# Chuanming-Liu/DAzimSurfTomo

Measured on AMD Instinct MI355X. Metric: FMM traveltime fields/sec (256^2 grid, 16 periods) + LSQR SpMV HBM GB/s, higher is better.
Workload: dtype f32

## Files before the change

dazimsurftomo_amd/csrc/assemble.hip:

```cpp
#include "sparse_internal.h"

#include <rocprim/device/device_scan.hpp>

namespace {

__device__ __forceinline__ bool tikh_face(int cell, int nvx, int nvz, int nzm1, int &i, int &j, int &k) {
  k = cell / (nvx * nvz);
  const int r = cell - k * nvx * nvz;
  j = r / nvx;
  i = r - j * nvx;
  return i == 0 || i == nvx - 1 || j == 0 || j == nvz - 1 || k == 0 || k == nzm1 - 1;
}
__global__ void k_tikh_count(int64_t r0, int64_t nrow, int maxvp, int nvx, int nvz, int nzm1, long *cnt) {
  const int64_t r = (int64_t)blockIdx.x * VB + threadIdx.x;
  if (r > nrow) return;
  int i, j, k;
  cnt[r] = r == nrow ? 0 : (tikh_face((int)((r0 + r) % maxvp), nvx, nvz, nzm1, i, j, k) ? 1 : 7);
}
__global__ void k_tikh_fill(int64_t r0, int64_t nrow, int maxvp, int nvx, int nvz, int nzm1, const long *off, int64_t nnz0,
                            const float *__restrict__ w, int64_t *__restrict__ rowptr, int *__restrict__ col,
                            float *__restrict__ val) {
  const int64_t r = (int64_t)blockIdx.x * VB + threadIdx.x;
  if (r > nrow) return;
  rowptr[r] = nnz0 + off[r];
// ... 94 lines not shown
    if (ratio > 1.0f) sigma = sigma * (float)exp((double)(ratio - 1.0f));
    const float wt = 1.0f / sigma;
    wgt[i] = wt;
    rhs[i] = res[i] * wt;
  }
}
__global__ void k_weight_sums(int64_t n, const float *res, const float *wgt, const float *rhs, double *part) {
  double a[5] = {0, 0, 0, 0, 0};
  for (int64_t i = (int64_t)blockIdx.x * VB + threadIdx.x; i < n; i += (int64_t)gridDim.x * VB) {
    const double r = res[i];
    a[0] += r; a[1] += fabs(r); a[2] += r * r; a[3] += wgt[i]; a[4] += fabsf(rhs[i]);
  }
  __shared__ double s[5][VB / 64];
#pragma unroll
  for (int q = 0; q < 5; q++) {
    const double t = wave_sum(a[q]);
    if ((threadIdx.x & 63) == 0) s[q][threadIdx.x >> 6] = t;
  }
  __syncthreads();
  if (threadIdx.x < 5) {
    double t = 0.0;
    for (int i = 0; i < VB / 64; i++) t += s[threadIdx.x][i];
    part[blockIdx.x * 5 + threadIdx.x] = t;
  }
}
__global__ void k_model_update(int nx, int ny, int nzm1, int joint, float *vs, float *dv, float minvel, float maxvel, float *gc,
                               float *gs) {
  const int nvx = nx - 2, nvz = ny - 2, maxvp = nvx * nvz * nzm1;
  const int ii = blockIdx.x * VB + threadIdx.x;
  if (ii >= maxvp) return;
  const int k = ii / (nvx * nvz), r = ii - k * nvx * nvz, j = r / nvx, i = r - j * nvx;
  float p = dv[ii];
  if (p >= 0.500f) p = 0.500f;
  if (p <= -0.500f) p = -0.500f;
  if (fabsf(p) < 1e-5f) p = 0.0f;
  dv[ii] = p;
  const size_t iv = ((size_t)k * ny + (j + 1)) * nx + (i + 1);
  float v = vs[iv] + p;
  if (v < minvel) v = minvel;
  if (v > maxvel) v = maxvel;
  vs[iv] = v;
  if (joint) {
    if (gc) gc[ii] = dv[maxvp + ii];
    if (gs) gs[ii] = dv[2 * maxvp + ii];
  }
}
__global__ void k_map_update(int nx, int ny, int kmax, int azim, double *pv, float *dm, float minc, float maxc, float *a1, float *a2) {
  const int nvx = nx - 2, nvz = ny - 2, nmap = nvx * nvz * kmax;
  const int ii = blockIdx.x * VB + threadIdx.x;
  if (ii >= nmap) return;
  const int k = ii / (nvx * nvz), r = ii - k * nvx * nvz, j = r / nvx, i = r - j * nvx;
  float p = dm[ii];
  if (p >= 0.500f) p = 0.500f;
  if (p <= -0.500f) p = -0.500f;
  if (fabsf(p) < 1e-5f) p = 0.0f;
  dm[ii] = p;
  const size_t iv = ((size_t)k * ny + (j + 1)) * nx + (i + 1);
  float v = (float)pv[iv] + p;
  if (v < minc) v = minc;
  if (v > maxc) v = maxc;
  pv[iv] = (double)v;
  if (azim) {
    if (a1) a1[ii] = dm[nmap + ii];
    if (a2) a2[ii] = dm[2 * nmap + ii];
  }
}
__global__ void k_update_stats(int ncell, const float *dv, float *out) {
  const float *x = dv + (size_t)blockIdx.x * ncell;
  float mn = INFINITY, mx = -INFINITY;
  double sa = 0.0;
  for (int i = threadIdx.x; i < ncell; i += VB) {
    const float v = x[i];
    mn = fminf(mn, v);
    mx = fmaxf(mx, v);
    sa += fabsf(v);
  }
#pragma unroll
  for (int o = 32; o > 0; o >>= 1) {
    mn = fminf(mn, __shfl_xor(mn, o));
    mx = fmaxf(mx, __shfl_xor(mx, o));
  }
  sa = wave_sum(sa);
  __shared__ float s_mn[VB / 64], s_mx[VB / 64];
  __shared__ double s_sa[VB / 64];
  if ((threadIdx.x & 63) == 0) { s_mn[threadIdx.x >> 6] = mn; s_mx[threadIdx.x >> 6] = mx; s_sa[threadIdx.x >> 6] = sa; }
  __syncthreads();
  if (threadIdx.x == 0) {
    for (int i = 1; i < VB / 64; i++) { mn = fminf(mn, s_mn[i]); mx = fmaxf(mx, s_mx[i]); sa += s_sa[i]; }
    out[blockIdx.x * 3 + 0] = mn; out[blockIdx.x * 3 + 1] = mx; out[blockIdx.x * 3 + 2] = (float)sa;
  }
}

}

extern "C" {

static int append_stencil_rows(dazim_ctx *ctx, dazim_csr *A, bool lap2d, int nvx, int nvz, int nzm1, int64_t maxvp, int64_t row_lo,
                               int64_t nrow, int nblock, const float *w_host, float *dw, long *cnt, long *off);

int dazim_csr_append_tikhonov(dazim_ctx *ctx, dazim_csr *A, int nx, int ny, int nz, int nblock, const float *w_host) {
  if (nblock < 1 || nx < 3 || ny < 3 || nz < 2) return dz_fail(ctx, DAZIM_E_BAD_ARG, "bad arguments to dazim_csr_append_tikhonov");
  return dazim_csr_append_tikhonov_rows(ctx, A, nx, ny, nz, nblock, w_host, 0, (int64_t)(nx - 2) * (ny - 2) * (nz - 1) * nblock);
}
int dazim_csr_append_tikhonov_rows(dazim_ctx *ctx, dazim_csr *A, int nx, int ny, int nz, int nblock, const float *w_host,
                                   int64_t row_lo, int64_t row_hi) {
  if (!ctx || !A || !w_host || nblock < 1 || nx < 3 || ny < 3 || nz < 2) return dz_fail(ctx, DAZIM_E_BAD_ARG, "bad arguments to dazim_csr_append_tikhonov");
  const int nvx = nx - 2, nvz = ny - 2, nzm1 = nz - 1;
  const int64_t maxvp = (int64_t)nvx * nvz * nzm1, nrow = row_hi - row_lo;
  if (row_lo < 0 || row_hi < row_lo || row_hi > maxvp * nblock) return dz_fail(ctx, DAZIM_E_BAD_ARG, "bad row range of the regularisation block");
  if (maxvp * nblock > A->n || maxvp > 0x7ffffff0) return dz_fail(ctx, DAZIM_E_BAD_ARG, "regularisation blocks do not fit the %lld columns", (long long)A->n);
  DZ_HIP(hipSetDevice(ctx->device));
  int rc;
  long *cnt, *off;
  float *dw;
  if ((rc = dz_scratch(ctx, "tikh.cnt", (size_t)(nrow + 1), &cnt)) || (rc = dz_scratch(ctx, "tikh.off", (size_t)(nrow + 1), &off)) ||
      (rc = dz_scratch(ctx, "tikh.w", 64, &dw)))
    return rc;
  if (nblock > 64) return dz_fail(ctx, DAZIM_E_BAD_ARG, "too many regularisation blocks");
  return append_stencil_rows(ctx, A, false, nvx, nvz, nzm1, maxvp, row_lo, nrow, nblock, w_host, dw, cnt, off);
}

static int append_stencil_rows(dazim_ctx *ctx, dazim_csr *A, bool lap2d, int nvx, int nvz, int nzm1, int64_t maxvp, int64_t row_lo,
                               int64_t nrow, int nblock, const float *w_host, float *dw, long *cnt, long *off) {
  int rc;
  void *p;
  DZ_HIP(hipMemcpyAsync(dw, w_host, (size_t)nblock * 4, hipMemcpyHostToDevice, ctx->stream));
  const unsigned nb = (unsigned)((nrow + 1 + VB - 1) / VB);
  if (lap2d)
    hipLaunchKernelGGL(k_lap2d_count, dim3(nb), dim3(VB), 0, ctx->stream, nrow, (int)maxvp, nvx, nvz, cnt);
  else
    hipLaunchKernelGGL(k_tikh_count, dim3(nb), dim3(VB), 0, ctx->stream, row_lo, nrow, (int)maxvp, nvx, nvz, nzm1, cnt);
  auto fill = [&](int64_t *rowptr, int *col, float *val) {
    if (lap2d)
      hipLaunchKernelGGL(k_lap2d_fill, dim3(nb), dim3(VB), 0, ctx->stream, nrow, (int)maxvp, nvx, nvz, off, A->nnz, dw, rowptr, col, val);
    else
      hipLaunchKernelGGL(k_tikh_fill, dim3(nb), dim3(VB), 0, ctx->stream, row_lo, nrow, (int)maxvp, nvx, nvz, nzm1, off, A->nnz, dw,
                         rowptr, col, val);
  };
  size_t tb = 0;
  DZ_HIP(rocprim::exclusive_scan(nullptr, tb, cnt, off, 0l, (size_t)(nrow + 1), rocprim::plus<long>(), ctx->stream));
  if ((rc = dz_scratch(ctx, "tikh.scan", tb + 256, &p))) return rc;
  DZ_HIP(rocprim::exclusive_scan(p, tb, cnt, off, 0l, (size_t)(nrow + 1), rocprim::plus<long>(), ctx->stream));
  long nnz2 = 0;
  DZ_HIP(hipMemcpyAsync(&nnz2, off + nrow, 8, hipMemcpyDeviceToHost, ctx->stream));
  DZ_HIP(hipStreamSynchronize(ctx->stream));
  const int64_t m2 = A->m + nrow, nz2 = A->nnz + nnz2;
  if (nz2 > 0xfffffff0ll) return dz_fail(ctx, DAZIM_E_NNZ_OVERFLOW, "too many stored entries");
  if (A->cap_m >= m2 && A->cap_nnz >= nz2) {
    const int64_t nnz1 = A->nnz;
    fill(A->rowptr + A->m, A->col, A->val);
    DZ_HIP(hipGetLastError());
    A->m = m2;
    A->nnz = nz2;
    if ((rc = dz_build_colblocks(ctx, A, nnz1 > 0 ? nnz1 : 0))) return rc;
    if ((rc = dz_invalidate_transpose(A))) return rc;
    DZ_HIP(hipStreamSynchronize(ctx->stream));
    return 0;
  }
  int64_t *rowptr;
  int *col;
  float *val;
  if ((rc = dz_big_get(ctx, (size_t)(m2 + 1), &rowptr)) || (rc = dz_big_get(ctx, (size_t)(nz2 > 0 ? nz2 : 1), &col)) ||
      (rc = dz_big_get(ctx, (size_t)(nz2 > 0 ? nz2 : 1), &val)))
    return rc;
  DZ_HIP(hipMemcpyAsync(rowptr, A->rowptr, (size_t)A->m * 8, hipMemcpyDeviceToDevice, ctx->stream));
  DZ_HIP(hipMemcpyAsync(col, A->col, (size_t)A->nnz * 4, hipMemcpyDeviceToDevice, ctx->stream));
  DZ_HIP(hipMemcpyAsync(val, A->val, (size_t)A->nnz * 4, hipMemcpyDeviceToDevice, ctx->stream));
  fill(rowptr + A->m, col, val);
  DZ_HIP(hipGetLastError());
  DZ_HIP(hipStreamSynchronize(ctx->stream));
  dz_big_put(ctx, A->rowptr);
  dz_big_put(ctx, A->col);
  dz_big_put(ctx, A->val);
  A->rowptr = rowptr; A->col = col; A->val = val;
  A->m = m2; A->nnz = nz2;
  A->cap_m = A->cap_nnz = 0;
  if ((rc = dz_build_colblocks(ctx, A))) return rc;
  if ((rc = dz_invalidate_transpose(A))) return rc;
  DZ_HIP(hipStreamSynchronize(ctx->stream));
  return 0;
}

int dazim_csr_append_laplacian2d(dazim_ctx *ctx, dazim_csr *A, int nx, int ny, int nmap, const float *w_host) {
  if (!ctx || !A || !w_host || nmap < 1 || nx < 3 || ny < 3) return dz_fail(ctx, DAZIM_E_BAD_ARG, "bad arguments to dazim_csr_append_laplacian2d");
  const int nvx = nx - 2, nvz = ny - 2;
  const int64_t ncell = (int64_t)nvx * nvz, nrow = ncell * nmap;
  if (nrow > A->n || nrow > 0x7ffffff0) return dz_fail(ctx, DAZIM_E_BAD_ARG, "regularisation maps do not fit the %lld columns", (long long)A->n);
  DZ_HIP(hipSetDevice(ctx->device));
  int rc;
  long *cnt, *off;
  float *dw;
  if ((rc = dz_scratch(ctx, "tikh.cnt", (size_t)(nrow + 1), &cnt)) || (rc = dz_scratch(ctx, "tikh.off", (size_t)(nrow + 1), &off)) ||
      (rc = dz_scratch(ctx, "lap2d.w", (size_t)nmap, &dw)))
    return rc;
  return append_stencil_rows(ctx, A, true, nvx, nvz, 1, ncell, 0, nrow, nmap, w_host, dw, cnt, off);
}

int dazim_weight_data(dazim_ctx *ctx, dazim_csr *G, int64_t dall, const float *obst_u, const float *dsyn_u, float *res_u,
                      float *wgt_u, float *rhs_u, float *stats) {
  return dazim_weight_data_sharded(ctx, G, dall, 0, dall, obst_u, dsyn_u, res_u, wgt_u, rhs_u, stats);
}
int dazim_weight_data_sharded(dazim_ctx *ctx, dazim_csr *G, int64_t dall, int64_t row0, int64_t dall_glob, const float *obst_u,
                              const float *dsyn_u, float *res_u, float *wgt_u, float *rhs_u, float *stats) {
  if (!ctx || dall < 1 || !obst_u || !dsyn_u || !res_u || !wgt_u || !rhs_u || (G && G->m < dall) || row0 < 0 || row0 + dall > dall_glob)
    return dz_fail(ctx, DAZIM_E_BAD_ARG, "bad arguments to dazim_weight_data");
  const bool sharded = ctx->comm && dall_glob > dall;
  DZ_HIP(hipSetDevice(ctx->device));
  DzBuf<float> obst, dsyn, res, wgt, rhs;
  int rc;
  if ((rc = obst.init(ctx, obst_u, dall, true, false)) || (rc = dsyn.init(ctx, dsyn_u, dall, true, false)) ||
      (rc = res.init(ctx, res_u, dall, false, true)) || (rc = wgt.init(ctx, wgt_u, dall, false, true)) ||
      (rc = rhs.init(ctx, rhs_u, dall, false, true)))
    return rc;
  float *rel, *ms;
  double *part;
  if ((rc = dz_scratch(ctx, "wd.rel", (size_t)dall, &rel)) || (rc = dz_scratch(ctx, "wd.ms", 16, &ms)) ||
      (rc = dz_scratch(ctx, "wd.part", (size_t)NPART * 5, &part)))
    return rc;
  const int nb = nblk(dall, NPART);
  hipLaunchKernelGGL(k_residual, dim3(nb), dim3(VB), 0, ctx->stream, dall, obst.dev, dsyn.dev, res.dev, rel);
  if (sharded) {
    float *relg;
    if ((rc = dz_scratch(ctx, "wd.relg", (size_t)dall_glob, &relg))) return rc;
    DZ_HIP(hipMemsetAsync(relg, 0, (size_t)dall_glob * 4, ctx->stream));
    DZ_HIP(hipMemcpyAsync(relg + row0, rel, (size_t)dall * 4, hipMemcpyDeviceToDevice, ctx->stream));
    if ((rc = dz_allreduce(ctx, (DzComm *)ctx->comm, relg, (size_t)dall_glob, DZ_F32, DZ_SUM))) return rc;
    hipLaunchKernelGGL(k_sigma_stats, dim3(1), dim3(VB), 0, ctx->stream, dall_glob, relg, ms);
  } else {
    hipLaunchKernelGGL(k_sigma_stats, dim3(1), dim3(VB), 0, ctx->stream, dall, rel, ms);
  }
  hipLaunchKernelGGL(k_sigma_weights, dim3(nb), dim3(VB), 0, ctx->stream, dall, obst.dev, res.dev, rel, ms, wgt.dev, rhs.dev);
  hipLaunchKernelGGL(k_weight_sums, dim3(nb), dim3(VB), 0, ctx->stream, dall, res.dev, wgt.dev, rhs.dev, part);
  DZ_HIP(hipGetLastError());
  std::vector<double> hp((size_t)nb * 5);
  float hms[2];
  DZ_HIP(hipMemcpyAsync(hp.data(), part, hp.size() * 8, hipMemcpyDeviceToHost, ctx->stream));
  DZ_HIP(hipMemcpyAsync(hms, ms, 8, hipMemcpyDeviceToHost, ctx->stream));
  if (G && (rc = dz_scale_rows(ctx, G, dall, wgt.dev))) return rc;
  DZ_HIP(hipStreamSynchronize(ctx->stream));
  if (stats) {
    double a[5] = {0, 0, 0, 0, 0};
    for (int b = 0; b < nb; b++)
      for (int q = 0; q < 5; q++) a[q] += hp[(size_t)b * 5 + q];
    if (sharded && (rc = dazim_comm_allreduce(ctx, a, 5, DZ_F64, DZ_SUM))) return rc;
    const double n = (double)dall_glob, mean = a[0] / n;
    stats[0] = (float)mean;
    stats[1] = (float)sqrt(fmax(a[2] / n - mean * mean, 0.0));
    stats[2] = (float)(a[1] / n);
    stats[3] = (float)sqrt(a[2] / n);
    stats[4] = hms[0];
    stats[5] = hms[1];
    stats[6] = (float)(a[3] / n);
    stats[7] = (float)(a[4] / n);
  }
  if ((rc = res.finish()) || (rc = wgt.finish()) || (rc = rhs.finish())) return rc;
  DZ_HIP(hipStreamSynchronize(ctx->stream));
  return 0;
}

int dazim_model_update(dazim_ctx *ctx, int nx, int ny, int nz, int joint, float *vs_u, float *dv_u, float minvel, float maxvel,
                       float *gc_u, float *gs_u, float *stats) {
  if (!ctx || !vs_u || !dv_u || nx < 3 || ny < 3 || nz < 2) return dz_fail(ctx, DAZIM_E_BAD_ARG, "bad arguments to dazim_model_update");
  DZ_HIP(hipSetDevice(ctx->device));
  const int nzm1 = nz - 1, ncell = (nx - 2) * (ny - 2), maxvp = ncell * nzm1, nblock = joint ? 3 : 1;
  DzBuf<float> vs, dv, gc, gs;
  int rc;
  if ((rc = vs.init(ctx, vs_u, (size_t)nx * ny * nz, true, true)) || (rc = dv.init(ctx, dv_u, (size_t)maxvp * nblock, true, true)) ||
      (rc = gc.init(ctx, gc_u, joint ? maxvp : 0, false, true)) || (rc = gs.init(ctx, gs_u, joint ? maxvp : 0, false, true)))
    return rc;
  hipLaunchKernelGGL(k_model_update, dim3((maxvp + VB - 1) / VB), dim3(VB), 0, ctx->stream, nx, ny, nzm1, joint, vs.dev, dv.dev,
                     minvel, maxvel, joint ? gc.dev : nullptr, joint ? gs.dev : nullptr);
  DZ_HIP(hipGetLastError());
  if (stats) {
    float *p;
    if ((rc = dz_scratch(ctx, "mu.stats", (size_t)nblock * nzm1 * 3, &p))) return rc;
    hipLaunchKernelGGL(k_update_stats, dim3(nblock * nzm1), dim3(VB), 0, ctx->stream, ncell, dv.dev, p);
    DZ_HIP(hipGetLastError());
    DZ_HIP(hipMemcpyAsync(stats, p, (size_t)nblock * nzm1 * 3 * 4, hipMemcpyDeviceToHost, ctx->stream));
  }
  if ((rc = vs.finish()) || (rc = dv.finish()) || (rc = gc.finish()) || (rc = gs.finish())) return rc;
  DZ_HIP(hipStreamSynchronize(ctx->stream));
  return 0;
}

int dazim_phase_map_update(dazim_ctx *ctx, int nx, int ny, int kmax, int azim, double *pv_u, float *dm_u, float minc, float maxc,
                           float *a1_u, float *a2_u, float *stats) {
  if (!ctx || !pv_u || !dm_u || nx < 3 || ny < 3 || kmax < 1) return dz_fail(ctx, DAZIM_E_BAD_ARG, "bad arguments to dazim_phase_map_update");
  DZ_HIP(hipSetDevice(ctx->device));
  const int ncell = (nx - 2) * (ny - 2), nmap = ncell * kmax, nblock = azim ? 3 : 1;
  DzBuf<double> pv;
  DzBuf<float> dm, a1, a2;
  int rc;
  if ((rc = pv.init(ctx, pv_u, (size_t)nx * ny * kmax, true, true)) || (rc = dm.init(ctx, dm_u, (size_t)nmap * nblock, true, true)) ||
      (rc = a1.init(ctx, a1_u, azim ? nmap : 0, false, true)) || (rc = a2.init(ctx, a2_u, azim ? nmap : 0, false, true)))
    return rc;
  hipLaunchKernelGGL(k_map_update, dim3((nmap + VB - 1) / VB), dim3(VB), 0, ctx->stream, nx, ny, kmax, azim ? 1 : 0, pv.dev, dm.dev,
                     minc, maxc, azim ? a1.dev : nullptr, azim ? a2.dev : nullptr);
  DZ_HIP(hipGetLastError());
  if (stats) {
    float *p;
    if ((rc = dz_scratch(ctx, "mu.stats", (size_t)nblock * kmax * 3, &p))) return rc;
    hipLaunchKernelGGL(k_update_stats, dim3(nblock * kmax), dim3(VB), 0, ctx->stream, ncell, dm.dev, p);
    DZ_HIP(hipGetLastError());
    DZ_HIP(hipMemcpyAsync(stats, p, (size_t)nblock * kmax * 3 * 4, hipMemcpyDeviceToHost, ctx->stream));
  }
  if ((rc = pv.finish()) || (rc = dm.finish()) || (rc = a1.finish()) || (rc = a2.finish())) return rc;
  DZ_HIP(hipStreamSynchronize(ctx->stream));
  return 0;
}

}
```

dazimsurftomo_amd/csrc/dazim_internal.h:

```cpp
#pragma once
#include <hip/hip_runtime.h>
#include <rccl/rccl.h>

#include <cstdarg>
#include <cstdio>
#include <cstring>
#include <functional>
#include <map>
#include <memory>
#include <string>
#include <vector>

#include "../../include/dazim.h"

struct dazim_ctx {
  int device = 0;
  hipStream_t stream = nullptr;
  hipEvent_t ev0 = nullptr, ev1 = nullptr;
  std::string err;
  std::map<std::string, double> ksec;
  int num_cu = 256;
  std::map<std::string, int> opts;
  std::map<std::string, std::pair<void *, size_t>> scratch;
  std::map<std::string, std::pair<void *, size_t>> pinned;
  bool fmm_busy = false;
  struct StageBlock { void *p; size_t bytes; bool busy; };
  std::vector<StageBlock> stage;
  std::vector<StageBlock> big;
  hipStream_t stream2 = nullptr;
  hipEvent_t ev_fork = nullptr, ev_a0 = nullptr, ev_a1 = nullptr;
  bool aux_pending = false, aux_timed = false;
  struct AuxRange { const char *p; size_t bytes; };
  std::vector<AuxRange> aux_ranges;
  int (*aux_epilogue)(dazim_ctx *) = nullptr;
  struct ShardPending {
    int nx = 0, ny = 0, nz = 0, kmax = 0;
    const double *send = nullptr;
    double *svs = nullptr, *svp = nullptr, *srho = nullptr;
  } shard;
  struct TiledFields {
    const unsigned *tiled = nullptr;
    const int *tslot = nullptr;
    int nfield = 0, nnx = 0, nnz = 0, stride = 0, tsh = 0;
    const int *fdone = nullptr;
    unsigned nwg = 0;
    volatile unsigned *hprog = nullptr;
    unsigned total_tasks = 0;
  } fields;
  std::function<int()> fmm_finish;
  unsigned *hprog = nullptr;
  hipStream_t stream3 = nullptr;
  hipEvent_t ev_f0 = nullptr, ev_f1 = nullptr, ev_pre = nullptr, ev_r0 = nullptr, ev_r1 = nullptr;
  void *comm = nullptr;
  void (*comm_release)(dazim_ctx *) = nullptr;
  int nranks = 1, rank = 0;
};

int dz_fail(dazim_ctx *c, int code, const char *fmt, ...);
static inline int dz_opt(const dazim_ctx *ctx, const char *name, int def) {
  const auto it = ctx->opts.find(name);
  return it == ctx->opts.end() ? def : it->second;
}

struct DzComm {
  ncclComm_t nccl = nullptr;
  std::string dir;
  std::string tag;
  unsigned seq = 0;
  int nranks = 1, rank = 0;
};
enum { DZ_F32 = 0, DZ_F64 = 1, DZ_I64 = 2, DZ_SUM = 0, DZ_MAX = 1 };
int dz_allgather(dazim_ctx *ctx, DzComm *c, const void *send_dev, void *recv_dev, size_t bytes);
int dz_allreduce(dazim_ctx *ctx, DzComm *c, void *dbuf, size_t count, int dtype, int op);
void dz_comm_abort(dazim_ctx *ctx);
static inline void dz_shard_even(int64_t n, int world, int rank, int64_t *lo, int64_t *hi) {
  const int64_t base = n / world, rem = n % world;
  *lo = rank * base + (rank < rem ? rank : rem);
  *hi = *lo + base + (rank < rem ? 1 : 0);
}

#define DZ_NCCL(call)                                                                                        \
  do {                                                                                                        \
    ncclResult_t r_ = (call);                                                                                 \
    if (r_ != ncclSuccess) return dz_fail(ctx, -2000 - (int)r_, "%s:%d %s -> %s", __FILE__, __LINE__, #call, ncclGetErrorString(r_)); \
  } while (0)
int dz_aux_init(dazim_ctx *ctx);
int dz_async_init(dazim_ctx *ctx);
int dz_fmm_finish(dazim_ctx *ctx);
int dz_join_aux(dazim_ctx *ctx);
int dz_join_aux_if_touched(dazim_ctx *ctx, const void *dev, size_t bytes);

#define DZ_HIP(call)                                                                           \
  do {                                                                                         \
    hipError_t e_ = (call);                                                                    \
    if (e_ != hipSuccess)                                                                      \
      return dz_fail(ctx, -(int)e_ - 1000, "%s:%d %s -> %s", __FILE__, __LINE__, #call,       \
                     hipGetErrorString(e_));                                                   \
  } while (0)

__host__ __device__ constexpr int dz_tile_shift(int nz) { int l = 0; while ((1 << l) < ((nz + 3) >> 2)) l++; return l + 4; }
__host__ __device__ constexpr int dz_tile_records(int nx, int nz) { return ((nx + 3) >> 2) << dz_tile_shift(nz); }
__host__ __device__ __forceinline__ constexpr int dz_tile_x(int x0, int tsh) { return ((x0 >> 2) << tsh) + ((x0 & 3) << 2); }
__host__ __device__ __forceinline__ constexpr int dz_tile_z(int z0) { return ((z0 & ~3) << 2) | (z0 & 3); }

__device__ __forceinline__ double dz_row_kernel(float v, double svs, double svp, double srho) {
  const float coe_a = (2.0947f - 0.8206f * 2 * v + 0.2683f * 3 * (v * v) - 0.0251f * 4 * (v * v * v));
  const float vpft = 0.9409f + 2.0947f * v - 0.8206f * (v * v) + 0.2683f * (v * v * v) - 0.0251f * (v * v * v * v);
  const float coe_rho = coe_a * (1.6612f - 0.4721f * 2 * vpft + 0.0671f * 3 * (vpft * vpft) -
                                 0.0043f * 4 * (vpft * vpft * vpft) + 0.000106f * 5 * (vpft * vpft * vpft * vpft));
  return svp * (double)coe_a + srho * (double)coe_rho + svs;
}

int dz_scratch(dazim_ctx *ctx, const char *name, size_t bytes, void **out);
int dz_pinned(dazim_ctx *ctx, const char *name, size_t bytes, void **out);

size_t dz_trim_caches(dazim_ctx *ctx);
hipError_t dz_malloc_retry(dazim_ctx *ctx, void **p, size_t bytes);
bool dz_is_device_ptr(const void *p);
int dz_stage_get(dazim_ctx *ctx, size_t bytes, void **out);
void dz_stage_put(dazim_ctx *ctx, void *p);
int dz_big_get(dazim_ctx *ctx, size_t bytes, void **out);
void dz_big_put(dazim_ctx *ctx, void *p);
template <class T>
static inline int dz_scratch(dazim_ctx *ctx, const char *name, size_t count, T **out) {
  void *p = nullptr;
  const int rc = dz_scratch(ctx, name, count * sizeof(T), &p);
  *out = (T *)p;
  return rc;
}
template <class T>
static inline int dz_big_get(dazim_ctx *ctx, size_t count, T **out) {
  void *p = nullptr;
  const int rc = dz_big_get(ctx, count * sizeof(T), &p);
  *out = (T *)p;
  return rc;
}

extern "C" int dz_csr_adopt_cap(dazim_ctx *ctx, int64_t m, int64_t n, int64_t nnz, int64_t *rowptr, int *col, float *val,
                                int64_t cap_m, int64_t cap_nnz, dazim_csr **out);

extern "C" int dz_csr_set_twin(dazim_ctx *ctx, dazim_csr *A, dazim_csr *B);

int dz_check_range(dazim_ctx *ctx, const int *a_dev, int64_t n, int lo, int hi, const char *what);

template <class T>
struct DzBuf {
  dazim_ctx *ctx = nullptr;
  T *user = nullptr;
  T *dev = nullptr;
  size_t n = 0;
  bool staged = false, out = false;
  int init(dazim_ctx *c, const T *p, size_t count, bool copy_in, bool copy_out) {
    ctx = c;
    user = const_cast<T *>(p);
    n = count;
    out = copy_out;
    if (!p || count == 0) return 0;
    if (dz_is_device_ptr(p)) {
      dev = user;
      return 0;
    }
    staged = true;
    {
      void *blk = nullptr;
      int rc_ = dz_stage_get(ctx, n * sizeof(T), &blk);
      if (rc_) return rc_;
      dev = (T *)blk;
    }
    if (copy_in) DZ_HIP(hipMemcpyAsync(dev, user, n * sizeof(T), hipMemcpyHostToDevice, ctx->stream));
    return 0;
  }
  int finish() {
    if (staged && out && dev)
      DZ_HIP(hipMemcpyAsync(user, dev, n * sizeof(T), hipMemcpyDeviceToHost, ctx->stream));
    return 0;
  }
  ~DzBuf() {
    if (staged && dev) {
      (void)hipStreamSynchronize(ctx->stream);
      dz_stage_put(ctx, dev);
    }
  }
};

struct DzTimer {
  dazim_ctx *ctx;
  const char *name;
  DzTimer(dazim_ctx *c, const char *n) : ctx(c), name(n) { (void)hipEventRecord(ctx->ev0, ctx->stream); }
  void stop() {
    (void)hipEventRecord(ctx->ev1, ctx->stream);
    (void)hipEventSynchronize(ctx->ev1);
    float ms = 0;
    (void)hipEventElapsedTime(&ms, ctx->ev0, ctx->ev1);
    ctx->ksec[name] = ms * 1e-3;
  }
};
```

dazimsurftomo_amd/csrc/lsmr.hip:

```cpp
#include "sparse_internal.h"

#include <rccl/rccl.h>
#include <cstdlib>

namespace {

__global__ void finish_norm(const double *part, int np, float *res, double *res_d) {
  double t = 0.0;
  for (int i = threadIdx.x; i < np; i += 64) t += part[i];
  t = wave_sum(t);
  if (threadIdx.x == 0) {
    res[0] = (float)sqrt(t);
    if (res_d) res_d[0] = t;
  }
}
__global__ void k_sqrt_sum(const double *sum, float *res) { res[0] = (float)sqrt(sum[0]); }
__global__ void k_axpby_norm(int64_t n, const float *w, float *v, const float *beta_p, float beta_sign, double *part,
                             const int *guard) {
  if (guard && *guard) return;
  const float beta = beta_p ? beta_sign * beta_p[0] : beta_sign;
  double sq = 0.0;
  for (int64_t i = (int64_t)blockIdx.x * VB + threadIdx.x; i < n; i += (int64_t)gridDim.x * VB) {
    const float o = beta * v[i] + w[i];
    v[i] = o;
// ... 232 lines not shown
      v[idx[e]] = vr[e];
      sq += (double)vr[e] * vr[e];
    }
  sq = wave_sum(sq);
  __syncthreads();
  if (lane == 0) s_w[w] = sq;
  __syncthreads();
  if (tid == 0) {
    double t = 0.0;
    for (int i = 0; i < RC_THREADS / 64; i++) t += s_w[i];
    part_out[blockIdx.x] = t;
  }
}
__global__ void k_alpha_update(int64_t n, float *v, float *h, float *hbar, float *x, const double *part, int np,
                               double *partx, LsmrState *S) {
  if (S->stop) return;
  __shared__ float s_f[4];
  const bool half2 = !S->stop2;
  const double t = half2 ? block_total(part, np) : 0.0;
  if (threadIdx.x == 0) {
    LsmrState st = *S;
    const float alpha = half2 ? (float)sqrt(t) : st.alpha;
    float f1, f2, f3;
    lsmr_recur(st, alpha, st.beta, f1, f2, f3);
    s_f[0] = f1; s_f[1] = f2; s_f[2] = f3; s_f[3] = alpha;
    if (blockIdx.x == 0) S->alpha_new = alpha;
  }
  __syncthreads();
  const float f1 = s_f[0], f2 = s_f[1], f3 = s_f[2], alpha = s_f[3];
  const bool scal = half2 && alpha > 0.0f;
  const float a = scal ? 1.0f / alpha : 1.0f;
  double sq = 0.0;
  for (int64_t i = (int64_t)blockIdx.x * VB + threadIdx.x; i < n; i += (int64_t)gridDim.x * VB) {
    float vi = v[i];
    if (scal) {
      vi = a * vi;
      v[i] = vi;
    }
    const float hb = h[i] - f1 * hbar[i];
    const float xn = x[i] + f2 * hb;
    hbar[i] = hb;
    x[i] = xn;
    h[i] = vi - f3 * h[i];
    sq += (double)xn * xn;
  }
  block_partial(sq, partx);
}
__global__ void k_tests(const double *partx, int npx, const float *x, LsmrState *S, dazim_lsmr_rec *trace, int trace_cap) {
  if (S->stop) return;
  const double t = block_total(partx, npx);
  if (threadIdx.x != 0) return;
  LsmrState st = *S;
  float f1, f2, f3;
  lsmr_recur(st, st.alpha_new, st.beta, f1, f2, f3);
  const float normx = (float)sqrt(t);
  st.normx = normx;
  const float test1 = st.normr / st.normb, test2 = st.normAr / (st.normA * st.normr), test3 = 1.0f / st.condA;
  const float t1 = test1 / (1.0f + st.normA * normx / st.normb);
  const float rtol = st.btol + st.atol * st.normA * normx / st.normb;
  int istop = 0;
  if (st.itn >= st.itnlim) istop = 7;
  if (1.0f + test3 <= 1.0f) istop = 6;
  if (1.0f + test2 <= 1.0f) istop = 5;
  if (1.0f + t1 <= 1.0f) istop = 4;
  if (test3 <= st.ctol) istop = 3;
  if (test2 <= st.atol) istop = 2;
  if (test1 <= rtol) istop = 1;
  st.istop = istop;
  st.stop = istop != 0;
  st.stop2 = st.stop;
  if (trace && st.itn < trace_cap) {
    dazim_lsmr_rec r;
    r.itn = st.itn; r.x1 = x[0]; r.normr = st.normr; r.normAr = st.normAr; r.test1 = test1; r.test2 = test2;
    r.test3 = test3; r.rtol = rtol; r.normA = st.normA; r.condA = st.condA;
    trace[st.itn] = r;
  }
  *S = st;
}

constexpr int CHECK = 8, NSLOT = 2;
struct LsmrArgs {
  dazim_ctx *ctx; const dazim_csr *A; const float *b_u;
  float damp, atol, btol, conlim; int itnlim, localSize; float *x_u;
  int *istop_o, *itn_o; float *normA_o, *condA_o, *normr_o, *normAr_o, *normx_o;
  dazim_lsmr_rec *trace; int trace_cap, *trace_n;
};
struct LsmrSolve : LsmrArgs {
  const int64_t m, n;
  DzComm *comm;
  DzBuf<float> b, x;
  double *d_sum = nullptr;
  long long *d_cons = nullptr;
  float *wbuf = nullptr;
  char *gbuf = nullptr;
  const size_t w_sum_off, w_bytes;
  int64_t m_glob;
  int localVecs = 0;
  float *u = nullptr, *v = nullptr, *h = nullptr, *hbar = nullptr, *localV = nullptr, *d_scal = nullptr;
  double *part = nullptr, *part2 = nullptr, *partx = nullptr;
  LsmrState *S = nullptr;
  dazim_lsmr_rec *d_trace = nullptr;
  const int gm, gn, bn, bm;
  int gm_t, gn_t;
  struct Pinned {
    LsmrState *h = nullptr;
    hipEvent_t e0 = nullptr, e1 = nullptr, done[NSLOT] = {}, ta[NSLOT][4] = {};
    ~Pinned() {
      if (e0) (void)hipEventDestroy(e0);
      if (e1) (void)hipEventDestroy(e1);
      for (int i = 0; i < NSLOT; i++) {
        if (done[i]) (void)hipEventDestroy(done[i]);
        for (int j = 0; j < 4; j++)
          if (ta[i][j]) (void)hipEventDestroy(ta[i][j]);
      }
      if (h) (void)hipHostFree(h);
    }
  } guard;
  LsmrState *h_state = nullptr;
  float *h_scal = nullptr;
  const int *g1 = nullptr, *g2 = nullptr;
  int istop = 0, itn = 0, ntrace = 0;
  float normA = 0, condA = 0, normr = 0, normAr = 0, normx = 0, normb = 0;
  double t_spmv = 0, t_spmvt = 0;
  int n_spmv = 0, n_spmvt = 0;
  long n_enq = 0;
  long n_coll = 0;
  bool rccl_allreduce = false;
  int host_syncs = 0;
  int coop_max = 0, rcb = 0;
  int64_t per_thread = 0;
  unsigned reorth_barriers = 0;

  explicit LsmrSolve(const LsmrArgs &a)
      : LsmrArgs(a), m(A->m), n(A->n), comm((DzComm *)ctx->comm), w_sum_off((((size_t)n * 4 + 7) / 8) * 8), w_bytes(w_sum_off + 8),
        m_glob(m), gm(dz_spmv_blocks(ctx, m, n)), gn(dz_spmv_blocks(ctx, n, m)), bn(nblk(n, NPART)), bm(nblk(m, NPART)), gm_t(gm),
        gn_t(gn) {}

  int alloc() {
    int r;
    if ((r = b.init(ctx, b_u, m, true, false)) || (r = x.init(ctx, x_u, n, false, true))) return r;
    if (comm) {
      if ((r = dz_scratch(ctx, "lsmr.cons", 8, &d_cons)) || (r = dz_scratch(ctx, "lsmr.sum", 8, &d_sum)) ||
          (r = dz_scratch(ctx, "lsmr.w", w_bytes / 4, &wbuf)) || (r = dz_scratch(ctx, "lsmr.gather", w_bytes * (size_t)comm->nranks, &gbuf)))
        return r;
    }
    const int npart = gm > gn ? (gm > NPART ? gm : NPART) : (gn > NPART ? gn : NPART);
    if ((r = dz_scratch(ctx, "lsmr.u", (size_t)m, &u)) || (r = dz_scratch(ctx, "lsmr.v", (size_t)n, &v)) ||
        (r = dz_scratch(ctx, "lsmr.h", (size_t)n, &h)) || (r = dz_scratch(ctx, "lsmr.hbar", (size_t)n, &hbar)) ||
        (r = dz_scratch(ctx, "lsmr.part", (size_t)npart, &part)) || (r = dz_scratch(ctx, "lsmr.part2", (size_t)NPART * 2 + 8, &part2)) ||
        (r = dz_scratch(ctx, "lsmr.partx", (size_t)NPART, &partx)) || (r = dz_scratch(ctx, "lsmr.scal", 16, &d_scal)) ||
        (r = dz_scratch(ctx, "lsmr.state", 1, &S)))
      return r;
    if (trace && (r = dz_scratch(ctx, "lsmr.trace", (size_t)trace_cap, &d_trace))) return r;
    if (!dz_use_scatter(ctx, A) && !A->colptr && (r = dz_build_transpose(ctx, const_cast<dazim_csr *>(A)))) return r;
    const int64_t lv = localSize < 0 ? 0 : (localSize < n ? localSize : n);
    if (lv > 0 && (r = dz_scratch(ctx, "lsmr.localV", (size_t)n * lv, &localV))) return r;
    return 0;
  }
  int leave(int code) {
    if (comm) dz_comm_abort(ctx);
    comm = nullptr;
    return code;
  }
  int agree(int rc) {
    if (!comm) return rc;
    long long hv[4] = {rc != 0 ? 1 : 0, (long long)n, -(long long)n, 0}, *dv = d_cons;
    double hm = (double)m;
    if (!dv) return leave(rc ? rc : dz_fail(ctx, -3, "row-sharded LSMR: no memory for the consensus buffer"));
    (void)hipMemcpyAsync(dv, hv, sizeof hv, hipMemcpyHostToDevice, ctx->stream);
    (void)hipMemcpyAsync(dv + 4, &hm, 8, hipMemcpyHostToDevice, ctx->stream);
    const int r1 = dz_allreduce(ctx, comm, dv, 3, DZ_I64, DZ_MAX);
    const int r2 = dz_allreduce(ctx, comm, dv + 4, 1, DZ_F64, DZ_SUM);
    (void)hipMemcpyAsync(hv, dv, sizeof hv, hipMemcpyDeviceToHost, ctx->stream);
    (void)hipMemcpyAsync(&hm, dv + 4, 8, hipMemcpyDeviceToHost, ctx->stream);
    hipError_t e = hipStreamSynchronize(ctx->stream);
    if (rc) return rc;
    if (r1 != 0 || r2 != 0 || e != hipSuccess) return dz_fail(ctx, -2000, "row-sharded LSMR: consensus all-reduce failed");
    if (hv[0]) return dz_fail(ctx, -2001, "row-sharded LSMR: another rank failed during set-up");
    if (hv[1] != -hv[2]) return dz_fail(ctx, DAZIM_E_BAD_ARG, "row-sharded LSMR: the ranks disagree on the number of columns (%lld here, %lld elsewhere)", (long long)n, hv[1]);
    m_glob = (int64_t)hm;
    return 0;
  }
  int prepare() {
    localVecs = localSize < 0 ? 0 : localSize;
    if (m_glob < localVecs) localVecs = (int)m_glob;
    if (n < localVecs) localVecs = (int)n;
    DZ_HIP(hipHostMalloc((void **)&guard.h, sizeof(LsmrState) * (NSLOT + 1) + 64));
    h_state = guard.h;
    h_scal = (float *)(guard.h + NSLOT + 1);
    DZ_HIP(hipEventCreate(&guard.e0));
    DZ_HIP(hipEventCreate(&guard.e1));
    for (int i = 0; i < NSLOT; i++) {
      DZ_HIP(hipEventCreate(&guard.done[i]));
      for (int j = 0; j < 4; j++) DZ_HIP(hipEventCreate(&guard.ta[i][j]));
    }
    return 0;
  }
  void plan_reorth() {
    if (!getenv("DAZIM_CU_MASK")) {
      int occ = 0;
      if (hipOccupancyMaxActiveBlocksPerMultiprocessor(&occ, k_reorth_coop<16>, RC_THREADS, 0) == hipSuccess && occ > 0) coop_max = occ * ctx->num_cu;
      else (void)hipGetLastError();
    }
    rcb = (int)((n + (int64_t)RC_THREADS * RC_EMAX - 1) / ((int64_t)RC_THREADS * RC_EMAX));
    if (rcb < 8) rcb = 8;
    if (rcb > (int)((n + RC_THREADS - 1) / RC_THREADS)) rcb = (int)((n + RC_THREADS - 1) / RC_THREADS);
    if (rcb > RC_BLOCKS) rcb = RC_BLOCKS;
    per_thread = (n + (int64_t)rcb * RC_THREADS - 1) / ((int64_t)rcb * RC_THREADS);
  }
  int norm_to_host(const double *pp, int np, float *res, bool rowwise = false) {
    if (comm && rowwise) {
      hipLaunchKernelGGL(finish_norm, dim3(1), dim3(64), 0, ctx->stream, pp, np, d_scal, d_sum);
      if (const int rr = dz_allreduce(ctx, comm, d_sum, 1, DZ_F64, DZ_SUM)) return rr;
      hipLaunchKernelGGL(k_sqrt_sum, dim3(1), dim3(1), 0, ctx->stream, d_sum, d_scal);
    } else {
      hipLaunchKernelGGL(finish_norm, dim3(1), dim3(64), 0, ctx->stream, pp, np, d_scal, (double *)nullptr);
    }
    DZ_HIP(hipMemcpyAsync(h_scal, d_scal, 4, hipMemcpyDeviceToHost, ctx->stream));
    DZ_HIP(hipStreamSynchronize(ctx->stream));
    *res = h_scal[0];
    return 0;
  }
  int spmvT(const float *beta_p, float sign, const int *g) {
    if (!comm) return dz_launch_spmvT(ctx, A, u, 1.0f, v, beta_p, sign, part, &gn_t, g);
    DZ_HIP(hipMemsetAsync(wbuf, 0, n * 4, ctx->stream));
    if (const int r = dz_launch_spmvT(ctx, A, u, 1.0f, wbuf, nullptr, 1.0f, nullptr, nullptr, g)) return r;
    if (const int rr = dz_allreduce(ctx, comm, wbuf, (size_t)n, DZ_F32, DZ_SUM)) return rr;
    hipLaunchKernelGGL(k_axpby_norm, dim3(bn), dim3(VB), 0, ctx->stream, n, wbuf, v, beta_p, sign, part, g);
    gn_t = bn;
    return 0;
  }
  int start() {
    int rc;
    DZ_HIP(hipEventRecord(guard.e0, ctx->stream));
    hipLaunchKernelGGL(k_copy, dim3(bm), dim3(VB), 0, ctx->stream, m, b.dev, u);
    DZ_HIP(hipMemsetAsync(v, 0, n * 4, ctx->stream));
    DZ_HIP(hipMemsetAsync(x.dev, 0, n * 4, ctx->stream));
    DZ_HIP(hipMemsetAsync(hbar, 0, n * 4, ctx->stream));
    hipLaunchKernelGGL(k_sumsq, dim3(bm), dim3(VB), 0, ctx->stream, m, u, part);
    float alpha = 0.0f, beta = 0.0f;
    if ((rc = norm_to_host(part, bm, &beta, true))) return rc;
    if (beta > 0.0f) {
      hipLaunchKernelGGL(k_scal_inv, dim3(bm), dim3(VB), 0, ctx->stream, m, u, d_scal, 1.0f);
      if ((rc = spmvT(nullptr, 1.0f, nullptr))) return rc;
      if ((rc = norm_to_host(part, gn_t, &alpha))) return rc;
    }
    if (alpha > 0.0f) hipLaunchKernelGGL(k_scal_inv, dim3(bn), dim3(VB), 0, ctx->stream, n, v, d_scal, 1.0f);
    normAr = alpha * beta;
    normb = beta;
    if (trace) {
      memset(&trace[0], 0, sizeof trace[0]);
      trace[0].normr = beta; trace[0].normAr = normAr; trace[0].test1 = 1.0f; trace[0].test2 = beta > 0.0f ? alpha / beta : 0.0f;
      ntrace = 1;
    }
    if (normAr == 0.0f) return 0;
    if (localVecs > 0) hipLaunchKernelGGL(k_copy, dim3(bn), dim3(VB), 0, ctx->stream, n, v, localV);
    hipLaunchKernelGGL(k_copy, dim3(bn), dim3(VB), 0, ctx->stream, n, v, h);
    LsmrState &s0 = h_state[NSLOT];
    memset(&s0, 0, sizeof s0);
    s0.alpha = alpha; s0.beta = beta; s0.alphabar = alpha; s0.zetabar = alpha * beta; s0.rho = 1; s0.rhobar = 1; s0.cbar = 1;
    s0.betadd = beta; s0.rhodold = 1; s0.normA2 = alpha * alpha; s0.minrbar = 1e+30f; s0.normb = beta;
    s0.ctol = conlim > 0.0f ? 1.0f / conlim : 0.0f;
    s0.normr = beta; s0.normAr = normAr; s0.damp = damp; s0.atol = atol; s0.btol = btol; s0.itnlim = itnlim;
    DZ_HIP(hipMemcpyAsync(S, &s0, sizeof s0, hipMemcpyHostToDevice, ctx->stream));
    if (d_trace) DZ_HIP(hipMemsetAsync(d_trace, 0, (size_t)trace_cap * sizeof(dazim_lsmr_rec), ctx->stream));
    g1 = &S->stop;
    g2 = &S->stop2;
    plan_reorth();
    rccl_allreduce = comm && comm->nccl && dz_opt(ctx, "comm.allreduce", 0) == 1;
    DZ_HIP(hipMemsetAsync(part2 + 2 * NPART, 0, 64, ctx->stream));
    return 0;
  }
  int half_step_u(hipEvent_t *tev) {
    if (tev) DZ_HIP(hipEventRecord(tev[0], ctx->stream));
    if (const int r = dz_launch_spmvA(ctx, A, v, u, &S->alpha, -1.0f, part, &gm_t, g1)) return r;
    if (tev) DZ_HIP(hipEventRecord(tev[1], ctx->stream));
    return 0;
  }
  int half_step_v(float *slot, hipEvent_t *tev) {
    int r;
    if (!comm) {
      hipLaunchKernelGGL(k_beta_scal_u, dim3(bm > bn ? bm : bn), dim3(VB), 0, ctx->stream, m, u, part, gm_t,
                         (const double *)nullptr, n, v, slot, S);
      if (tev) DZ_HIP(hipEventRecord(tev[2], ctx->stream));
      if ((r = spmvT(&S->beta, -1.0f, g2))) return r;
      if (tev) DZ_HIP(hipEventRecord(tev[3], ctx->stream));
      return 0;
    }
    float *d_bp = reinterpret_cast<float *>(d_sum + 4);
    double *w_sum = reinterpret_cast<double *>(reinterpret_cast<char *>(wbuf) + w_sum_off);
    const int bmn = bm > bn ? bm : bn;
    hipLaunchKernelGGL(k_local_norm_scal, dim3(bm), dim3(VB), 0, ctx->stream, m, u, part, gm_t, w_sum, d_bp, S);
    if (tev) DZ_HIP(hipEventRecord(tev[2], ctx->stream));
    DZ_HIP(hipMemsetAsync(wbuf, 0, n * 4, ctx->stream));
    if ((r = dz_launch_spmvT(ctx, A, u, 1.0f, wbuf, nullptr, 1.0f, nullptr, nullptr, g1))) return r;
    hipLaunchKernelGGL(k_scale_by, dim3(bn), dim3(VB), 0, ctx->stream, n, wbuf, d_bp, g1);
    if (tev) DZ_HIP(hipEventRecord(tev[3], ctx->stream));
    if (rccl_allreduce) {
      DZ_NCCL(ncclGroupStart());
      const ncclResult_t ra = ncclAllReduce(wbuf, wbuf, (size_t)n, ncclFloat, ncclSum, comm->nccl, ctx->stream);
      const ncclResult_t rb = ncclAllReduce(w_sum, w_sum, 1, ncclDouble, ncclSum, comm->nccl, ctx->stream);
      const ncclResult_t rg = ncclGroupEnd();
      if (ra != ncclSuccess || rb != ncclSuccess || rg != ncclSuccess) {
        const ncclResult_t bad = ra != ncclSuccess ? ra : (rb != ncclSuccess ? rb : rg);
        return dz_fail(ctx, -2000 - (int)bad, "row-sharded LSMR: grouped ncclAllReduce -> %s", ncclGetErrorString(bad));
      }
// ... 156 lines not shown
```

dazimsurftomo_amd/csrc/rays.hip:

```cpp
#include <cmath>
#include <chrono>
#include <unistd.h>

#include "dazim_internal.h"

#include <rocprim/device/device_scan.hpp>
#include <rocprim/device/device_radix_sort.hpp>

namespace {

constexpr int GDX = 5, GDZ = 5;
constexpr int RM = DAZIM_RMAX;
constexpr float EARTH = 6371.0f;
constexpr float FTOL = 1e-4f;

struct RayArgs {
  dazim_geom g;
  int nx, ny, nz, kmax;
  long nray;
  const int *field;
  const float *rcx, *rcz;
  const float *scx, *scz;
  const int *period;
  const int *kidx;
  const float *veln;
  const float *ttn;
  const int *tslot;
  int tsh;
  long fstride;
  const int *fdone;
  int *defer_mark;
  int max_quads;
  int sweeps;
  const float *ttnr;
  const int *nstsr;
  const dazim_refbox *boxes;
  const float *vels;
  const double *svs, *svp, *srho;
  unsigned nvx_magic;
  const double *skern;
  const float *lsen;
  double r_dnx, r_dnz, r_dnxr, r_dnzr, r_dvx, r_dvz, r_e2dnx, r_e2dnxr;
  float dplh;
  float *dsurf;
  int *status;
  int *rbflag;
  long *count;
  int *nlist;
  unsigned short *lcell;
  float *lval;
  float *fdm_scratch;
  int LK;
  int lcap;
  const unsigned *perm;
  unsigned *qcount;
  float2 *pts;
  int *npts;
  int pcap;
  int dense;
  long *countd;
  int keep_small;
  const long *rowptr;
  float *val;
  int *col;
};

__device__ __forceinline__ float dz_sinf(float x) {
  if (!(x > 0.0f && x < 3.1415927f)) return (float)sin((double)x);
  const double y = (double)x - 1.5707963267948966192;
  const double y2 = y * y;
  double p = -1.5619206968586226e-16;
  p = fma(p, y2, 4.7794773323873853e-14);
  p = fma(p, y2, -1.1470745597729725e-11);
  p = fma(p, y2, 2.0876756987868099e-09);
  p = fma(p, y2, -2.7557319223985891e-07);
  p = fma(p, y2, 2.4801587301587302e-05);
  p = fma(p, y2, -1.3888888888888889e-03);
  p = fma(p, y2, 4.1666666666666664e-02);
  p = fma(p, y2, -0.5);
  p = fma(p, y2, 1.0);
  return (float)p;
}

__device__ __forceinline__ void step_azimuth(float x0, float z0, float x1, float z1, float &c2psi, float &s2psi) {
  const float PI_F = 3.1415926535898f;
  const float evtlat = (PI_F / 2 - x0) * 180.0f / PI_F, evtlon = z0 * 180.0f / PI_F;
  const float stalat = (PI_F / 2 - x1) * 180.0f / PI_F, stalon = z1 * 180.0f / PI_F;
  const double pi = (double)3.1415926535898f;
  const float piby2 = (float)(pi / (double)2.f);
  const double rad = (double)2.f * pi / (double)360.f;
  const double sph = (double)(1.0f / 298.257f);
  const double scolat = (double)piby2 - atan((1. - sph) * (1. - sph) * tan((double)stalat * rad));
  const double ecolat = (double)piby2 - atan((1. - sph) * (1. - sph) * tan((double)evtlat * rad));
  const double slon = (double)stalon * rad, elon = (double)evtlon * rad;
  const double a = sin(scolat) * cos(slon), b = sin(scolat) * sin(slon), c = cos(scolat);
  const double dd = sin(elon), ee = -cos(elon), cc = cos(ecolat);
  const double gg = -cc * ee, hh = cc * dd, kk = -sin(ecolat);
  const double rhs1 = (a - dd) * (a - dd) + (b - ee) * (b - ee) + c * c - (double)2.f;
  const double rhs2 = (a - gg) * (a - gg) + (b - hh) * (b - hh) + (c - kk) * (c - kk) - (double)2.f;
  double daz = atan2(rhs1, rhs2);
  if (daz < 0.0) daz = daz + 2 * pi;
  float az = (float)(daz / rad);
  if (fabsf(az - 360.f) < .00001f) az = 0.0f;
  const float rgpsi = az / 180 * PI_F;
  c2psi = (float)cos((double)(2.0f * rgpsi));
  s2psi = (float)sin((double)(2.0f * rgpsi));
}

__device__ __forceinline__ float divr(float x, double rd) { return (float)((double)x * rd); }

__device__ __forceinline__ void basis(float v, float b[4]) {
  const float om = 1.0f - v;
  b[0] = om * om * om / 6.0f;
  b[1] = (4.0f - 6.0f * (v * v) + 3.0f * (v * v * v)) / 6.0f;
  b[2] = (1.0f + 3.0f * v + 3.0f * (v * v) - 3.0f * (v * v * v)) / 6.0f;
  b[3] = v * v * v / 6.0f;
}

__device__ __forceinline__ float div6(float x) { return divr(x, 1.0 / 6.0); }
__device__ __forceinline__ float basis1(float v, int i) {
  const float om = 1.0f - v;
  const float n0 = om * om * om;
  const float n1 = 4.0f - 6.0f * (v * v) + 3.0f * (v * v * v);
  const float n2 = 1.0f + 3.0f * v + 3.0f * (v * v) - 3.0f * (v * v * v);
  const float n3 = v * v * v;
  return div6(i == 0 ? n0 : (i == 1 ? n1 : (i == 2 ? n2 : n3)));
}

__device__ __forceinline__ float vel_at(const dazim_geom &g, const float *veln, int ipx, int ipz, float drx, float drz,
                                        double rdnx, double rdnz) {
  float vel = 0.0f;
#pragma unroll
  for (int l = 1; l <= 2; l++)
#pragma unroll
    for (int m = 1; m <= 2; m++) {
      float produ = (1.0f - fabsf(divr((float)(m - 1) * g.dnz - drz, rdnz)));
      produ = produ * (1.0f - fabsf(divr((float)(l - 1) * g.dnx - drx, rdnx)));
      if (ipz - 1 + m <= g.nnz && ipx - 1 + l <= g.nnx && ipz - 1 + m >= 1 && ipx - 1 + l >= 1)
        vel = vel + veln[(size_t)(ipx - 2 + l) * g.nnz + (ipz - 2 + m)] * produ;
    }
  return vel;
}

__device__ __forceinline__ float bilin_cell(const dazim_geom &g, const float *veln, int cx, int cz, float px, float pz,
                                            double rdnx, double rdnz) {
  const float drx = (px - g.gox) - (float)(cx - 1) * g.dnx;
  const float drz = (pz - g.goz) - (float)(cz - 1) * g.dnz;
  float biv = 0.0f;
#pragma unroll
  for (int i = 1; i <= 2; i++)
#pragma unroll
    for (int j = 1; j <= 2; j++) {
      const float produ = (1.0f - fabsf(divr((float)(i - 1) * g.dnx - drx, rdnx))) *
                          (1.0f - fabsf(divr((float)(j - 1) * g.dnz - drz, rdnz)));
      biv = biv + veln[(size_t)(cx - 2 + i) * g.nnz + (cz - 2 + j)] * produ;
    }
  return biv;
}

__global__ void k_row_kernels(long n, int kmax, long ncol, const float *__restrict__ vels, const double *__restrict__ svs,
                              const double *__restrict__ svp, const double *__restrict__ srho, double *__restrict__ out) {
  const long i = (long)blockIdx.x * blockDim.x + threadIdx.x;
  if (i >= n) return;
  const long k = i / (kmax * ncol), c = i % ncol;
  out[i] = dz_row_kernel(vels[k * ncol + c], svs[i], svp[i], srho[i]);
}

__global__ void k_ray_keys(long nray, const int *__restrict__ field, const float *__restrict__ scx, const float *__restrict__ scz,
                           const float *__restrict__ rcx, const float *__restrict__ rcz, float inv_dmax, int dbits,
                           unsigned *__restrict__ keys, unsigned *__restrict__ iota, const int *__restrict__ order) {
  const long i = (long)blockIdx.x * blockDim.x + threadIdx.x;
  if (i >= nray) return;
  const int f = field[i];
  const float dx = scx[f] - rcx[i], dz = (scz[f] - rcz[i]) * __sinf(rcx[i]);
  const float d = sqrtf(dx * dx + dz * dz) * inv_dmax;
  const unsigned dmaxq = (1u << dbits) - 1u;
  unsigned q = d >= 1.0f ? dmaxq : (unsigned)(d * (float)dmaxq);
  keys[i] = ((unsigned)(order ? order[f] : f) << dbits) | (dmaxq - q);
  iota[i] = (unsigned)i;
}

constexpr int GP_COUNT = 8, GP_EMIT = 16;
constexpr int RAYS_MINW = 4;
constexpr int RPW_MAX = 64 / GP_COUNT;
__device__ __forceinline__ void cbar() { asm volatile("" ::: "memory"); }

template <bool EMIT, bool AZIM, bool TILED, bool MAP>
__global__ __launch_bounds__(64, AZIM ? 2 : RAYS_MINW) void rays_kernel(RayArgs A_) {
  using ArgP = const __attribute__((address_space(4))) RayArgs *;
  auto launder = [](ArgP p) {
    int z;
    asm volatile("v_mov_b32 %0, 0" : "=v"(z));
    return (ArgP)((const __attribute__((address_space(4))) char *)p + __builtin_amdgcn_readfirstlane(z));
  };
  ArgP Ap = launder((ArgP)__builtin_amdgcn_kernarg_segment_ptr());
#define A (*Ap)
#define RAYS_ARGS_FRESH Ap = launder(Ap)
  constexpr int GP = EMIT ? GP_EMIT : GP_COUNT;
  constexpr int RPW = 64 / GP;
  constexpr int LPR = 16 / GP;
  constexpr int LSTEP = 4 / LPR;
  constexpr unsigned GMASK = (1u << GP) - 1u;
  extern __shared__ __attribute__((aligned(16))) unsigned short s_lists[];
  dazim_geom g;
  g.nvx = A.g.nvx; g.nvz = A.g.nvz; g.nnx = A.g.nnx; g.nnz = A.g.nnz;
  g.gox = A.g.gox; g.goz = A.g.goz; g.dnx = A.g.dnx; g.dnz = A.g.dnz; g.dvx = A.g.dvx; g.dvz = A.g.dvz;
  const int lane = threadIdx.x, grp = lane / GP, gl = lane & (GP - 1);
  const int lm = gl & 3, l0 = gl >> 2;
  const int nnx = g.nnx, nnz = g.nnz, nvx = g.nvx, nvz = g.nvz, ldf = nvz + 2, nf = ldf * (nvx + 2);
  constexpr int NG = AZIM ? 3 : 1;
  const unsigned nvx_magic = A.nvx_magic;
  const int LC = A.lcap;
  unsigned short *s_list = s_lists + (size_t)grp * LC;
  float *gfdm = A.fdm_scratch + ((size_t)blockIdx.x * RPW + grp) * nf * NG;
  float *gfdmc = gfdm + nf, *gfdms = gfdm + 2 * nf;
  const float gox = g.gox, goz = g.goz, dnx = g.dnx, dnz = g.dnz, dvx = g.dvx, dvz = g.dvz;
  const double rdnx = A.r_dnx, rdnz = A.r_dnz, rdnxr = A.r_dnxr, rdnzr = A.r_dnzr, rdvx = A.r_dvx, rdvz = A.r_dvz;
  const unsigned gmask_shift = grp * GP;
  const long nquad = (A.nray + RPW - 1) / RPW;
  const int nxcd = (gridDim.x % 8 == 0) ? 8 : 1;
  unsigned *qcnt = A.qcount + (EMIT ? 8 : 0);
  int chunk = (int)(blockIdx.x % nxcd);
  int traced = 0;
  for (;;) {
    RAYS_ARGS_FRESH;
    long quad = -1;
    if (lane == 0) {
      for (int tried = 0; tried < nxcd; tried++) {
        const long lo = nquad * chunk / nxcd, hi = nquad * (chunk + 1) / nxcd;
        const long b = lo < hi ? (long)atomicAdd(&qcnt[chunk], 1u) : hi;
        if (lo + b < hi) {
          quad = lo + b;
          break;
        }
        if (!EMIT && A.sweeps > 1 && lo < hi && b < (hi - lo) * A.sweeps) {
          quad = lo + b % (hi - lo);
          break;
        }
        chunk = (chunk + 1) % nxcd;
      }
    }
    quad = ((long)__shfl((int)(quad >> 32), 0) << 32) | (unsigned)__shfl((int)quad, 0);
    chunk = __shfl(chunk, 0);
    if (quad < 0) break;
    const long slot = quad * RPW + grp;
    if (!EMIT && A.defer_mark) {
      if (!A.defer_mark[quad]) continue;
      if (A.fdone) {
        const int fq = slot < A.nray ? A.field[A.perm ? (long)A.perm[slot] : slot] : -1;
        const int st = fq >= 0 ? __hip_atomic_load(A.fdone + fq, __ATOMIC_ACQUIRE, __HIP_MEMORY_SCOPE_AGENT) : 1;
        if (__ballot(st != 1) != 0) continue;
        __builtin_amdgcn_fence(__ATOMIC_ACQUIRE, "agent");
      }
      if (A.max_quads > 0 && traced >= A.max_quads) break;
      int mine = 0;
      if (lane == 0) mine = __hip_atomic_exchange(A.defer_mark + quad, 0, __ATOMIC_RELAXED, __HIP_MEMORY_SCOPE_AGENT);
      mine = __shfl(mine, 0);
      if (!mine) continue;
      traced++;
      if (lane == 0) atomicAdd(&A.qcount[18], 1u);
    }
    if (slot >= A.nray) continue;
    const long ray = A.perm ? (long)A.perm[slot] : slot;
    const int f = A.field[ray];
    const float scx = A.scx[f], scz = A.scz[f], rcx = A.rcx[ray], rcz = A.rcz[ray];
    const float *veln = A.veln + (size_t)(A.period[f] - 1) * nnx * nnz;
    const float *ttn = TILED ? A.ttn + (size_t)(A.tslot ? A.tslot[f] : f) * A.fstride : A.ttn + (size_t)f * nnx * nnz;
    const int tsh = TILED ? A.tsh : 0;
    auto tnode = [&](int x0, int z0) -> float {
      return TILED ? ttn[dz_tile_x(x0, tsh) + dz_tile_z(z0)] : ttn[(size_t)x0 * nnz + z0];
    };
    const float *ttnr = A.ttnr + (size_t)f * RM * RM;
    const int *nstsr = A.nstsr + (size_t)f * RM * RM;
    const dazim_refbox bx = A.boxes[f];
    const int saved = EMIT ? A.nlist[ray] : -1;
    if (saved < 0)
      for (int i = gl; i < nf * NG; i += GP) gfdm[i] = 0.0f;
    cbar();
    int status = 0, rb = 0;
    if (!EMIT) {
      int irx = (int)divr(rcx - gox, rdnx) + 1, irz = (int)divr(rcz - goz, rdnz) + 1;
      if (irx < 1 || irx > nnx || irz < 1 || irz > nnz) status = DAZIM_E_RECEIVER_OUTSIDE;
      if (!status) {
        if (irx == nnx) irx--;
        if (irz == nnz) irz--;
        const int isx = (int)divr(scx - gox, rdnx) + 1, isz = (int)divr(scz - goz, rdnz) + 1;
        float sred = ((scx - rcx) * EARTH) * ((scx - rcx) * EARTH);
        const float e2 = (scz - rcz) * EARTH * dz_sinf(rcx);
        sred = sqrtf(sred + e2 * e2);
        bool sw = sred < A.dplh;
        if (isx == irx && isz == irz) sw = true;
        float trr;
        if (sw) {
          const float vs = bilin_cell(g, veln, isx, isz, scx, scz, rdnx, rdnz);
          const float vr = bilin_cell(g, veln, irx, irz, rcx, rcz, rdnx, rdnz);
          trr = 2.0f * sred / (vs + vr);
        } else {
          const float drx = (rcx - gox) - (float)(irx - 1) * dnx;
          const float drz = (rcz - goz) - (float)(irz - 1) * dnz;
          trr = 0.0f;
#pragma unroll
          for (int k = 1; k <= 2; k++)
#pragma unroll
            for (int l = 1; l <= 2; l++) {
              const float produ = (1.0f - fabsf(divr((float)(l - 1) * dnz - drz, rdnz))) *
                                  (1.0f - fabsf(divr((float)(k - 1) * dnx - drx, rdnx)));
              trr = trr + tnode(irx - 2 + k, irz - 2 + l) * produ;
            }
        }
        if (gl == 0) A.dsurf[ray] = trr;
      }
    }
    const float goxr = bx.goxr, gozr = bx.gozr, dnxr = bx.dnxr, dnzr = bx.dnzr;
    const int nnxr = bx.nnxr, nnzr = bx.nnzr;
    const int isx = (int)divr(scx - goxr, rdnxr) + 1, isz = (int)divr(scz - gozr, rdnzr) + 1;
    const float dpl = 0.5f * A.dplh;
    int ipx = (int)divr(rcx - gox, rdnx) + 1, ipz = (int)divr(rcz - goz, rdnz) + 1;
    if (ipx < 1 || ipx >= nnx || ipz < 1 || ipz >= nnz) status = DAZIM_E_RECEIVER_OUTSIDE;
    if (!status && saved < 0) {
      float x0 = rcx, z0 = rcz;
      float sinx0 = dz_sinf(x0);
      int sw = 0;
      float sred = ((scx - x0) * EARTH) * ((scx - x0) * EARTH);
      float e2 = (scz - z0) * EARTH * sinx0;
      sred = sqrtf(sred + e2 * e2);
      if (sred < 2.0f * dpl) sw = 1;
      int ipxr = (int)divr(rcx - goxr, rdnxr) + 1, ipzr = (int)divr(rcz - gozr, rdnzr) + 1;
      auto in_refined = [&](int px, int pz) -> int {
        if (px < 1 || px >= nnxr || pz < 1 || pz >= nnzr) return 0;
        const int *sp = nstsr + (size_t)(px - 1) * RM + (pz - 1);
        if (sp[0] != 0 || sp[1] != 0) return 0;
        if (sp[RM] != 0 || sp[RM + 1] != 0) return 0;
        return 1;
      };
      int igref = in_refined(ipxr, ipzr);
      if (sw == 0 && igref == 1 && ipxr == isx && ipzr == isz) sw = 1;
      const bool keep_pts = !EMIT && A.pts != nullptr && gl == 0;
      float2 *rp = A.pts ? A.pts + (size_t)ray * A.pcap : nullptr;
      int np = 1;
      if (keep_pts) {
        rp[0] = make_float2(rcx, rcz);
        if (sw == 1) { if (A.pcap > 1) rp[1] = make_float2(scx, scz); np = 2; }
      }
      int cbx = -100, cbz = -100;
      float acc[LPR], accc[LPR], accs[LPR];
#pragma unroll
      for (int q = 0; q < LPR; q++) acc[q] = accc[q] = accs[q] = 0.0f;
      auto flush = [&]() {
        if (cbx > -100) {
#pragma unroll
          for (int q = 0; q < LPR; q++) {
            const int fi = (cbx + lm) * ldf + (cbz + l0 + q * LSTEP);
            gfdm[fi] = acc[q];
            if (AZIM) { gfdmc[fi] = accc[q]; gfdms[fi] = accs[q]; }
          }
        }
      };
      float tc00, tc01, tc10, tc11, tr00 = 0.0f, tr01 = 0.0f, tr10 = 0.0f, tr11 = 0.0f;
      auto load_corner_times = [&]() {
        if (TILED) {
          const int x0 = dz_tile_x(ipx - 1, tsh), x1 = dz_tile_x(ipx, tsh), z0 = dz_tile_z(ipz - 1), z1 = dz_tile_z(ipz);
          tc00 = ttn[x0 + z0]; tc01 = ttn[x0 + z1]; tc10 = ttn[x1 + z0]; tc11 = ttn[x1 + z1];
        } else {
          const float *t = ttn + (size_t)(ipx - 1) * nnz + (ipz - 1);
          tc00 = t[0]; tc01 = t[1]; tc10 = t[nnz]; tc11 = t[nnz + 1];
        }
        if (ipxr >= 1 && ipxr < nnxr && ipzr >= 1 && ipzr < nnzr) {
          const float *u = ttnr + (size_t)(ipxr - 1) * RM + (ipzr - 1);
          tr00 = u[0]; tr01 = u[1]; tr10 = u[RM]; tr11 = u[RM + 1];
        }
      };
      load_corner_times();
      bool carry = false;
      float vel_c = 0.0f, vi_c = 0.0f, wi_c[LPR];
#pragma unroll
      for (int q = 0; q < LPR; q++) wi_c[q] = 0.0f;
// ... 127 lines not shown
            cbx = nbx;
            cbz = nbz;
#pragma unroll
            for (int q = 0; q < LPR; q++) {
              const int fi = (cbx + lm) * ldf + (cbz + l0 + q * LSTEP);
              acc[q] = gfdm[fi];
              if (AZIM) { accc[q] = gfdmc[fi]; accs[q] = gfdms[fi]; }
            }
          }
#pragma unroll
          for (int q = 0; q < LPR; q++) {
            const float rdc1 = vi * wi[q] / (vel * vel);
            const float rdc2 = vio * wio[q] / (velo * velo);
            float r1 = -(rdc1 + rdc2) * dinc / 2.0f;
            acc[q] = r1 + acc[q];
            if (AZIM) {
              r1 = -(rdc1 * c2psi + rdc2 * c2psi) * dinc / 2.0f;
              accc[q] = r1 + accc[q];
              r1 = -(rdc1 * s2psi + rdc2 * s2psi) * dinc / 2.0f;
              accs[q] = r1 + accs[q];
            }
          }
        }
        carry = endsame;
        vel_c = vel;
        vi_c = vi;
#pragma unroll
        for (int q = 0; q < LPR; q++) wi_c[q] = wi[q];
        x0 = x1;
        z0 = z1;
        sinx0 = sinx1;
      }
      flush();
      if (keep_pts) A.npts[ray] = np <= A.pcap ? np : -1;
    }
    cbar();
    if (!EMIT && gl == 0) {
      if (A.pts && status) A.npts[ray] = 0;
      A.status[ray] = status;
      A.rbflag[ray] = rb;
    }
    int nlist = 0;
    if (saved >= 0) {
      nlist = saved;
      const size_t o = (size_t)ray * A.LK, ov = o * NG;
      for (int i = gl; i < nlist; i += GP) {
        const int c = A.lcell[o + i];
        const int jj = (int)__umulhi((unsigned)c, nvx_magic) + 1, kk = c - (jj - 1) * nvx + 1;
        s_list[i] = (unsigned short)c;
        gfdm[kk * ldf + jj] = A.lval[ov + i];
        if (AZIM) {
          gfdmc[kk * ldf + jj] = A.lval[ov + A.LK + i];
          gfdms[kk * ldf + jj] = A.lval[ov + 2 * A.LK + i];
        }
      }
    } else if (!status) {
      for (int base = 0; base < nvz * nvx; base += GP) {
        const int c = base + gl;
        bool keep = false;
        if (c < nvz * nvx) {
          const int jj = (int)__umulhi((unsigned)c, nvx_magic) + 1, kk = c - (jj - 1) * nvx + 1;
          keep = fabsf(gfdm[kk * ldf + jj]) >= FTOL;
        }
        const unsigned m = (unsigned)((__ballot(keep) >> gmask_shift) & GMASK);
        const int pos = nlist + __popc(m & ((1u << gl) - 1u));
        if (keep && pos < LC) s_list[pos] = (unsigned short)c;
        nlist += __popc(m);
      }
    }
    cbar();
    if (!EMIT) {
      const size_t o = (size_t)ray * A.LK, ov = o * NG;
      if (nlist <= A.LK)
        for (int i = gl; i < nlist; i += GP) {
          const int c = s_list[i];
          const int jj = (int)__umulhi((unsigned)c, nvx_magic) + 1, kk = c - (jj - 1) * nvx + 1;
          A.lcell[o + i] = (unsigned short)c;
          A.lval[ov + i] = gfdm[kk * ldf + jj];
          if (AZIM) {
            A.lval[ov + A.LK + i] = gfdmc[kk * ldf + jj];
            A.lval[ov + 2 * A.LK + i] = gfdms[kk * ldf + jj];
          }
        }
      if (gl == 0) A.nlist[ray] = (status || nlist <= A.LK) ? (status ? 0 : nlist) : -1;
    }
    const size_t ncol = (size_t)A.nx * A.ny;
    const int kslot = A.kidx[f] - 1;
    long cnt = 0;
    const long rstart = EMIT ? A.rowptr[ray] : 0;
    const int nparpi = nvx * nvz * (A.nz - 1);
    const int nlay = MAP ? 1 : A.nz - 1;
    const int bstride = MAP ? A.kmax * nvx * nvz : nparpi;
    const int poff = MAP ? (A.period[f] - 1) * nvx * nvz : 0;
    const bool lovf = nlist > LC;
    const int ntot = lovf ? nvz * nvx : nlist;
    long cntd = 0;
    int jjL = 1, kkL = 1;
    if (A.dense) {
      int clast = -1;
      if (!lovf) {
        if (nlist > 0) clast = s_list[nlist - 1];
      } else {
        for (int base = ((nvz * nvx - 1) / GP) * GP; base >= 0 && clast < 0; base -= GP) {
          const int c = base + gl;
          bool k2 = false;
          if (c < nvz * nvx) {
            const int jj = (int)__umulhi((unsigned)c, nvx_magic) + 1, kk = c - (jj - 1) * nvx + 1;
            k2 = fabsf(gfdm[kk * ldf + jj]) >= FTOL;
          }
          const unsigned m2 = (unsigned)((__ballot(k2) >> gmask_shift) & GMASK);
          if (m2) clast = base + (31 - __clz(m2));
        }
      }
      if (clast >= 0) { jjL = (int)__umulhi((unsigned)clast, nvx_magic) + 1; kkL = clast - (jjL - 1) * nvx + 1; }
    }
    constexpr int RC = 8;
    const bool rowcache = !lovf && ntot <= RC * GP && (MAP || A.skern != nullptr) && !A.dense;
    if (rowcache) {
      int sidx[RC], cbase[RC], fidx[RC];
#pragma unroll
      for (int i = 0; i < RC; i++) {
        const int li = i * GP + gl;
        const int c = li < ntot ? (int)s_list[li] : 0;
        const int jj = (int)__umulhi((unsigned)c, nvx_magic) + 1, kk = c - (jj - 1) * nvx + 1;
        sidx[i] = jj * (nvx + 2) + kk;
        cbase[i] = (jj - 1) * nvx + kk;
        fidx[i] = kk * ldf + jj;
      }
      for (int blk = 0; blk < NG; blk++) {
        float fdv[RC];
        const float *fsrc = blk == 0 ? gfdm : (blk == 1 ? gfdmc : gfdms);
#pragma unroll
        for (int i = 0; i < RC; i++) fdv[i] = (i * GP + gl < ntot) ? fsrc[fidx[i]] : 0.0f;
        for (int k = 1; k <= nlay; k++) {
          const size_t sk = ((size_t)(k - 1) * A.kmax + kslot) * ncol;
          const int nk = blk * bstride + poff + (k - 1) * nvz * nvx;
#pragma unroll
          for (int i = 0; i < RC; i++) {
            if (i * GP >= ntot) break;
            const bool cell = i * GP + gl < ntot;
            float rowv = 0.0f;
            bool keep = false;
            if (cell) {
              if (MAP) rowv = fdv[i];
              else if (blk == 0) rowv = (float)(A.skern[sk + sidx[i]] * (double)fdv[i]);
              else rowv = A.lsen[sk + sidx[i]] * fdv[i];
              keep = A.keep_small ? (rowv != 0.0f) : (fabsf(rowv) > FTOL);
            }
            const unsigned m = (unsigned)((__ballot(keep) >> gmask_shift) & GMASK);
            if (EMIT && keep) {
              const long pos = rstart + cnt + __popc(m & ((1u << gl) - 1u));
              A.val[pos] = rowv;
              A.col[pos] = nk + cbase[i] - 1;
            }
            cnt += __popc(m);
          }
        }
      }
    } else
    for (int blk = 0; blk < NG; blk++)
      for (int k = 1; k <= nlay; k++) {
        for (int base = 0; base < ntot; base += GP) {
          const int li = base + gl;
          bool keep = false, keepd = false;
          float rowv = 0.0f;
          int nn = 0;
          bool cell = li < ntot;
          int c = 0;
          if (cell) c = lovf ? li : s_list[li];
          const int jj = (int)__umulhi((unsigned)c, nvx_magic) + 1, kk = c - (jj - 1) * nvx + 1;
          if (cell && lovf) cell = fabsf(gfdm[kk * ldf + jj]) >= FTOL;
          if (cell && MAP) {
            rowv = (blk == 0 ? gfdm : (blk == 1 ? gfdmc : gfdms))[kk * ldf + jj];
            keep = A.keep_small ? (rowv != 0.0f) : (fabsf(rowv) > FTOL);
            nn = blk * bstride + poff + (jj - 1) * nvx + kk;
          } else if (cell) {
            const size_t si = ((size_t)(k - 1) * A.kmax + kslot) * ncol + (size_t)jj * (nvx + 2) + kk;
            if (blk == 0) {
              const float fd = gfdm[kk * ldf + jj];
              double r;
              if (A.skern) {
                r = A.skern[si] * (double)fd;
              } else {
                const float v = A.vels[((size_t)(k - 1) * A.ny + jj) * A.nx + kk];
                const float coe_a = (2.0947f - 0.8206f * 2 * v + 0.2683f * 3 * (v * v) - 0.0251f * 4 * (v * v * v));
                const float vpft = 0.9409f + 2.0947f * v - 0.8206f * (v * v) + 0.2683f * (v * v * v) - 0.0251f * (v * v * v * v);
                const float coe_rho = coe_a * (1.6612f - 0.4721f * 2 * vpft + 0.0671f * 3 * (vpft * vpft) -
                                               0.0043f * 4 * (vpft * vpft * vpft) + 0.000106f * 5 * (vpft * vpft * vpft * vpft));
                r = (A.svp[si] * (double)coe_a + A.srho[si] * (double)coe_rho + A.svs[si]) * (double)fd;
              }
              rowv = (float)r;
              if (A.dense) {
                const float vL = A.vels[((size_t)(k - 1) * A.ny + jjL) * A.nx + kkL];
                const float caL = (2.0947f - 0.8206f * 2 * vL + 0.2683f * 3 * (vL * vL) - 0.0251f * 4 * (vL * vL * vL));
                const float vpL = 0.9409f + 2.0947f * vL - 0.8206f * (vL * vL) + 0.2683f * (vL * vL * vL) - 0.0251f * (vL * vL * vL * vL);
                const float crL = caL * (1.6612f - 0.4721f * 2 * vpL + 0.0671f * 3 * (vpL * vpL) -
                                         0.0043f * 4 * (vpL * vpL * vpL) + 0.000106f * 5 * (vpL * vpL * vpL * vpL));
                const double rd = (A.svp[si] * (double)caL + A.srho[si] * (double)crL + A.svs[si]) * (double)fd;
                keepd = (float)rd != 0.0f;
                if (EMIT && A.dense == 1) rowv = (float)rd;
              }
            } else {
              rowv = A.lsen[si] * (blk == 1 ? gfdmc : gfdms)[kk * ldf + jj];
              keepd = rowv != 0.0f;
            }
            keep = A.keep_small ? (rowv != 0.0f) : (fabsf(rowv) > FTOL);
            if (EMIT && A.dense == 1) keep = keepd;
            nn = blk * bstride + (k - 1) * nvz * nvx + (jj - 1) * nvx + kk;
          }
          if (!EMIT && A.dense == 2) cntd += __popc((unsigned)((__ballot(keepd) >> gmask_shift) & GMASK));
          const unsigned m = (unsigned)((__ballot(keep) >> gmask_shift) & GMASK);
          if (EMIT && keep) {
            const long pos = rstart + cnt + __popc(m & ((1u << gl) - 1u));
            A.val[pos] = rowv;
            A.col[pos] = nn - 1;
          }
          cnt += __popc(m);
        }
      }
    if (!EMIT && gl == 0) {
      A.count[ray] = cnt;
      if (A.dense == 2) A.countd[ray] = cntd;
      if (lovf) atomicAdd(&A.qcount[16], 1u);
      if (!status && nlist > A.LK) atomicAdd(&A.qcount[17], 1u);
    }
  }
}
#undef A
#undef RAYS_ARGS_FRESH

struct RayBuild {
  dazim_ctx *ctx;
  int nx = 0, ny = 0, nz = 0, kmax = 0, nfield = 0;
  float goxd = 0, gozd = 0, dvxd = 0, dvzd = 0;
  const float *vels = nullptr, *scx = nullptr, *scz = nullptr, *veln = nullptr, *ttn = nullptr, *ttnr = nullptr, *rcx = nullptr, *rcz = nullptr;
  const float *lsen = nullptr;
  const int *period = nullptr, *kidx = nullptr, *nstsr = nullptr, *field = nullptr;
  const dazim_refbox *boxes = nullptr;
  const double *svs = nullptr, *svp = nullptr, *srho = nullptr;
  int64_t nray = 0;
  float *dsurf = nullptr;
  dazim_csr **G = nullptr;
  int64_t *nnz_out = nullptr;
  int *n_boundary = nullptr;
  bool map = false, azim = false;
  struct StreamSwap {
    dazim_ctx *c; hipStream_t main; bool on = false;
    void restore() { if (on) { c->stream = main; on = false; } }
    ~StreamSwap() {
      if (on) (void)hipStreamSynchronize(c->stream);
      restore();
    }
  } swap;
  struct {
    DzBuf<float> vels, scx, scz, veln, ttn, ttnr, rcx, rcz, dsurf, lsen;
    DzBuf<int> period, kidx, nstsr, field;
    DzBuf<dazim_refbox> boxes;
    DzBuf<double> svs, svp, srho;
  } d;
  struct Arrays {
    dazim_ctx *c; int64_t *rp = nullptr; float *v = nullptr; int *cl = nullptr; int64_t nnz = 0, cap_nnz = 0; bool keep = false;
    ~Arrays() { if (!keep) { dz_big_put(c, rp); dz_big_put(c, v); dz_big_put(c, cl); } }
  } arrays, arrays_d;
  dazim_geom g;
  bool joint = false, tiled = false, overlap = false, twin = false;
  size_t nn = 0, nr = 0, ncol = 0, nk = 0, nr1 = 0, lds = 0;
  int64_t res_rows = 0, res_nnz = 0;
  long nwg = 0;
  double overlap_tail_s = 0.0;
  RayArgs A;
  explicit RayBuild(dazim_ctx *c) : ctx(c), swap{c, c ? c->stream : nullptr}, arrays{c}, arrays_d{c} {}
  int check() {
    if (!ctx || !G) return DAZIM_E_BAD_ARG;
    joint = map ? azim : lsen != nullptr;
    if (map) nz = 2;
    if (map && dz_opt(ctx, "rays.dense_twin", 0) != 0)
      return dz_fail(ctx, DAZIM_E_BAD_ARG, "dazim_rays_build_G_maps: option rays.dense_twin serves the 3-D program's diagnostics only");
    if (dazim_geometry(nx, ny, goxd, gozd, dvxd, dvzd, &g)) return dz_fail(ctx, DAZIM_E_BAD_ARG, "bad grid");
    if (nray < 0 || nfield < 1 || nz < 2 || kmax < 1 || (size_t)g.nvx * g.nvz > 65535u) return dz_fail(ctx, DAZIM_E_BAD_ARG, "bad arguments to dazim_rays_build_G");
    tiled = ttn == nullptr;
    if (tiled && (!ctx->fields.tiled || ctx->fields.nfield != nfield || ctx->fields.nnx != g.nnx || ctx->fields.nnz != g.nnz))
      return dz_fail(ctx, DAZIM_E_BAD_ARG, "dazim_rays_build_G: ttn is NULL and the last dazim_fmm_batch call did not keep %d fields of this grid inside the library (call it with ttn = NULL)", nfield);
    if (!scx || !scz || !period || !veln || !ttnr || !nstsr || !boxes || !dsurf ||
        (!map && (!vels || !svs || !svp || !srho)) || (nray > 0 && (!field || !rcx || !rcz)))
      return dz_fail(ctx, DAZIM_E_BAD_ARG, "dazim_rays_build_G: NULL array (the refined fields ttnr, nstsr and boxes of dazim_fmm_batch are required)");
    DZ_HIP(hipSetDevice(ctx->device));
    return 0;
  }
  int decide_overlap() {
    overlap = (bool)ctx->fmm_finish && tiled && ctx->fields.fdone && nray > 0;
    if (overlap && ctx->aux_epilogue && ctx->comm && ((DzComm *)ctx->comm)->nccl) overlap = false;
    if (overlap)
      for (const void *q : {(const void *)vels, (const void *)scx, (const void *)scz, (const void *)period, (const void *)veln,
                            (const void *)ttnr, (const void *)nstsr, (const void *)boxes, (const void *)field, (const void *)rcx,
                            (const void *)rcz, (const void *)svs, (const void *)svp, (const void *)srho, (const void *)dsurf,
                            (const void *)kidx, (const void *)lsen})
        if (q && !dz_is_device_ptr(q)) overlap = false;
    if (!overlap) { const int rcf = dz_fmm_finish(ctx); if (rcf) return rcf; }
    if (overlap) {
      DZ_HIP(hipStreamWaitEvent(ctx->stream3, ctx->ev_pre, 0));
      ctx->stream = ctx->stream3;
      swap.on = true;
    }
    return dz_join_aux(ctx);
  }
  int stage_inputs() {
    nn = (size_t)g.nnx * g.nnz; nr = (size_t)RM * RM; ncol = (size_t)nx * ny;
    int rc;
    if (!map && (rc = d.vels.init(ctx, vels, (size_t)nz * ncol, true, false))) return rc;
    if ((rc = d.scx.init(ctx, scx, nfield, true, false)) || (rc = d.scz.init(ctx, scz, nfield, true, false)) ||
        (rc = d.period.init(ctx, period, nfield, true, false)) || (rc = d.kidx.init(ctx, kidx ? kidx : period, nfield, true, false)) ||
        (rc = d.veln.init(ctx, veln, nn * kmax, true, false)) || (!tiled && (rc = d.ttn.init(ctx, ttn, nn * nfield, true, false))) ||
        (rc = d.ttnr.init(ctx, ttnr, nr * nfield, true, false)) || (rc = d.nstsr.init(ctx, nstsr, nr * nfield, true, false)) ||
        (rc = d.boxes.init(ctx, boxes, nfield, true, false)) || (rc = d.field.init(ctx, field, nray, true, false)) ||
        (rc = d.rcx.init(ctx, rcx, nray, true, false)) || (rc = d.rcz.init(ctx, rcz, nray, true, false)))
      return rc;
    nk = (size_t)nz * kmax * ncol;
    if (!map && ((rc = d.svs.init(ctx, svs, nk, true, false)) || (rc = d.svp.init(ctx, svp, nk, true, false)) ||
                  (rc = d.srho.init(ctx, srho, nk, true, false))))
      return rc;
    if ((rc = d.dsurf.init(ctx, dsurf, nray, false, true))) return rc;
    if (joint && !map && (rc = d.lsen.init(ctx, lsen, (size_t)(nz - 1) * kmax * ncol, true, false))) return rc;
    if ((rc = dz_check_range(ctx, d.period.dev, nfield, 1, kmax, "period_idx"))) return rc;
    if ((rc = dz_check_range(ctx, d.kidx.dev, nfield, 1, kmax, "kernel_idx"))) return rc;
    return dz_check_range(ctx, d.field.dev, nray, 0, nfield - 1, "field_of_ray");
  }
  int kernel_constants() {
    int rc;
    A.g = g;
    A.nx = nx; A.ny = ny; A.nz = nz; A.kmax = kmax;
    A.nray = nray;
    A.field = d.field.dev; A.rcx = d.rcx.dev; A.rcz = d.rcz.dev; A.scx = d.scx.dev; A.scz = d.scz.dev;
    A.period = d.period.dev; A.kidx = d.kidx.dev; A.veln = d.veln.dev; A.ttn = d.ttn.dev; A.ttnr = d.ttnr.dev;
    A.tslot = nullptr; A.tsh = 0; A.fstride = (long)nn;
    if (tiled) {
      A.ttn = reinterpret_cast<const float *>(ctx->fields.tiled);
      A.tslot = ctx->fields.tslot; A.tsh = ctx->fields.tsh; A.fstride = ctx->fields.stride;
    }
    ctx->ksec["rays.tiled_fields"] = tiled ? 1.0 : 0.0;
    ctx->ksec["rays.map"] = map ? 1.0 : 0.0;
    ctx->ksec["rays.overlap"] = overlap ? 1.0 : 0.0;
    A.fdone = overlap ? ctx->fields.fdone : nullptr;
    A.defer_mark = nullptr; A.max_quads = 0; A.sweeps = 1;
    A.nstsr = d.nstsr.dev; A.boxes = d.boxes.dev; A.vels = d.vels.dev; A.svs = d.svs.dev; A.svp = d.svp.dev; A.srho = d.srho.dev;
    A.lsen = joint && !map ? d.lsen.dev : nullptr;
    A.skern = nullptr;
    {
      const unsigned dv = (unsigned)g.nvx;
      A.nvx_magic = (unsigned)((0x100000000ull + dv - 1) / dv);
      for (unsigned c = 0; c < 65536u; c++)
        if ((unsigned)(((unsigned long long)c * A.nvx_magic) >> 32) != c / dv) return dz_fail(ctx, DAZIM_E_BAD_ARG, "internal: reciprocal of nvx");
    }
    if (!map && dz_opt(ctx, "rays.skern", 1) != 0) {
      double *pk;
      if ((rc = dz_scratch(ctx, "rays.skern", nk, &pk))) return rc;
      hipLaunchKernelGGL(k_row_kernels, dim3((unsigned)((nk + 255) / 256)), dim3(256), 0, ctx->stream, (long)nk, kmax, (long)ncol,
                         d.vels.dev, d.svs.dev, d.svp.dev, d.srho.dev, pk);
      DZ_HIP(hipGetLastError());
      A.skern = pk;
    }
    {
      float dpl = g.dnx * EARTH;
      float rd1 = g.dnz * EARTH * sinf(g.gox);
      if (rd1 < dpl) dpl = rd1;
      rd1 = g.dnz * EARTH * sinf(g.gox + (float)(g.nnx - 1) * g.dnx);
      if (rd1 < dpl) dpl = rd1;
      A.dplh = dpl;
    }
    {
      const float dnxr = g.dvx / (float)(GDX * 8), dnzr = g.dvz / (float)(GDZ * 8);
      const float e2dnx = 2.0f * EARTH * g.dnx, e2dnxr = 2.0f * EARTH * dnxr;
      A.r_dnx = 1.0 / (double)g.dnx;   A.r_dnz = 1.0 / (double)g.dnz;
      A.r_dnxr = 1.0 / (double)dnxr;   A.r_dnzr = 1.0 / (double)dnzr;
      A.r_dvx = 1.0 / (double)g.dvx;   A.r_dvz = 1.0 / (double)g.dvz;
      A.r_e2dnx = 1.0 / (double)e2dnx; A.r_e2dnxr = 1.0 / (double)e2dnxr;
    }
    return 0;
  }
  int scratch() {
    int rc;
    nr1 = (size_t)(nray > 0 ? nray : 1);
    if ((rc = dz_scratch(ctx, "rays.status", nr1, &A.status))) return rc;
    if ((rc = dz_scratch(ctx, "rays.rb", nr1, &A.rbflag))) return rc;
    if ((rc = dz_scratch(ctx, "rays.count", (size_t)(nray + 1), &A.count))) return rc;
    A.lcap = g.nvx * g.nvz <= 4096 ? 512 : 1024;
    if (dz_opt(ctx, "rays.lcap", 0) >= 16 && dz_opt(ctx, "rays.lcap", 0) <= 8192) A.lcap = dz_opt(ctx, "rays.lcap", 0);
    if (A.lcap > g.nvx * g.nvz) A.lcap = g.nvx * g.nvz;
    A.LK = A.lcap;
    A.keep_small = dz_opt(ctx, "rays.keep_small", 0) != 0 ? 1 : 0;
    A.pts = nullptr; A.npts = nullptr; A.pcap = 0;
    if (dz_opt(ctx, "rays.keep_paths", 0) != 0) {
      A.pcap = 4 * (g.nnx + g.nnz) + 16;
      if ((rc = dz_scratch(ctx, "rays.pts", nr1 * (size_t)A.pcap, &A.pts))) return rc;
      if ((rc = dz_scratch(ctx, "rays.npts", nr1, &A.npts))) return rc;
      DZ_HIP(hipMemsetAsync(A.npts, 0, nr1 * 4, ctx->stream));
    }
    ctx->ksec["rays.path_cap"] = A.pcap;
    ctx->ksec["rays.path_rays"] = A.pts ? (double)nray : 0.0;
    twin = dz_opt(ctx, "rays.dense_twin", 0) != 0 && !A.keep_small;
    A.dense = twin ? 2 : 0;
    A.countd = nullptr;
    if (twin) {
      if ((rc = dz_scratch(ctx, "rays.countd", (size_t)(nray + 1), &A.countd))) return rc;
      DZ_HIP(hipMemsetAsync(A.countd, 0, (size_t)(nray + 1) * 8, ctx->stream));
    }
    if ((rc = dz_scratch(ctx, "rays.nlist", nr1, &A.nlist))) return rc;
    if ((rc = dz_scratch(ctx, "rays.lcell", nr1 * A.LK, &A.lcell))) return rc;
    if ((rc = dz_scratch(ctx, "rays.lval", nr1 * A.LK * (joint ? 3 : 1), &A.lval))) return rc;
    res_rows = (int64_t)g.nvx * g.nvz * (map ? kmax : nz - 1) * (joint ? 3 : 1);
    res_nnz = (map ? 5 : 7) * res_rows;
    if (dz_opt(ctx, "csr.reserve_rows", 0) > res_rows) res_rows = dz_opt(ctx, "csr.reserve_rows", 0);
    if (dz_opt(ctx, "csr.reserve_nnz", 0) > res_nnz) res_nnz = dz_opt(ctx, "csr.reserve_nnz", 0);
    if ((rc = dz_big_get(ctx, (size_t)(nray + res_rows + 1), &arrays.rp))) return rc;
    A.dsurf = d.dsurf.dev;
    A.rowptr = (const long *)arrays.rp; A.val = nullptr; A.col = nullptr;
    return 0;
  }
  template <int I> static const void *kernel_no() { return (const void *)rays_kernel<(I & 8) != 0, (I & 4) != 0, (I & 2) != 0, (I & 1) != 0>; }
  const void *kern(bool emit) const {
    static const void *const tab[16] = {kernel_no<0>(),  kernel_no<1>(),  kernel_no<2>(),  kernel_no<3>(), kernel_no<4>(),  kernel_no<5>(),
                                        kernel_no<6>(),  kernel_no<7>(),  kernel_no<8>(),  kernel_no<9>(), kernel_no<10>(), kernel_no<11>(),
                                        kernel_no<12>(), kernel_no<13>(), kernel_no<14>(), kernel_no<15>()};
    return tab[(emit ? 8 : 0) + (joint ? 4 : 0) + (tiled ? 2 : 0) + (map ? 1 : 0)];
  }
  int launch(bool emit, const RayArgs &R, long nwg_) {
    RayArgs args = R;
    void *params[] = {&args};
    DZ_HIP(hipLaunchKernel(kern(emit), dim3((unsigned)nwg_), dim3(64), params, lds, ctx->stream));
    return 0;
  }
  int launch_shape() {
    lds = (size_t)A.lcap * 2 * RPW_MAX + 16;
    DZ_HIP(hipFuncSetAttribute(kern(false), hipFuncAttributeMaxDynamicSharedMemorySize, (int)lds));
    DZ_HIP(hipFuncSetAttribute(kern(true), hipFuncAttributeMaxDynamicSharedMemorySize, (int)lds));
    int per_cu = (int)(160 * 1024 / (lds + 256));
    {
      int occ = 0;
      const void *kf = kern(false);
      if (hipOccupancyMaxActiveBlocksPerMultiprocessor(&occ, kf, 64, lds) == hipSuccess && occ > 0 && occ < per_cu) per_cu = occ;
    }
    if (per_cu > 16) per_cu = 16;
    if (per_cu < 1) return dz_fail(ctx, DAZIM_E_BAD_ARG, "inversion grid too large for the LDS cell lists");
    if (dz_opt(ctx, "rays.wg_per_cu", 0) > 0 && dz_opt(ctx, "rays.wg_per_cu", 0) < per_cu) per_cu = dz_opt(ctx, "rays.wg_per_cu", 0);
    nwg = (long)ctx->num_cu * per_cu;
    if (nwg > (nray + RPW_MAX - 1) / RPW_MAX) nwg = (nray + RPW_MAX - 1) / RPW_MAX;
    if (nwg >= 8) nwg -= nwg % 8;
    if (nwg < 1) nwg = 1;
    return dz_scratch(ctx, "rays.fdm", (size_t)nwg * RPW_MAX * (g.nvx + 2) * (g.nvz + 2) * (joint ? 3 : 1), &A.fdm_scratch);
  }
  int sort_rays() {
    int rc;
    A.perm = nullptr;
    if (nray >= 64 && nray < (1ll << 32) && dz_opt(ctx, "rays.sort", 1) != 0) {
      int fbits = 1;
      while ((1ll << fbits) < nfield) fbits++;
      const int dbits = 32 - fbits > 12 ? 12 : 32 - fbits;
      if (dbits >= 4) {
        unsigned *k0, *k1, *v0, *v1;
        if ((rc = dz_scratch(ctx, "rays.sortbuf", (size_t)nray * 4 + 16, &k0))) return rc;
        k1 = k0 + nray; v0 = k1 + nray; v1 = v0 + nray;
        const float ex = (float)g.nnx * g.dnx, ez = (float)g.nnz * g.dnz;
        const float inv_dmax = 1.0f / sqrtf(ex * ex + ez * ez);
        hipLaunchKernelGGL(k_ray_keys, dim3((unsigned)((nray + 255) / 256)), dim3(256), 0, ctx->stream, (long)nray, d.field.dev, d.scx.dev,
                           d.scz.dev, d.rcx.dev, d.rcz.dev, inv_dmax, dbits, k0, v0, overlap ? A.tslot : (const int *)nullptr);
        size_t tb = 0;
        DZ_HIP(rocprim::radix_sort_pairs(nullptr, tb, k0, k1, v0, v1, (size_t)nray, 0, fbits + dbits, ctx->stream));
        void *tmp;
        if ((rc = dz_scratch(ctx, "rays.sorttmp", tb + 256, &tmp))) return rc;
        DZ_HIP(rocprim::radix_sort_pairs(tmp, tb, k0, k1, v0, v1, (size_t)nray, 0, fbits + dbits, ctx->stream));
        A.perm = v1;
      }
    }
    if ((rc = dz_scratch(ctx, "rays.qcount", 32, &A.qcount))) return rc;
    DZ_HIP(hipMemsetAsync(A.qcount, 0, 128, ctx->stream));
    if (overlap) {
      const size_t nq = (size_t)((nray + RPW_MAX - 1) / RPW_MAX) + 8;
      if ((rc = dz_scratch(ctx, "rays.defer", nq, &A.defer_mark))) return rc;
      DZ_HIP(hipMemsetAsync(A.defer_mark, 0, nq * 4, ctx->stream));
    }
    return 0;
  }
  int count_pass() { return nray > 0 ? launch(false, A, nwg) : 0; }
  int count_passes_beside_eikonal() {
    int rc;
    const auto t_poll0 = std::chrono::steady_clock::now();
    auto fmm_over = [&]() {
      const bool over = hipEventQuery(ctx->ev_f1) == hipSuccess;
      if (!over) (void)hipGetLastError();
      return over;
    };
    if (ctx->fields.hprog && ctx->fields.total_tasks > 0) {
      const unsigned slack = ctx->fields.nwg / 4 + 8 * 16;
      const unsigned total = ctx->fields.total_tasks;
      const unsigned want = total > slack ? total - slack : 0;
      for (;;) {
        unsigned have = 0;
        for (int c = 0; c < 8; c++) have += ctx->fields.hprog[c];
        if (have >= want || fmm_over()) break;
        if (std::chrono::steady_clock::now() - t_poll0 > std::chrono::seconds(120)) break;
        usleep(50);
      }
    }
    const unsigned nquad_all = (unsigned)((nray + RPW_MAX - 1) / RPW_MAX);
    unsigned pending = nquad_all, *h_traced = nullptr;
    { void *hp; if ((rc = dz_pinned(ctx, "rays.host_pending", 64, &hp))) return rc; h_traced = (unsigned *)hp; }
    DZ_HIP(hipMemsetAsync(A.defer_mark, 1, (size_t)nquad_all * 4, ctx->stream));
    int npass = 0;
    bool collected = false, ev0_set = false;
    unsigned left_by_first = 0;
    int rcf = 0;
    while (pending > 0) {
      const bool last = fmm_over();
      if (last && !collected) {
        swap.restore();
        DZ_HIP(hipStreamSynchronize(ctx->stream3));
        rcf = dz_fmm_finish(ctx);
        collected = true;
        if (rcf) break;
        if (npass == 0) (void)hipEventRecord(ctx->ev_r1, ctx->stream);
        (void)hipEventRecord(ctx->ev0, ctx->stream);
        ev0_set = true;
      }
      long nwg_pass = nwg;
      A.max_quads = 0;
      A.sweeps = collected ? 1 : 3;
      if (collected) A.fdone = nullptr;
      DZ_HIP(hipMemsetAsync(A.qcount, 0, 32, ctx->stream));
      if ((rc = launch(false, A, nwg_pass))) return rc;
      if (!collected) DZ_HIP(hipEventRecord(ctx->ev_r1, ctx->stream));
      DZ_HIP(hipMemcpyAsync(h_traced, A.qcount + 18, 4, hipMemcpyDeviceToHost, ctx->stream));
      DZ_HIP(hipStreamSynchronize(ctx->stream));
      const unsigned before = pending;
      pending = collected ? 0u : nquad_all - *h_traced;
      if (npass == 0) left_by_first = pending;
      npass++;
      if (pending > 0 && pending == before) usleep(100);
    }
    swap.restore();
    if (!collected) rcf = dz_fmm_finish(ctx);
    DZ_HIP(hipStreamSynchronize(ctx->stream3));
    if (rcf) return rcf;
    ctx->ksec["rays.passes"] = npass;
    ctx->ksec["rays.deferred_quads"] = left_by_first;
    A.fdone = nullptr; A.defer_mark = nullptr; A.max_quads = 0; A.sweeps = 1;
    float ms_tail = 0;
    if (hipEventElapsedTime(&ms_tail, ctx->ev_f1, ctx->ev_r1) == hipSuccess && ms_tail > 0) overlap_tail_s = ms_tail * 1e-3;
    if (!ev0_set) (void)hipEventRecord(ctx->ev0, ctx->stream);
    return 0;
  }
  int scan_and_emit(Arrays &M, long *count, int64_t slack, bool dense_twin) {
    int rc; void *p; size_t tb = 0;
    DZ_HIP(rocprim::exclusive_scan(nullptr, tb, count, (long *)M.rp, 0l, (size_t)(nray + 1), rocprim::plus<long>(), ctx->stream));
    if ((rc = dz_scratch(ctx, "rays.scan", tb + 256, &p))) return rc;
    DZ_HIP(rocprim::exclusive_scan(p, tb, count, (long *)M.rp, 0l, (size_t)(nray + 1), rocprim::plus<long>(), ctx->stream));
    DZ_HIP(hipMemcpyAsync(&M.nnz, M.rp + nray, 8, hipMemcpyDeviceToHost, ctx->stream));
    DZ_HIP(hipStreamSynchronize(ctx->stream));
    M.cap_nnz = M.nnz + slack;
    const size_t cap = (size_t)(M.cap_nnz > 0 ? M.cap_nnz : 1);
    if ((rc = dz_big_get(ctx, cap, &M.v)) || (rc = dz_big_get(ctx, cap, &M.cl))) return rc;
    RayArgs R = A;
    R.rowptr = (const long *)M.rp; R.val = M.v; R.col = M.cl;
    if (dense_twin) {
      R.dense = 1;
      DZ_HIP(hipMemsetAsync(A.qcount + 8, 0, 32, ctx->stream));
    }
    return nray > 0 ? launch(true, R, nwg) : 0;
  }
  int statuses() {
    int rc;
    std::vector<int> hs(nr1), hb(nr1);
    unsigned hq[2] = {0, 0};
    if (nray > 0) {
      DZ_HIP(hipMemcpyAsync(hq, A.qcount + 16, 8, hipMemcpyDeviceToHost, ctx->stream));
      DZ_HIP(hipMemcpyAsync(hs.data(), A.status, nray * 4, hipMemcpyDeviceToHost, ctx->stream));
      DZ_HIP(hipMemcpyAsync(hb.data(), A.rbflag, nray * 4, hipMemcpyDeviceToHost, ctx->stream));
      DZ_HIP(hipStreamSynchronize(ctx->stream));
    }
    int nb = 0, err = 0;
    for (int64_t i = 0; i < nray; i++) {
      nb += hb[i];
      if (hs[i] && !err) err = dz_fail(ctx, hs[i], "ray %ld: receiver lies outside model", (long)i);
    }
    if (n_boundary) *n_boundary = nb;
    if (nnz_out) *nnz_out = arrays.nnz;
    ctx->ksec["rays.list_sweeps"] = hq[0];
    ctx->ksec["rays.list_retraced"] = hq[1];
    ctx->ksec["rays.lcap"] = A.lcap;
    if ((rc = d.dsurf.finish())) return rc;
    DZ_HIP(hipStreamSynchronize(ctx->stream));
    return err;
  }
  int adopt() {
    int rc;
    const int64_t n = (int64_t)g.nvx * g.nvz * (map ? kmax : nz - 1) * (joint ? 3 : 1);
    arrays.keep = true;
    if ((rc = dz_csr_adopt_cap(ctx, nray, n, arrays.nnz, arrays.rp, arrays.cl, arrays.v, nray + res_rows, arrays.cap_nnz, G))) return rc;
    if (twin) {
      dazim_csr *Gd = nullptr;
      arrays_d.keep = true;
      if ((rc = dz_csr_adopt_cap(ctx, nray, n, arrays_d.nnz, arrays_d.rp, arrays_d.cl, arrays_d.v, 0, 0, &Gd)) || (rc = dz_csr_set_twin(ctx, *G, Gd))) {
        dazim_csr_free(ctx, *G);
        *G = nullptr;
        return rc;
      }
    }
    return 0;
  }
  int run() {
    int rc;
    if ((rc = check()) || (rc = decide_overlap()) || (rc = stage_inputs()) || (rc = kernel_constants()) || (rc = scratch()) ||
        (rc = launch_shape()) || (rc = sort_rays()))
      return rc;
    DzTimer t(ctx, "rays");
    DZ_HIP(hipMemsetAsync(A.count, 0, (size_t)(nray + 1) * 8, ctx->stream));
    if ((rc = overlap ? count_passes_beside_eikonal() : count_pass())) return rc;
    if ((rc = scan_and_emit(arrays, A.count, res_nnz, false))) return rc;
    if (twin && ((rc = dz_big_get(ctx, (size_t)(nray + 1), &arrays_d.rp)) || (rc = scan_and_emit(arrays_d, A.countd, 0, true)))) return rc;
    t.stop();
    if (overlap) {
      ctx->ksec["rays.after_fmm_count"] = overlap_tail_s;
      ctx->ksec["rays"] += overlap_tail_s;
    }
    return (rc = statuses()) ? rc : adopt();
  }
};

}

extern "C" int dazim_rays_build_G(dazim_ctx *ctx, int nx, int ny, int nz, float goxd, float gozd, float dvxd,
                                  float dvzd, int kmax, const float *vels, int nfield, const float *scx,
                                  const float *scz, const int *period, const int *kidx, const float *veln,
                                  const float *ttn, const float *ttnr, const int *nstsr, const dazim_refbox *boxes,
                                  int64_t nray, const int *field, const float *rcx, const float *rcz,
                                  const double *svs, const double *svp, const double *srho, float *dsurf,
                                  dazim_csr **G, int64_t *nnz_out, int *n_boundary) {
  RayBuild b(ctx);
  b.nx = nx; b.ny = ny; b.nz = nz; b.goxd = goxd; b.gozd = gozd; b.dvxd = dvxd; b.dvzd = dvzd;
  b.kmax = kmax; b.vels = vels; b.svs = svs; b.svp = svp; b.srho = srho;
  b.nfield = nfield; b.scx = scx; b.scz = scz; b.period = period; b.kidx = kidx;
  b.veln = veln; b.ttn = ttn; b.ttnr = ttnr; b.nstsr = nstsr; b.boxes = boxes;
  b.nray = nray; b.field = field; b.rcx = rcx; b.rcz = rcz;
  b.dsurf = dsurf; b.G = G; b.nnz_out = nnz_out; b.n_boundary = n_boundary;
  return b.run();
}
extern "C" int dazim_rays_build_G_joint(dazim_ctx *ctx, int nx, int ny, int nz, float goxd, float gozd, float dvxd,
                                        float dvzd, int kmax, const float *vels, int nfield, const float *scx,
                                        const float *scz, const int *period, const int *kidx, const float *veln,
                                        const float *ttn, const float *ttnr, const int *nstsr,
                                        const dazim_refbox *boxes, int64_t nray, const int *field, const float *rcx,
                                        const float *rcz, const double *svs, const double *svp, const double *srho,
                                        const float *lsen, float *dsurf, dazim_csr **G, int64_t *nnz_out,
                                        int *n_boundary) {
  if (!lsen) return dz_fail(ctx, DAZIM_E_BAD_ARG, "joint mode needs Lsen_Gsc");
  RayBuild b(ctx);
  b.nx = nx; b.ny = ny; b.nz = nz; b.goxd = goxd; b.gozd = gozd; b.dvxd = dvxd; b.dvzd = dvzd;
  b.kmax = kmax; b.vels = vels; b.svs = svs; b.svp = svp; b.srho = srho; b.lsen = lsen;
  b.nfield = nfield; b.scx = scx; b.scz = scz; b.period = period; b.kidx = kidx;
  b.veln = veln; b.ttn = ttn; b.ttnr = ttnr; b.nstsr = nstsr; b.boxes = boxes;
  b.nray = nray; b.field = field; b.rcx = rcx; b.rcz = rcz;
  b.dsurf = dsurf; b.G = G; b.nnz_out = nnz_out; b.n_boundary = n_boundary;
  return b.run();
}

extern "C" int dazim_rays_build_G_maps(dazim_ctx *ctx, int nx, int ny, float goxd, float gozd, float dvxd, float dvzd, int kmax,
                                       int azim, int nfield, const float *scx, const float *scz, const int *period,
                                       const float *veln, const float *ttn, const float *ttnr, const int *nstsr,
                                       const dazim_refbox *boxes, int64_t nray, const int *field, const float *rcx,
                                       const float *rcz, float *dsurf, dazim_csr **G, int64_t *nnz_out, int *n_boundary) {
  RayBuild b(ctx);
  b.map = true; b.azim = azim != 0;
  b.nx = nx; b.ny = ny; b.nz = 2; b.goxd = goxd; b.gozd = gozd; b.dvxd = dvxd; b.dvzd = dvzd;
  b.kmax = kmax; b.nfield = nfield; b.scx = scx; b.scz = scz; b.period = period;
  b.veln = veln; b.ttn = ttn; b.ttnr = ttnr; b.nstsr = nstsr; b.boxes = boxes;
  b.nray = nray; b.field = field; b.rcx = rcx; b.rcz = rcz;
  b.dsurf = dsurf; b.G = G; b.nnz_out = nnz_out; b.n_boundary = n_boundary;
  return b.run();
}

extern "C" int dazim_ray_paths_dims(dazim_ctx *ctx, int64_t *nray, int *cap) {
  if (!ctx || !nray || !cap) return DAZIM_E_BAD_ARG;
  *nray = (int64_t)dazim_last_kernel_seconds(ctx, "rays.path_rays");
  *cap = (int)dazim_last_kernel_seconds(ctx, "rays.path_cap");
  if (*nray < 0) *nray = 0;
  if (*cap < 0) *cap = 0;
  return 0;
}
extern "C" int dazim_ray_paths_copy(dazim_ctx *ctx, float *xz, int *nrp) {
  int64_t nray;
  int cap;
  if (!ctx || !xz || !nrp || dazim_ray_paths_dims(ctx, &nray, &cap)) return DAZIM_E_BAD_ARG;
  if (nray == 0 || cap == 0) return dz_fail(ctx, DAZIM_E_BAD_ARG, "no ray paths were kept (option rays.keep_paths)");
  auto a = ctx->scratch.find("rays.pts"), b = ctx->scratch.find("rays.npts");
  if (a == ctx->scratch.end() || b == ctx->scratch.end()) return dz_fail(ctx, DAZIM_E_BAD_ARG, "no ray paths were kept");
  DZ_HIP(hipMemcpyAsync(xz, a->second.first, (size_t)nray * cap * 8, hipMemcpyDefault, ctx->stream));
  DZ_HIP(hipMemcpyAsync(nrp, b->second.first, (size_t)nray * 4, hipMemcpyDefault, ctx->stream));
  DZ_HIP(hipStreamSynchronize(ctx->stream));
  return 0;
}
```

dazimsurftomo_amd/csrc/sparse.hip:

```cpp
#include "sparse_internal.h"

#include <type_traits>

#include <rocprim/device/device_radix_sort.hpp>
#include <rocprim/device/device_scan.hpp>

namespace {

__global__ __launch_bounds__(64 * WPB) void spmv_rows(int64_t nrows, const int64_t *__restrict__ ptr,
                                                        const int *__restrict__ idx,
                                                        const float *__restrict__ val,
                                                        const float *__restrict__ x, float *__restrict__ out,
                                                        const float *__restrict__ beta_p, float beta_sign,
                                                        double *__restrict__ sumsq, const int *__restrict__ guard) {
  if (guard && *guard) return;
  const int lane = threadIdx.x & 63, w = threadIdx.x >> 6;
  const float beta = beta_p ? beta_sign * beta_p[0] : beta_sign;
  double sq = 0.0;
  for (int64_t r = (int64_t)blockIdx.x * WPB + w; r < nrows; r += (int64_t)gridDim.x * WPB) {
    const int64_t s = ptr[r], e = ptr[r + 1];
    float acc = 0.0f;
    int64_t s4 = (s + 3) & ~(int64_t)3;
    if (s4 > e) s4 = e;
    for (int64_t i = s + lane; i < s4; i += 64) acc += val[i] * x[idx[i]];
// ... 35 lines not shown
                                                           const IT *__restrict__ idx, const float *__restrict__ val,
                                                           const float *__restrict__ x, float *__restrict__ out,
                                                           const float *__restrict__ beta_p, float beta_sign,
                                                           double *__restrict__ sumsq, const int *__restrict__ guard) {
  extern __shared__ __attribute__((aligned(16))) float xs[];
  if (guard && *guard) return;
  for (int64_t i = threadIdx.x * 4; i < nx; i += 64 * LWPB * 4) {
    if (i + 3 < nx)
      *reinterpret_cast<float4 *>(xs + i) = *reinterpret_cast<const float4 *>(x + i);
    else
      for (int64_t j = i; j < nx; j++) xs[j] = x[j];
  }
  __syncthreads();
  const int lane = threadIdx.x & 63, w = threadIdx.x >> 6;
  const float beta = beta_p ? beta_sign * beta_p[0] : beta_sign;
  double sq = 0.0;
  for (int64_t r = (int64_t)blockIdx.x * LWPB + w; r < nrows; r += (int64_t)gridDim.x * LWPB) {
    const int64_t s = ptr[r], e = ptr[r + 1];
    float acc = 0.0f;
    int64_t s4 = (s + 3) & ~(int64_t)3;
    if (s4 > e) s4 = e;
    for (int64_t i = s + lane; i < s4; i += 64) acc += val[i] * xs[idx[i]];
    const int64_t e4 = s4 + ((e - s4) & ~(int64_t)3);
    int64_t i = s4 + 4 * lane;
    for (; i + 768 < e4; i += 1024) {
      using I4 = typename Idx4<IT>::type;
      float4 v[4];
      I4 c[4];
#pragma unroll
      for (int g = 0; g < 4; g++) {
        v[g] = *reinterpret_cast<const float4 *>(val + i + 256 * g);
        c[g] = *reinterpret_cast<const I4 *>(idx + i + 256 * g);
      }
#pragma unroll
      for (int g = 0; g < 4; g++) {
        acc += v[g].x * xs[c[g].x];
        acc += v[g].y * xs[c[g].y];
        acc += v[g].z * xs[c[g].z];
        acc += v[g].w * xs[c[g].w];
      }
    }
    for (; i + 256 < e4; i += 512) {
      using I4 = typename Idx4<IT>::type;
      const float4 v0 = *reinterpret_cast<const float4 *>(val + i);
      const I4 c0 = *reinterpret_cast<const I4 *>(idx + i);
      const float4 v1 = *reinterpret_cast<const float4 *>(val + i + 256);
      const I4 c1 = *reinterpret_cast<const I4 *>(idx + i + 256);
      acc += v0.x * xs[c0.x];
      acc += v0.y * xs[c0.y];
      acc += v0.z * xs[c0.z];
      acc += v0.w * xs[c0.w];
      acc += v1.x * xs[c1.x];
      acc += v1.y * xs[c1.y];
      acc += v1.z * xs[c1.z];
      acc += v1.w * xs[c1.w];
    }
    for (; i < e4; i += 256) {
      using I4 = typename Idx4<IT>::type;
      const float4 v = *reinterpret_cast<const float4 *>(val + i);
      const I4 c = *reinterpret_cast<const I4 *>(idx + i);
      acc += v.x * xs[c.x];
      acc += v.y * xs[c.y];
      acc += v.z * xs[c.z];
      acc += v.w * xs[c.w];
    }
    for (int64_t k = e4 + lane; k < e; k += 64) acc += val[k] * xs[idx[k]];
    acc = wave_sum(acc);
    if (lane == 0) {
      const float o = beta * out[r] + acc;
      out[r] = o;
      sq += (double)o * (double)o;
    }
  }
  if (sumsq) {
    __shared__ double s_sq[LWPB];
    if (lane == 0) s_sq[w] = sq;
    __syncthreads();
    if (threadIdx.x == 0) {
      double t = 0.0;
      for (int k = 0; k < LWPB; k++) t += s_sq[k];
      sumsq[blockIdx.x] = t;
    }
  }
}
__global__ void k_scale_rows(int64_t nrows, const int64_t *ptr, float *val, const float *w) {
  const int lane = threadIdx.x & 63, wv = threadIdx.x >> 6;
  for (int64_t r = (int64_t)blockIdx.x * WPB + wv; r < nrows; r += (int64_t)gridDim.x * WPB) {
    const float a = w[r];
    for (int64_t i = ptr[r] + lane; i < ptr[r + 1]; i += 64) val[i] *= a;
  }
}
__global__ void k_col_abs_sums(int64_t n, const int *col, const float *val, double scale, unsigned long long *acc) {
  for (int64_t i = (int64_t)blockIdx.x * VB + threadIdx.x; i < n; i += (int64_t)gridDim.x * VB)
    atomicAdd(&acc[col[i]], (unsigned long long)__double2ll_rn((double)fabsf(val[i]) * scale));
}
__global__ void k_fixed_to_float(int64_t n, const unsigned long long *acc, double inv_scale, float *out) {
  for (int64_t i = (int64_t)blockIdx.x * VB + threadIdx.x; i < n; i += (int64_t)gridDim.x * VB) out[i] = (float)((double)acc[i] * inv_scale);
}
__global__ void k_gather_f(int64_t n, const unsigned *perm, const float *src, float *dst) {
  for (int64_t i = (int64_t)blockIdx.x * VB + threadIdx.x; i < n; i += (int64_t)gridDim.x * VB) dst[i] = src[perm[i]];
}
__global__ void k_gather_i(int64_t n, const unsigned *perm, const int *src, int *dst, int add) {
  for (int64_t i = (int64_t)blockIdx.x * VB + threadIdx.x; i < n; i += (int64_t)gridDim.x * VB) dst[i] = src[perm ? perm[i] : (unsigned)i] + add;
}
__global__ void k_iota_keys(int64_t n, const int *one_based, unsigned *keys, unsigned *iota) {
  for (int64_t i = (int64_t)blockIdx.x * VB + threadIdx.x; i < n; i += (int64_t)gridDim.x * VB) {
    if (keys) keys[i] = (unsigned)(one_based[i] - 1);
    iota[i] = (unsigned)i;
  }
}
__global__ void k_lower_bound(int64_t nrows, int64_t nnz, const unsigned *keys, int64_t *ptr) {
  for (int64_t r = (int64_t)blockIdx.x * VB + threadIdx.x; r <= nrows; r += (int64_t)gridDim.x * VB) {
    int64_t lo = 0, hi = nnz;
    while (lo < hi) {
      const int64_t mid = (lo + hi) >> 1;
      if ((int64_t)keys[mid] < r) lo = mid + 1; else hi = mid;
    }
    ptr[r] = lo;
  }
}
__global__ void k_check_range(int64_t n, const int *a, int lo, int hi, int *bad) {
  for (int64_t i = (int64_t)blockIdx.x * VB + threadIdx.x; i < n; i += (int64_t)gridDim.x * VB)
    if (a[i] < lo || a[i] > hi) atomicOr(bad, 1);
}

constexpr int SCW = 16;
constexpr int CBW_MAX = 19 * 1024;

__global__ void k_colblock_ptr(int64_t nrows, int ncb, int cbw, const int64_t *__restrict__ ptr,
                               const int *__restrict__ col, int64_t *__restrict__ cbptr) {
  const int64_t t = (int64_t)blockIdx.x * VB + threadIdx.x;
  if (t >= nrows * (ncb + 1)) return;
  const int64_t r = t / (ncb + 1);
  const int b = (int)(t - r * (ncb + 1));
  int64_t lo = ptr[r], hi = ptr[r + 1];
  const int target = b * cbw;
  while (lo < hi) {
    const int64_t mid = (lo + hi) >> 1;
    if (col[mid] < target) lo = mid + 1; else hi = mid;
  }
  cbptr[t] = lo;
}
constexpr int SPLIT_SHORT = 64;
__global__ void k_last_long_row(int64_t nrows, const int64_t *__restrict__ ptr, int thresh, unsigned long long *res) {
  unsigned long long best = 0;
  for (int64_t r = (int64_t)blockIdx.x * VB + threadIdx.x; r < nrows; r += (int64_t)gridDim.x * VB)
    if (ptr[r + 1] - ptr[r] >= thresh) best = (unsigned long long)(r + 1);
#pragma unroll
  for (int o = 32; o > 0; o >>= 1) {
    const unsigned long long b = __shfl_xor(best, o);
    best = b > best ? b : best;
  }
  if ((threadIdx.x & 63) == 0 && best) atomicMax(res, best);
}
__global__ void k_narrow_cols(int64_t n, const int *__restrict__ col, unsigned short *__restrict__ col16, int mod) {
  for (int64_t i = ((int64_t)blockIdx.x * VB + threadIdx.x) * 4; i < n; i += (int64_t)gridDim.x * VB * 4) {
    if (i + 3 < n) {
      int4 c = *reinterpret_cast<const int4 *>(col + i);
      if (mod > 0) { c.x %= mod; c.y %= mod; c.z %= mod; c.w %= mod; }
      *reinterpret_cast<ushort4 *>(col16 + i) = make_ushort4((unsigned short)c.x, (unsigned short)c.y, (unsigned short)c.z, (unsigned short)c.w);
    } else {
      for (int64_t j = i; j < n; j++) col16[j] = (unsigned short)(mod > 0 ? col[j] % mod : col[j]);
    }
  }
}
__global__ void k_absmax(int64_t n, const float *x, float *part) {
  float v = 0.0f;
  const int64_t n4 = ((reinterpret_cast<uintptr_t>(x) & 15) == 0) ? n / 4 : 0;
  for (int64_t i = (int64_t)blockIdx.x * VB + threadIdx.x; i < n4; i += (int64_t)gridDim.x * VB) {
    const float4 q = reinterpret_cast<const float4 *>(x)[i];
    v = fmaxf(fmaxf(v, fmaxf(fabsf(q.x), fabsf(q.y))), fmaxf(fabsf(q.z), fabsf(q.w)));
  }
  for (int64_t i = n4 * 4 + (int64_t)blockIdx.x * VB + threadIdx.x; i < n; i += (int64_t)gridDim.x * VB) v = fmaxf(v, fabsf(x[i]));
#pragma unroll
  for (int o = 32; o > 0; o >>= 1) v = fmaxf(v, __shfl_xor(v, o));
  __shared__ float s[VB / 64];
  if ((threadIdx.x & 63) == 0) s[threadIdx.x >> 6] = v;
  __syncthreads();
  if (threadIdx.x == 0) {
    float t = 0.0f;
    for (int i = 0; i < VB / 64; i++) t = fmaxf(t, s[i]);
    part[blockIdx.x] = t;
  }
}
__global__ void k_absmax_finish(const float *part, int np, float *res) {
  float v = 0.0f;
  for (int i = threadIdx.x; i < np; i += 64) v = fmaxf(v, part[i]);
#pragma unroll
  for (int o = 32; o > 0; o >>= 1) v = fmaxf(v, __shfl_xor(v, o));
  if (threadIdx.x == 0) res[0] = v;
}

struct RowPtr { int64_t s, e; float aux; };
template <int GL, int NG, class IT, class PtrF, class ElemF, class EndF>
__device__ __forceinline__ void walk_rows(int64_t r_first, int64_t stride, int64_t nrows, int lane, const IT *__restrict__ col,
                                          const float *__restrict__ val, PtrF ptrf, ElemF elemf, EndF endf) {
  using I4 = typename Idx4<IT>::type;
  struct Ent { int64_t r, s4, e4; float aux; float4 v[NG]; I4 k[NG]; float hv, tv; int hk, tk; bool hh, ht; };
  auto load_ptr = [&](int64_t r) {
    RowPtr p = ptrf(r < nrows ? r : 0);
    if (r >= nrows) p.e = p.s;
    return p;
  };
  auto issue = [&](int64_t r, const RowPtr &p) {
    Ent t;
    t.r = r;
    t.aux = p.aux;
    t.s4 = (p.s + 3) & ~(int64_t)3;
    if (t.s4 > p.e) t.s4 = p.e;
    t.e4 = t.s4 + ((p.e - t.s4) & ~(int64_t)3);
#pragma unroll
    for (int g = 0; g < NG; g++) {
      const int64_t i = t.s4 + 4 * lane + (int64_t)g * 4 * GL;
      const int64_t j = i < t.e4 ? i : 0;
      t.v[g] = *reinterpret_cast<const float4 *>(val + j);
      t.k[g] = *reinterpret_cast<const I4 *>(col + j);
    }
    const int64_t ih = p.s + lane, it = t.e4 + lane;
    t.hh = ih < t.s4;
    t.ht = it < p.e;
    t.hv = val[t.hh ? ih : 0];
    t.hk = (int)col[t.hh ? ih : 0];
    t.tv = val[t.ht ? it : 0];
    t.tk = (int)col[t.ht ? it : 0];
    return t;
  };
  auto consume = [&](const Ent &t) {
    if (t.hh) elemf(t.hk, t.hv, t.aux);
#pragma unroll
    for (int g = 0; g < NG; g++) {
      const int64_t i = t.s4 + 4 * lane + (int64_t)g * 4 * GL;
      if (i < t.e4) {
        elemf((int)t.k[g].x, t.v[g].x, t.aux); elemf((int)t.k[g].y, t.v[g].y, t.aux);
        elemf((int)t.k[g].z, t.v[g].z, t.aux); elemf((int)t.k[g].w, t.v[g].w, t.aux);
      }
    }
    for (int64_t i = t.s4 + 4 * lane + (int64_t)NG * 4 * GL; i < t.e4; i += 4 * GL) {
      const float4 v = *reinterpret_cast<const float4 *>(val + i);
      const I4 k = *reinterpret_cast<const I4 *>(col + i);
      elemf((int)k.x, v.x, t.aux); elemf((int)k.y, v.y, t.aux); elemf((int)k.z, v.z, t.aux); elemf((int)k.w, v.w, t.aux);
    }
    if (t.ht) elemf(t.tk, t.tv, t.aux);
    endf(t.r, t.aux);
  };
  int64_t r = r_first;
  Ent eC = issue(r, load_ptr(r));
  RowPtr pB = load_ptr(r + stride);
  for (; r < nrows; r += stride) {
    const RowPtr pA = load_ptr(r + 2 * stride);
    const Ent eB = issue(r + stride, pB);
    consume(eC);
    eC = eB;
    pB = pA;
  }
}

template <int GL, int NG, class IT>
__global__ __launch_bounds__(64 * SCW) void spmvT_scatter(int64_t nsplit, int64_t nrows, int nchunk, int ncb, int cbw, int64_t ncols,
                                                          const int64_t *__restrict__ cbptr, const IT *__restrict__ col,
                                                          const float *__restrict__ val, const float *__restrict__ y,
                                                          double scale, long long *__restrict__ part, const int *__restrict__ guard,
                                                          int pairlocal) {
  extern __shared__ __attribute__((aligned(16))) long long acc[];
  if (guard && *guard) return;
  const int chunk = blockIdx.x / ncb, cb = blockIdx.x - chunk * ncb;
  const int c0 = cb * cbw;
  const int csub = pairlocal ? (cb & 1) * cbw : c0;
  const int width = (int)((ncols - c0) < cbw ? (ncols - c0) : cbw);
  for (int i = threadIdx.x; i < width; i += 64 * SCW) acc[i] = 0;
  __syncthreads();
  constexpr int RPWV = 64 / GL;
  const int lane = (threadIdx.x & 63) % GL, grp = (threadIdx.x & 63) / GL;
  constexpr double MAGIC = 6755399441055744.0;
  auto ptrf = [&](int64_t r) { return RowPtr{cbptr[r * (ncb + 1) + cb], cbptr[r * (ncb + 1) + cb + 1], y[r]}; };
  auto elemf = [&](int c, float v, float yr) {
    atomicAdd((unsigned long long *)&acc[c - csub],
              (unsigned long long)(__double_as_longlong(fma((double)(v * yr), scale, MAGIC)) - __double_as_longlong(MAGIC)));
  };
  walk_rows<GL, NG, IT>(((int64_t)chunk + (int64_t)nchunk * (threadIdx.x >> 6)) * RPWV + grp, (int64_t)nchunk * SCW * RPWV, nsplit, lane,
                        col, val, ptrf, elemf, [](int64_t, float) {});
  if (nsplit < nrows) {
    constexpr int GS = 16, RS = 64 / GS;
    const int lane_s = (threadIdx.x & 63) % GS, grp_s = (threadIdx.x & 63) / GS;
    walk_rows<GS, 1, IT>(nsplit + ((int64_t)chunk + (int64_t)nchunk * (threadIdx.x >> 6)) * RS + grp_s, (int64_t)nchunk * SCW * RS, nrows,
                         lane_s, col, val, ptrf, elemf, [](int64_t, float) {});
  }
  __syncthreads();
  long long *dst = part + (size_t)chunk * ncols + c0;
  for (int i = threadIdx.x; i < width; i += 64 * SCW) dst[i] = acc[i];
}
__global__ void k_scatter_combine(int64_t ncols, int nchunk, const long long *__restrict__ part, double inv_scale,
                                  float *__restrict__ out, const float *__restrict__ beta_p, float beta_sign,
                                  double *__restrict__ sumsq, const int *__restrict__ guard) {
  if (guard && *guard) return;
  const float beta = beta_p ? beta_sign * beta_p[0] : beta_sign;
  double sq = 0.0;
  for (int64_t c = (int64_t)blockIdx.x * VB + threadIdx.x; c < ncols; c += (int64_t)gridDim.x * VB) {
    long long t8[8] = {0, 0, 0, 0, 0, 0, 0, 0};
    int k = 0;
    for (; k + 8 <= nchunk; k += 8)
#pragma unroll
      for (int j = 0; j < 8; j++) t8[j] += part[(size_t)(k + j) * ncols + c];
    for (; k < nchunk; k++) t8[0] += part[(size_t)k * ncols + c];
    const long long t = ((t8[0] + t8[1]) + (t8[2] + t8[3])) + ((t8[4] + t8[5]) + (t8[6] + t8[7]));
    const float o = beta * out[c] + (float)((double)t * inv_scale);
    out[c] = o;
    sq += (double)o * o;
  }
  if (sumsq) block_partial(sq, sumsq);
}

template <int GL, int NG, class IT>
__global__ __launch_bounds__(64 * SCW) void spmv_rows_blocked(int64_t nsplit, int64_t nrows, int nset, int npair, int ncb, int cbw, int64_t ncols,
                                                              const int64_t *__restrict__ cbptr, const IT *__restrict__ col,
                                                              const float *__restrict__ val, const float *__restrict__ x,
                                                              float *__restrict__ part, const int *__restrict__ guard, int pairlocal) {
  extern __shared__ __attribute__((aligned(16))) float xblk[];
  if (guard && *guard) return;
  const int set = blockIdx.x / npair, pr = blockIdx.x - set * npair;
  const int cb0 = 2 * pr, cb1 = (cb0 + 2 < ncb) ? cb0 + 2 : ncb;
  const int c0 = cb0 * cbw;
  const int csub = pairlocal ? 0 : c0;
  const int width = (int)((ncols - c0) < 2 * (int64_t)cbw ? (ncols - c0) : 2 * (int64_t)cbw);
  for (int i = threadIdx.x; i < width; i += 64 * SCW) xblk[i] = x[c0 + i];
  __syncthreads();
  constexpr int RPWV = 64 / GL;
  const int lane = (threadIdx.x & 63) % GL, grp = (threadIdx.x & 63) / GL;
  float acc = 0.0f;
  float *dst = part + (size_t)pr * nrows;
  auto ptrf = [&](int64_t r) { return RowPtr{cbptr[r * (ncb + 1) + cb0], cbptr[r * (ncb + 1) + cb1], 0.0f}; };
  auto elemf = [&](int c, float v, float) { acc += v * xblk[c - csub]; };
  walk_rows<GL, NG, IT>(((int64_t)set + (int64_t)nset * (threadIdx.x >> 6)) * RPWV + grp, (int64_t)nset * SCW * RPWV, nsplit, lane, col, val,
                        ptrf, elemf, [&](int64_t r, float) {
                          float a = acc;
#pragma unroll
                          for (int o = GL / 2; o > 0; o >>= 1) a += __shfl_xor(a, o);
                          if (lane == 0 && r < nsplit) dst[r] = a;
                          acc = 0.0f;
                        });
  if (nsplit < nrows) {
    constexpr int GS = 16, RS = 64 / GS;
    const int lane_s = (threadIdx.x & 63) % GS, grp_s = (threadIdx.x & 63) / GS;
    acc = 0.0f;
    walk_rows<GS, 1, IT>(nsplit + ((int64_t)set + (int64_t)nset * (threadIdx.x >> 6)) * RS + grp_s, (int64_t)nset * SCW * RS, nrows, lane_s,
                         col, val, ptrf, elemf, [&](int64_t r, float) {
                           float a = acc;
#pragma unroll
                           for (int o = GS / 2; o > 0; o >>= 1) a += __shfl_xor(a, o);
                           if (lane_s == 0 && r < nrows) dst[r] = a;
                           acc = 0.0f;
                         });
  }
}
__global__ void k_rows_combine(int64_t nrows, int npair, const float *__restrict__ part, float *__restrict__ out,
                               const float *__restrict__ beta_p, float beta_sign, double *__restrict__ sumsq,
                               const int *__restrict__ guard) {
  if (guard && *guard) return;
  const float beta = beta_p ? beta_sign * beta_p[0] : beta_sign;
  double sq = 0.0;
  for (int64_t r = (int64_t)blockIdx.x * blockDim.x + threadIdx.x; r < nrows; r += (int64_t)gridDim.x * blockDim.x) {
    float t = part[r];
    for (int k = 1; k < npair; k++) t += part[(size_t)k * nrows + r];
    const float o = beta * out[r] + t;
    out[r] = o;
    sq += (double)o * o;
  }
  if (sumsq) block_partial(sq, sumsq);
}

constexpr int64_t LDSX_MAX = 38 * 1024;
bool use_ldsx(dazim_ctx *ctx, int64_t nrows, int64_t nx) {
  if (dz_opt(ctx, "spmv.ldsx", 1) == 0) return false;
  return nx <= LDSX_MAX && nrows >= (int64_t)ctx->num_cu * LWPB * 4;
}
int launch_spmv(dazim_ctx *ctx, int64_t nrows, int64_t nx, const int64_t *ptr, const int *idx, const float *val,
                const float *x, float *out, const float *beta_p, float beta_sign, double *sumsq,
                int nblocks, const int *guard = nullptr, const unsigned short *idx16 = nullptr) {
  if (use_ldsx(ctx, nrows, nx)) {
    const size_t lds = (size_t)((nx + 3) & ~(int64_t)3) * 4;
    if (idx16) {
      DZ_HIP(hipFuncSetAttribute((const void *)spmv_rows_ldsx<unsigned short>, hipFuncAttributeMaxDynamicSharedMemorySize, (int)lds));
      hipLaunchKernelGGL(spmv_rows_ldsx<unsigned short>, dim3(nblocks), dim3(64 * LWPB), lds, ctx->stream, nrows, nx, ptr, idx16, val,
                         x, out, beta_p, beta_sign, sumsq, guard);
    } else {
      DZ_HIP(hipFuncSetAttribute((const void *)spmv_rows_ldsx<int>, hipFuncAttributeMaxDynamicSharedMemorySize, (int)lds));
      hipLaunchKernelGGL(spmv_rows_ldsx<int>, dim3(nblocks), dim3(64 * LWPB), lds, ctx->stream, nrows, nx, ptr, idx, val, x, out,
                         beta_p, beta_sign, sumsq, guard);
    }
  } else {
    hipLaunchKernelGGL(spmv_rows, dim3(nblocks), dim3(64 * WPB), 0, ctx->stream, nrows, ptr, idx, val, x, out,
                       beta_p, beta_sign, sumsq, guard);
  }
  DZ_HIP(hipGetLastError());
  return 0;
}
__global__ void k_expand_rows(int64_t nrows, const int64_t *ptr, unsigned *rowid) {
  const int lane = threadIdx.x & 63, wv = threadIdx.x >> 6;
  for (int64_t r = (int64_t)blockIdx.x * WPB + wv; r < nrows; r += (int64_t)gridDim.x * WPB)
    for (int64_t i = ptr[r] + lane; i < ptr[r + 1]; i += 64) rowid[i] = (unsigned)r;
}
__global__ void k_offset_ptr(int64_t n, const int64_t *src, int64_t add, int64_t *dst) {
  for (int64_t i = (int64_t)blockIdx.x * VB + threadIdx.x; i < n; i += (int64_t)gridDim.x * VB) dst[i] = src[i] + add;
}
template <bool FILL>
__global__ __launch_bounds__(256) void k_threshold_rows(int64_t m, const int64_t *__restrict__ rowptr, const int *__restrict__ col,
                                                        const float *__restrict__ val, float tol, long *__restrict__ cnt,
                                                        const long *__restrict__ rowptr2, int *__restrict__ col2,
                                                        float *__restrict__ val2) {
  const int lane = threadIdx.x & 63;
  const int64_t r = (int64_t)blockIdx.x * 4 + (threadIdx.x >> 6);
  if (r > m) return;
  if (r == m) {
    if (!FILL && lane == 0) cnt[m] = 0;
    return;
  }
  const int64_t s = rowptr[r], e = rowptr[r + 1];
  long kept = 0;
  const long o = FILL ? rowptr2[r] : 0;
  for (int64_t i = s; i < e; i += 64) {
    const int64_t k = i + lane;
    float v = 0.0f;
    int c = 0;
    if (k < e) { v = val[k]; c = col[k]; }
    const bool keep = k < e && fabsf(v) > tol;
    const unsigned long long b = __ballot(keep);
    if (FILL && keep) {
      const long q = o + kept + __popcll(b & ((1ull << lane) - 1ull));
      val2[q] = v;
      col2[q] = c;
    }
    kept += __popcll(b);
  }
  if (!FILL && lane == 0) cnt[r] = kept;
}

bool use_blocked(dazim_ctx *ctx, const dazim_csr *A) {
  if (dz_opt(ctx, "spmv.blocked", 1) == 0) return false;
  return A->cbptr && A->n > LDSX_MAX && A->nnz >= (1 << 22) && A->m >= (int64_t)ctx->num_cu * SCW;
}
int absmax_to_host(dazim_ctx *ctx, const float *x, int64_t n, float *res) {
  int rc;
  float *pm;
  if ((rc = dz_scratch(ctx, "csr.absmax", (size_t)APART + 4, &pm))) return rc;
  const int nb = nblk((n + 3) / 4, APART);
  hipLaunchKernelGGL(k_absmax, dim3(nb), dim3(VB), 0, ctx->stream, n, x, pm);
  hipLaunchKernelGGL(k_absmax_finish, dim3(1), dim3(64), 0, ctx->stream, pm, nb, pm + APART);
  DZ_HIP(hipMemcpyAsync(res, pm + APART, 4, hipMemcpyDeviceToHost, ctx->stream));
  return 0;
}
double fixed_scale(double pm, int64_t m) {
  int e = 0;
  if (pm > 0) (void)frexp(pm, &e);
  int lgm = 0;
  while (((int64_t)1 << lgm) < m) lgm++;
  const int fb = 62 - lgm < 40 ? 62 - lgm : 40;
  return ldexp(1.0, fb - e);
}
struct RowSplit { int64_t nsplit; bool shortseg; };
RowSplit row_split(dazim_ctx *ctx, const dazim_csr *A, double thresh) {
  const bool split = dz_opt(ctx, "spmv.split", 1) != 0 && A->split_row < A->m;
  return {split ? A->split_row : A->m, (split ? A->long_avg : (double)A->nnz / (double)A->m) < thresh};
}
template <class F>
int dispatch_rows(const dazim_csr *A, bool shortseg, F launch) {
  using GL16 = std::integral_constant<int, 16>; using NG2 = std::integral_constant<int, 2>;
  using GL64 = std::integral_constant<int, 64>; using NG4 = std::integral_constant<int, 4>;
  if (A->col16) return shortseg ? launch(GL16(), NG2(), A->col16) : launch(GL64(), NG4(), A->col16);
  return shortseg ? launch(GL16(), NG2(), A->col) : launch(GL64(), NG4(), A->col);
}

}

int dz_spmv_blocks(dazim_ctx *ctx, int64_t nrows, int64_t nx) {
  if (nx >= 0 && use_ldsx(ctx, nrows, nx)) return ctx->num_cu;
  int64_t b = (nrows + WPB - 1) / WPB;
  const int64_t cap = (int64_t)ctx->num_cu * 8;
  if (b > cap) b = cap;
  if (b < 1) b = 1;
  return (int)b;
}

int dz_invalidate_transpose(dazim_csr *A) {
  for (void **pp : {(void **)&A->colptr, (void **)&A->row, (void **)&A->tval, (void **)&A->tperm})
    if (*pp) { (void)hipFree(*pp); *pp = nullptr; }
  return 0;
}
int dz_build_transpose(dazim_ctx *ctx, dazim_csr *A) {
  const int64_t nnz = A->nnz, n = A->n, m = A->m;
  const size_t nz = (size_t)(nnz > 0 ? nnz : 1);
  (void)dz_invalidate_transpose(A);
  DZ_HIP(dz_malloc_retry(ctx, (void **)&A->colptr, (n + 1) * 8));
  DZ_HIP(dz_malloc_retry(ctx, (void **)&A->row, nz * 4));
  DZ_HIP(dz_malloc_retry(ctx, (void **)&A->tval, nz * 4));
  DZ_HIP(dz_malloc_retry(ctx, (void **)&A->tperm, nz * 4));
  if (nnz == 0) {
    DZ_HIP(hipMemsetAsync(A->colptr, 0, (n + 1) * 8, ctx->stream));
    return 0;
  }
  int rc;
  unsigned *ck, *cks, *iota, *rowid;
  if ((rc = dz_scratch(ctx, "csr.k0", nz, &ck)) || (rc = dz_scratch(ctx, "csr.k1", nz, &cks)) ||
      (rc = dz_scratch(ctx, "csr.v0", nz, &iota)) || (rc = dz_scratch(ctx, "csr.perm", nz, &rowid)))
    return rc;
  const int nb = nblk(nnz);
  int cbits = 1;
  while (((int64_t)1 << cbits) < n) cbits++;
  hipLaunchKernelGGL(k_gather_i, dim3(nb), dim3(VB), 0, ctx->stream, nnz, (const unsigned *)nullptr, A->col, (int *)ck, 0);
  hipLaunchKernelGGL(k_iota_keys, dim3(nb), dim3(VB), 0, ctx->stream, nnz, (const int *)nullptr, (unsigned *)nullptr, iota);
  hipLaunchKernelGGL(k_expand_rows, dim3(dz_spmv_blocks(ctx, m, -1)), dim3(64 * WPB), 0, ctx->stream, m, A->rowptr, rowid);
  size_t tb = 0;
  DZ_HIP(rocprim::radix_sort_pairs(nullptr, tb, ck, cks, iota, A->tperm, (size_t)nnz, 0, cbits, ctx->stream));
  void *tmp;
  if ((rc = dz_scratch(ctx, "csr.tmp", tb + 256, &tmp))) return rc;
  DZ_HIP(rocprim::radix_sort_pairs(tmp, tb, ck, cks, iota, A->tperm, (size_t)nnz, 0, cbits, ctx->stream));
  hipLaunchKernelGGL(k_lower_bound, dim3(nblk(n + 1)), dim3(VB), 0, ctx->stream, n, nnz, cks, A->colptr);
  hipLaunchKernelGGL(k_gather_f, dim3(nb), dim3(VB), 0, ctx->stream, nnz, A->tperm, A->val, A->tval);
  hipLaunchKernelGGL(k_gather_i, dim3(nb), dim3(VB), 0, ctx->stream, nnz, A->tperm, (const int *)rowid, A->row, 0);
  DZ_HIP(hipGetLastError());
  return 0;
}

int dz_build_colblocks(dazim_ctx *ctx, dazim_csr *A, int64_t changed_from) {
  if (A->cbptr) { dz_big_put(ctx, A->cbptr); A->cbptr = nullptr; }
  A->ncb = (int)((A->n + CBW_MAX - 1) / CBW_MAX);
  A->cbw = (int)(((A->n + A->ncb - 1) / A->ncb + 3) & ~3ll);
  const int mod16 = A->n <= 65536 ? 0 : 2 * A->cbw;
  const bool want16 = mod16 <= 65536 && A->nnz > 0 && dz_opt(ctx, "spmv.col16", 1) != 0;
  if (A->col16 && (!want16 || A->col16_cap < A->nnz || changed_from == 0 || A->col16_mod != mod16)) {
    dz_big_put(ctx, A->col16);
    A->col16 = nullptr;
    A->col16_cap = 0;
  }
  if (want16 && (!A->col16 || changed_from >= 0)) {
    int64_t from = 0;
    if (!A->col16) {
      A->col16_cap = ((A->cap_nnz > A->nnz ? A->cap_nnz : A->nnz) + 3) & ~(int64_t)3;
      if (int rcp = dz_big_get(ctx, (size_t)A->col16_cap, &A->col16)) return rcp;
      A->col16_mod = mod16;
    } else {
      from = changed_from & ~(int64_t)3;
    }
    const int64_t cnt = A->nnz - from;
    if (cnt > 0)
      hipLaunchKernelGGL(k_narrow_cols, dim3(nblk((cnt + 3) / 4)), dim3(VB), 0, ctx->stream, cnt, A->col + from, A->col16 + from, mod16);
    DZ_HIP(hipGetLastError());
  }
  const int64_t np = A->m * (A->ncb + 1);
  if (np > 0) {
    if (int rcp = dz_big_get(ctx, (size_t)np, &A->cbptr)) return rcp;
    hipLaunchKernelGGL(k_colblock_ptr, dim3((unsigned)((np + VB - 1) / VB)), dim3(VB), 0, ctx->stream, A->m, A->ncb, A->cbw,
                       A->rowptr, A->col, A->cbptr);
    DZ_HIP(hipGetLastError());
  }
  int rc;
  A->vmax = 0.0f;
  A->split_row = A->m;
  A->long_avg = A->m > 0 ? (double)A->nnz / (double)A->m : 0.0;
  if (A->m > 0 && A->nnz > 0) {
    float *pm;
    if ((rc = dz_scratch(ctx, "csr.absmax", (size_t)APART + 4, &pm))) return rc;
    unsigned long long *d_last = reinterpret_cast<unsigned long long *>(pm + APART + 2), h_last = 0;
    DZ_HIP(hipMemsetAsync(d_last, 0, 8, ctx->stream));
    hipLaunchKernelGGL(k_last_long_row, dim3(nblk(A->m)), dim3(VB), 0, ctx->stream, A->m, A->rowptr, SPLIT_SHORT, d_last);
    DZ_HIP(hipMemcpyAsync(&h_last, d_last, 8, hipMemcpyDeviceToHost, ctx->stream));
    DZ_HIP(hipStreamSynchronize(ctx->stream));
    if ((int64_t)h_last < A->m && (int64_t)h_last > 0) {
      int64_t at = 0;
      DZ_HIP(hipMemcpy(&at, A->rowptr + h_last, 8, hipMemcpyDeviceToHost));
      A->split_row = (int64_t)h_last;
      A->long_avg = (double)at / (double)h_last;
    }
  }
  if (A->nnz > 0 && (rc = absmax_to_host(ctx, A->val, A->nnz, &A->vmax))) return rc;
  DZ_HIP(hipStreamSynchronize(ctx->stream));
  return 0;
}
bool dz_use_scatter(dazim_ctx *ctx, const dazim_csr *A) {
  if (dz_opt(ctx, "spmv.scatter", 1) == 0) return false;
  return A->cbptr && A->nnz >= (1 << 22) && A->m >= (int64_t)ctx->num_cu * SCW;
}
int dz_launch_spmvT(dazim_ctx *ctx, const dazim_csr *A, const float *y, float ymax, float *out, const float *beta_p,
                    float beta_sign, double *sumsq, int *npart, const int *guard) {
  const double pm = (double)A->vmax * (double)ymax;
  ctx->ksec["spmvt.kind"] = (dz_use_scatter(ctx, A) && std::isfinite(pm)) ? 1 : 0;
  ctx->ksec["spmvt.idx_bytes"] = (A->col16 && dz_use_scatter(ctx, A) && std::isfinite(pm)) ? 2 : 4;
  if (!dz_use_scatter(ctx, A) || !std::isfinite(pm)) {
    if (!A->colptr) {
      int rc0 = dz_build_transpose(ctx, const_cast<dazim_csr *>(A));
      if (rc0) return rc0;
    }
    const int gn = dz_spmv_blocks(ctx, A->n, A->m);
    if (npart) *npart = gn;
    return launch_spmv(ctx, A->n, A->m, A->colptr, A->row, A->tval, y, out, beta_p, beta_sign, sumsq, gn, guard);
  }
  int nchunk = ctx->num_cu / A->ncb;
  if (nchunk < 1) nchunk = 1;
  int rc;
  long long *part;
  if ((rc = dz_scratch(ctx, "spmvt.part", (size_t)nchunk * A->n, &part))) return rc;
  const double scale = fixed_scale(pm, A->m);
  const size_t lds = (size_t)A->cbw * 8;
  const RowSplit rs = row_split(ctx, A, 400.0 * A->ncb);
  ctx->ksec["spmvt.split_row"] = (double)rs.nsplit;
  const dim3 sgrid(nchunk * A->ncb), sblock(64 * SCW);
  rc = dispatch_rows(A, rs.shortseg, [&](auto gl, auto ng, auto *colp) -> int {
    using IT = std::remove_pointer_t<decltype(colp)>;
    const auto kern = spmvT_scatter<decltype(gl)::value, decltype(ng)::value, IT>;
    DZ_HIP(hipFuncSetAttribute((const void *)kern, hipFuncAttributeMaxDynamicSharedMemorySize, (int)lds));
    hipLaunchKernelGGL(kern, sgrid, sblock, lds, ctx->stream, rs.nsplit, A->m, nchunk, A->ncb, A->cbw, A->n, A->cbptr,
                       (const IT *)colp, A->val, y, scale, part, guard, (sizeof(IT) == 2 && A->col16_mod > 0) ? 1 : 0);
    return 0;
  });
  if (rc) return rc;
  const int nb = nblk(A->n, NPART);
  hipLaunchKernelGGL(k_scatter_combine, dim3(nb), dim3(VB), 0, ctx->stream, A->n, nchunk, part, 1.0 / scale, out, beta_p,
                     beta_sign, sumsq, guard);
  DZ_HIP(hipGetLastError());
  if (npart) *npart = nb;
  return 0;
}

int dz_launch_spmvA(dazim_ctx *ctx, const dazim_csr *A, const float *x, float *out, const float *beta_p, float beta_sign,
                    double *sumsq, int *npart, const int *guard) {
  ctx->ksec["spmv.kind"] = use_blocked(ctx, A) ? 2 : (use_ldsx(ctx, A->m, A->n) ? 1 : 0);
  ctx->ksec["spmv.idx_bytes"] = (A->col16 && (use_blocked(ctx, A) || (use_ldsx(ctx, A->m, A->n) && A->col16_mod == 0))) ? 2 : 4;
  if (!use_blocked(ctx, A)) {
    const int gm = dz_spmv_blocks(ctx, A->m, A->n);
    if (npart) *npart = gm;
    return launch_spmv(ctx, A->m, A->n, A->rowptr, A->col, A->val, x, out, beta_p, beta_sign, sumsq, gm, guard,
                       A->col16_mod == 0 ? A->col16 : nullptr);
  }
  const int npair = (A->ncb + 1) / 2;
  int nset = ctx->num_cu / npair;
  if (nset < 1) nset = 1;
  int rc;
  float *part;
  if ((rc = dz_scratch(ctx, "spmv.part", (size_t)npair * A->m, &part))) return rc;
  const size_t lds = (size_t)A->cbw * 2 * 4;
  const RowSplit rs = row_split(ctx, A, 600.0 * npair);
  ctx->ksec["spmv.split_row"] = (double)rs.nsplit;
  const dim3 bgrid(nset * npair), bblock(64 * SCW);
  rc = dispatch_rows(A, rs.shortseg, [&](auto gl, auto ng, auto *colp) -> int {
    using IT = std::remove_pointer_t<decltype(colp)>;
    const auto kern = spmv_rows_blocked<decltype(gl)::value, decltype(ng)::value, IT>;
    DZ_HIP(hipFuncSetAttribute((const void *)kern, hipFuncAttributeMaxDynamicSharedMemorySize, (int)lds));
    hipLaunchKernelGGL(kern, bgrid, bblock, lds, ctx->stream, rs.nsplit, A->m, nset, npair, A->ncb, A->cbw, A->n, A->cbptr,
                       (const IT *)colp, A->val, x, part, guard, (sizeof(IT) == 2 && A->col16_mod > 0) ? 1 : 0);
    return 0;
  });
  if (rc) return rc;
  const int nb = nblk(A->m, NPART);
  hipLaunchKernelGGL(k_rows_combine, dim3(nb), dim3(VB), 0, ctx->stream, A->m, npair, part, out, beta_p, beta_sign, sumsq, guard);
  DZ_HIP(hipGetLastError());
  if (npart) *npart = nb;
  return 0;
}
int dz_scale_rows(dazim_ctx *ctx, dazim_csr *A, int64_t nrows, const float *w) {
  hipLaunchKernelGGL(k_scale_rows, dim3(dz_spmv_blocks(ctx, nrows, -1)), dim3(64 * WPB), 0, ctx->stream, nrows, A->rowptr, A->val, w);
  if (A->tperm) hipLaunchKernelGGL(k_gather_f, dim3(nblk(A->nnz)), dim3(VB), 0, ctx->stream, A->nnz, A->tperm, A->val, A->tval);
  DZ_HIP(hipGetLastError());
  DZ_HIP(hipStreamSynchronize(ctx->stream));
  return dz_build_colblocks(ctx, A, -1);
}

extern "C" {

int dz_csr_set_twin(dazim_ctx *ctx, dazim_csr *A, dazim_csr *B) {
  if (!A || !B || A->twin) return dz_fail(ctx, DAZIM_E_BAD_ARG, "bad arguments to dz_csr_set_twin");
  A->twin = B;
  return 0;
}
int dazim_csr_take_twin(dazim_ctx *ctx, dazim_csr *A, dazim_csr **twin) {
  if (!A || !twin) return dz_fail(ctx, DAZIM_E_BAD_ARG, "bad arguments to dazim_csr_take_twin");
  *twin = A->twin;
  A->twin = nullptr;
  return 0;
}

int dazim_csr_free(dazim_ctx *ctx, dazim_csr *A) {
  if (!A) return 0;
  if (A->twin) { dazim_csr *t = A->twin; A->twin = nullptr; (void)dazim_csr_free(ctx, t); }
  if (ctx) DZ_HIP(hipStreamSynchronize(ctx->stream));
  else (void)hipDeviceSynchronize();
  void *ps[] = {A->rowptr, A->colptr, A->col, A->row, A->val, A->tval, A->tperm, A->cbptr, A->col16};
  for (void *p : ps)
    if (p) dz_big_put(ctx, p);
  delete A;
  return 0;
}

int dazim_csr_dims(const dazim_csr *A, int64_t *m, int64_t *n, int64_t *nnz) {
  if (!A) return DAZIM_E_BAD_ARG;
  if (m) *m = A->m;
  if (n) *n = A->n;
  if (nnz) *nnz = A->nnz;
  return 0;
}

int dazim_csr_from_coo(dazim_ctx *ctx, int64_t m, int64_t n, int64_t nnz, const int *irow_u,
                       const int *icol_u, const float *rw_u, dazim_csr **out) {
  if (!ctx || !out || m < 1 || n < 1 || nnz < 0 || nnz > 0xfffffff0ll || m > 0x7ffffff0 || n > 0x7ffffff0)
    return dz_fail(ctx, DAZIM_E_BAD_ARG, "bad arguments to dazim_csr_from_coo");
  DZ_HIP(hipSetDevice(ctx->device));
  DzBuf<int> irow, icol;
  DzBuf<float> rw;
  int rc;
  if ((rc = irow.init(ctx, irow_u, nnz, true, false))) return rc;
  if ((rc = icol.init(ctx, icol_u, nnz, true, false))) return rc;
  if ((rc = rw.init(ctx, rw_u, nnz, true, false))) return rc;
  dazim_csr *A = new dazim_csr;
  auto fail = [&](int r) { dazim_csr_free(ctx, A); return r; };
  A->m = m;
  A->n = n;
  A->nnz = nnz;
  const size_t nz = (size_t)(nnz > 0 ? nnz : 1);
  if ((rc = dz_big_get(ctx, (size_t)m + 1, &A->rowptr)) || (rc = dz_big_get(ctx, nz, &A->col)) || (rc = dz_big_get(ctx, nz, &A->val)))
    return fail(rc);
  unsigned *k0, *k1, *v0, *perm;
  int *bad;
  if ((rc = dz_scratch(ctx, "csr.k0", nz, &k0)) || (rc = dz_scratch(ctx, "csr.k1", nz, &k1)) ||
      (rc = dz_scratch(ctx, "csr.v0", nz, &v0)) || (rc = dz_scratch(ctx, "csr.perm", nz, &perm)) ||
      (rc = dz_scratch(ctx, "csr.bad", 4, &bad)))
    return fail(rc);
  DZ_HIP(hipMemsetAsync(bad, 0, 4, ctx->stream));
  const int nb = nblk(nnz);
  if (nnz > 0) {
    hipLaunchKernelGGL(k_check_range, dim3(nb), dim3(VB), 0, ctx->stream, nnz, irow.dev, 1, (int)m, bad);
    hipLaunchKernelGGL(k_check_range, dim3(nb), dim3(VB), 0, ctx->stream, nnz, icol.dev, 1, (int)n, bad);
    int hbad = 0;
    DZ_HIP(hipMemcpyAsync(&hbad, bad, 4, hipMemcpyDeviceToHost, ctx->stream));
    DZ_HIP(hipStreamSynchronize(ctx->stream));
    if (hbad) {
      dazim_csr_free(ctx, A);
      return dz_fail(ctx, DAZIM_E_BAD_ARG, "COO index outside 1..m / 1..n");
    }
    int rbits = 1, cbits = 1;
    while (((int64_t)1 << rbits) < m) rbits++;
    while (((int64_t)1 << cbits) < n) cbits++;
    unsigned *permc;
    if ((rc = dz_scratch(ctx, "csr.permc", nz, &permc))) return fail(rc);
    hipLaunchKernelGGL(k_iota_keys, dim3(nb), dim3(VB), 0, ctx->stream, nnz, icol.dev, k0, v0);
    size_t tb = 0, tb1 = 0;
    DZ_HIP(rocprim::radix_sort_pairs(nullptr, tb, k0, k1, v0, permc, (size_t)nnz, 0, cbits, ctx->stream));
    DZ_HIP(rocprim::radix_sort_pairs(nullptr, tb1, k0, k1, permc, perm, (size_t)nnz, 0, rbits, ctx->stream));
    if (tb1 > tb) tb = tb1;
    void *tmp;
    if ((rc = dz_scratch(ctx, "csr.tmp", tb + 256, &tmp))) return fail(rc);
    DZ_HIP(rocprim::radix_sort_pairs(tmp, tb, k0, k1, v0, permc, (size_t)nnz, 0, cbits, ctx->stream));
    hipLaunchKernelGGL(k_gather_i, dim3(nb), dim3(VB), 0, ctx->stream, nnz, permc, irow.dev, (int *)k0, -1);
    DZ_HIP(rocprim::radix_sort_pairs(tmp, tb, k0, k1, permc, perm, (size_t)nnz, 0, rbits, ctx->stream));
    hipLaunchKernelGGL(k_lower_bound, dim3(nblk(m + 1)), dim3(VB), 0, ctx->stream, m, nnz, k1, A->rowptr);
    hipLaunchKernelGGL(k_gather_f, dim3(nb), dim3(VB), 0, ctx->stream, nnz, perm, rw.dev, A->val);
    hipLaunchKernelGGL(k_gather_i, dim3(nb), dim3(VB), 0, ctx->stream, nnz, perm, icol.dev, A->col, -1);
    DZ_HIP(hipGetLastError());
  } else {
    DZ_HIP(hipMemsetAsync(A->rowptr, 0, (m + 1) * 8, ctx->stream));
  }
  if ((rc = dz_build_colblocks(ctx, A))) return fail(rc);
  if ((rc = dz_invalidate_transpose(A))) return fail(rc);
  DZ_HIP(hipStreamSynchronize(ctx->stream));
  *out = A;
  return 0;
}

int dazim_csr_adopt(dazim_ctx *ctx, int64_t m, int64_t n, int64_t nnz, int64_t *rowptr, int *col, float *val,
                    dazim_csr **out) {
  return dz_csr_adopt_cap(ctx, m, n, nnz, rowptr, col, val, 0, 0, out);
}

int dz_csr_adopt_cap(dazim_ctx *ctx, int64_t m, int64_t n, int64_t nnz, int64_t *rowptr, int *col, float *val,
                     int64_t cap_m, int64_t cap_nnz, dazim_csr **out) {
  if (!ctx || !out || !rowptr) return DAZIM_E_BAD_ARG;
  dazim_csr *A = new dazim_csr;
  A->m = m; A->n = n; A->nnz = nnz;
  A->rowptr = rowptr; A->col = col; A->val = val;
  if (cap_m > m) A->cap_m = cap_m;
  if (cap_nnz > nnz) A->cap_nnz = cap_nnz;
  int rc;
  if ((rc = dz_build_colblocks(ctx, A)) || (rc = dz_invalidate_transpose(A))) {
    dazim_csr_free(ctx, A);
    return rc;
  }
  DZ_HIP(hipStreamSynchronize(ctx->stream));
  *out = A;
  return 0;
}

int dazim_csr_threshold(dazim_ctx *ctx, const dazim_csr *A, float tol, int64_t reserve_rows, int64_t reserve_nnz, dazim_csr **out) {
  if (!ctx || !A || !out || reserve_rows < 0 || reserve_nnz < 0) return dz_fail(ctx, DAZIM_E_BAD_ARG, "bad arguments to dazim_csr_threshold");
  DZ_HIP(hipSetDevice(ctx->device));
  const int64_t m = A->m;
  int rc;
  long *cnt;
  if ((rc = dz_scratch(ctx, "thr.cnt", (size_t)(m + 1), &cnt))) return rc;
  int64_t *rowptr = nullptr;
  float *val = nullptr;
  int *col = nullptr;
  struct Arrays {
    dazim_ctx *c; int64_t *&rp; float *&v; int *&cl; bool keep = false;
    ~Arrays() { if (!keep) { dz_big_put(c, rp); dz_big_put(c, v); dz_big_put(c, cl); } }
  } arrays{ctx, rowptr, val, col};
  if ((rc = dz_big_get(ctx, (size_t)(m + reserve_rows + 1), &rowptr))) return rc;
  const unsigned nb = (unsigned)((m + 1 + 3) / 4);
  hipLaunchKernelGGL((k_threshold_rows<false>), dim3(nb), dim3(256), 0, ctx->stream, m, A->rowptr, A->col, A->val, tol, cnt,
                     (const long *)nullptr, (int *)nullptr, (float *)nullptr);
  size_t tb = 0;
  DZ_HIP(rocprim::exclusive_scan(nullptr, tb, cnt, (long *)rowptr, 0l, (size_t)(m + 1), rocprim::plus<long>(), ctx->stream));
  void *p;
  if ((rc = dz_scratch(ctx, "thr.scan", tb + 256, &p))) return rc;
  DZ_HIP(rocprim::exclusive_scan(p, tb, cnt, (long *)rowptr, 0l, (size_t)(m + 1), rocprim::plus<long>(), ctx->stream));
  long nnz = 0;
  DZ_HIP(hipMemcpyAsync(&nnz, rowptr + m, 8, hipMemcpyDeviceToHost, ctx->stream));
  DZ_HIP(hipStreamSynchronize(ctx->stream));
  const int64_t cap = nnz + reserve_nnz;
  if ((rc = dz_big_get(ctx, (size_t)(cap > 0 ? cap : 1), &val)) || (rc = dz_big_get(ctx, (size_t)(cap > 0 ? cap : 1), &col))) return rc;
  hipLaunchKernelGGL((k_threshold_rows<true>), dim3(nb), dim3(256), 0, ctx->stream, m, A->rowptr, A->col, A->val, tol, cnt,
                     (const long *)rowptr, col, val);
  DZ_HIP(hipGetLastError());
  arrays.keep = true;
  return dz_csr_adopt_cap(ctx, m, A->n, nnz, rowptr, col, val, m + reserve_rows, cap, out);
}

int dazim_csr_append_coo(dazim_ctx *ctx, dazim_csr *A, int64_t extra_m, int64_t nnz2, const int *irow_u,
                         const int *icol_u, const float *rw_u) {
  if (!ctx || !A || extra_m < 0 || nnz2 < 0) return DAZIM_E_BAD_ARG;
  if (extra_m == 0 && nnz2 == 0) return 0;
  DzBuf<int> irow;
  int rc;
  if ((rc = irow.init(ctx, irow_u, nnz2, true, false))) return rc;
  int *shifted;
  if ((rc = dz_scratch(ctx, "csr.shift", (size_t)(nnz2 > 0 ? nnz2 : 1), &shifted))) return rc;
  if (nnz2 > 0) hipLaunchKernelGGL(k_gather_i, dim3(nblk(nnz2)), dim3(VB), 0, ctx->stream, nnz2, (const unsigned *)nullptr, irow.dev, shifted, (int)-A->m);
  dazim_csr *B = nullptr;
  if ((rc = dazim_csr_from_coo(ctx, extra_m > 0 ? extra_m : 1, A->n, nnz2, shifted, icol_u, rw_u, &B))) return rc;
  const int64_t m2 = A->m + extra_m, nz2 = A->nnz + nnz2;
  if (A->cap_m >= m2 && A->cap_nnz >= nz2) {
    const int64_t nnz1 = A->nnz;
    if (extra_m > 0)
      hipLaunchKernelGGL(k_offset_ptr, dim3(nblk(extra_m + 1)), dim3(VB), 0, ctx->stream, extra_m + 1, B->rowptr, A->nnz, A->rowptr + A->m);
    DZ_HIP(hipMemcpyAsync(A->col + nnz1, B->col, (size_t)nnz2 * 4, hipMemcpyDeviceToDevice, ctx->stream));
    DZ_HIP(hipMemcpyAsync(A->val + nnz1, B->val, (size_t)nnz2 * 4, hipMemcpyDeviceToDevice, ctx->stream));
    DZ_HIP(hipStreamSynchronize(ctx->stream));
    dazim_csr_free(ctx, B);
    A->m = m2;
    A->nnz = nz2;
    if ((rc = dz_build_colblocks(ctx, A, nnz1 > 0 ? nnz1 : 0))) return rc;
    if ((rc = dz_invalidate_transpose(A))) return rc;
    DZ_HIP(hipStreamSynchronize(ctx->stream));
    return 0;
  }
  int64_t *rowptr;
  int *col;
  float *val;
  if ((rc = dz_big_get(ctx, (size_t)(m2 + 1), &rowptr)) || (rc = dz_big_get(ctx, (size_t)(nz2 > 0 ? nz2 : 1), &col)) ||
      (rc = dz_big_get(ctx, (size_t)(nz2 > 0 ? nz2 : 1), &val)))
    return rc;
  DZ_HIP(hipMemcpyAsync(rowptr, A->rowptr, (A->m + 1) * 8, hipMemcpyDeviceToDevice, ctx->stream));
  if (extra_m > 0)
    hipLaunchKernelGGL(k_offset_ptr, dim3(nblk(extra_m + 1)), dim3(VB), 0, ctx->stream, extra_m + 1, B->rowptr, A->nnz, rowptr + A->m);
  DZ_HIP(hipMemcpyAsync(col, A->col, (size_t)A->nnz * 4, hipMemcpyDeviceToDevice, ctx->stream));
  DZ_HIP(hipMemcpyAsync(val, A->val, (size_t)A->nnz * 4, hipMemcpyDeviceToDevice, ctx->stream));
  DZ_HIP(hipMemcpyAsync(col + A->nnz, B->col, (size_t)nnz2 * 4, hipMemcpyDeviceToDevice, ctx->stream));
  DZ_HIP(hipMemcpyAsync(val + A->nnz, B->val, (size_t)nnz2 * 4, hipMemcpyDeviceToDevice, ctx->stream));
  DZ_HIP(hipStreamSynchronize(ctx->stream));
  dazim_csr_free(ctx, B);
  dz_big_put(ctx, A->rowptr);
  dz_big_put(ctx, A->col);
  dz_big_put(ctx, A->val);
  A->rowptr = rowptr; A->col = col; A->val = val;
  A->m = m2; A->nnz = nz2;
  A->cap_m = A->cap_nnz = 0;
  if ((rc = dz_build_colblocks(ctx, A))) return rc;
  if ((rc = dz_invalidate_transpose(A))) return rc;
  DZ_HIP(hipStreamSynchronize(ctx->stream));
  return 0;
}

int dazim_csr_to_coo(dazim_ctx *ctx, const dazim_csr *A, int *irow_u, int *icol_u, float *rw_u) {
  if (!ctx || !A) return DAZIM_E_BAD_ARG;
  DzBuf<int> irow, icol;
  DzBuf<float> rw;
  int rc;
  if ((rc = irow.init(ctx, irow_u, A->nnz, false, true))) return rc;
  if ((rc = icol.init(ctx, icol_u, A->nnz, false, true))) return rc;
  if ((rc = rw.init(ctx, rw_u, A->nnz, false, true))) return rc;
  if (A->nnz > 0) {
    unsigned *rowid;
    if ((rc = dz_scratch(ctx, "csr.perm", (size_t)A->nnz, &rowid))) return rc;
    hipLaunchKernelGGL(k_expand_rows, dim3(dz_spmv_blocks(ctx, A->m, -1)), dim3(64 * WPB), 0, ctx->stream, A->m, A->rowptr, rowid);
    const int nb = nblk(A->nnz);
    if (irow.dev) hipLaunchKernelGGL(k_gather_i, dim3(nb), dim3(VB), 0, ctx->stream, A->nnz, (const unsigned *)nullptr, (const int *)rowid, irow.dev, 1);
    if (icol.dev) hipLaunchKernelGGL(k_gather_i, dim3(nb), dim3(VB), 0, ctx->stream, A->nnz, (const unsigned *)nullptr, A->col, icol.dev, 1);
    if (rw.dev) DZ_HIP(hipMemcpyAsync(rw.dev, A->val, (size_t)A->nnz * 4, hipMemcpyDeviceToDevice, ctx->stream));
    DZ_HIP(hipGetLastError());
  }
  if ((rc = irow.finish()) || (rc = icol.finish()) || (rc = rw.finish())) return rc;
  DZ_HIP(hipStreamSynchronize(ctx->stream));
  return 0;
}

int dazim_csr_scale_rows(dazim_ctx *ctx, dazim_csr *A, const float *w_u) {
  if (!ctx || !A || !w_u) return DAZIM_E_BAD_ARG;
  DzBuf<float> w;
  int rc;
  if ((rc = w.init(ctx, w_u, A->m, true, false))) return rc;
  return dz_scale_rows(ctx, A, A->m, w.dev);
}

int dazim_csr_col_abs_sums(dazim_ctx *ctx, const dazim_csr *A, float *out_u) {
  if (!ctx || !A || !out_u) return DAZIM_E_BAD_ARG;
  DzBuf<float> out;
  int rc;
  if ((rc = out.init(ctx, out_u, A->n, false, true))) return rc;
  unsigned long long *acc;
  if ((rc = dz_scratch(ctx, "csr.colacc", (size_t)A->n, &acc))) return rc;
  DZ_HIP(hipMemsetAsync(acc, 0, (size_t)A->n * 8, ctx->stream));
  const double scale = fixed_scale((double)A->vmax, A->m);
  if (A->nnz) hipLaunchKernelGGL(k_col_abs_sums, dim3(nblk(A->nnz)), dim3(VB), 0, ctx->stream, A->nnz, A->col, A->val, scale, acc);
  hipLaunchKernelGGL(k_fixed_to_float, dim3(nblk(A->n)), dim3(VB), 0, ctx->stream, A->n, acc, 1.0 / scale, out.dev);
  DZ_HIP(hipGetLastError());
  if ((rc = out.finish())) return rc;
  DZ_HIP(hipStreamSynchronize(ctx->stream));
  return 0;
}

int dazim_aprod(dazim_ctx *ctx, int mode, const dazim_csr *A, float *x_u, float *y_u) {
  if (!ctx || !A || !x_u || !y_u || (mode != 1 && mode != 2)) return dz_fail(ctx, DAZIM_E_BAD_ARG, "bad arguments to dazim_aprod");
  DZ_HIP(hipSetDevice(ctx->device));
  DzBuf<float> x, y;
  int rc;
  if ((rc = x.init(ctx, x_u, A->n, true, mode == 2))) return rc;
  if ((rc = y.init(ctx, y_u, A->m, true, mode == 1))) return rc;
  if (mode == 1) {
    DzTimer t(ctx, "spmv");
    if ((rc = dz_launch_spmvA(ctx, A, x.dev, y.dev, nullptr, 1.0f, nullptr, nullptr))) return rc;
    t.stop();
  } else {
    float ymax = 1.0f;
    if (dz_use_scatter(ctx, A)) {
      if ((rc = absmax_to_host(ctx, y.dev, A->m, &ymax))) return rc;
      DZ_HIP(hipStreamSynchronize(ctx->stream));
    }
    DzTimer t(ctx, "spmvt");
    if ((rc = dz_launch_spmvT(ctx, A, y.dev, ymax, x.dev, nullptr, 1.0f, nullptr, nullptr))) return rc;
    t.stop();
  }
  if ((rc = x.finish()) || (rc = y.finish())) return rc;
  DZ_HIP(hipStreamSynchronize(ctx->stream));
  return 0;
}

}
```

dazimsurftomo_amd/csrc/sparse_internal.h:

```cpp
#pragma once
#include "dazim_internal.h"

struct dazim_csr {
  int64_t m = 0, n = 0, nnz = 0;
  int64_t *rowptr = nullptr, *colptr = nullptr;
  int *col = nullptr, *row = nullptr;
  float *val = nullptr, *tval = nullptr;
  unsigned *tperm = nullptr;
  int ncb = 0, cbw = 0;
  int64_t *cbptr = nullptr;
  float vmax = 0.0f;
  int64_t split_row = 0;
  double long_avg = 0.0;
  unsigned short *col16 = nullptr;
  int64_t col16_cap = 0;
  int col16_mod = 0;
  int64_t cap_m = 0, cap_nnz = 0;
  dazim_csr *twin = nullptr;
};

constexpr int WPB = 4;
constexpr int VB = 256;
constexpr int NPART = 256;
constexpr int APART = 2048;

__device__ __forceinline__ float wave_sum(float v) {
#pragma unroll
  for (int o = 32; o > 0; o >>= 1) v += __shfl_xor(v, o);
  return v;
}
__device__ __forceinline__ double wave_sum(double v) {
#pragma unroll
  for (int o = 32; o > 0; o >>= 1) v += __shfl_xor(v, o);
  return v;
}
__device__ __forceinline__ void block_partial(double v, double *part) {
  __shared__ double s[VB / 64];
  v = wave_sum(v);
  if ((threadIdx.x & 63) == 0) s[threadIdx.x >> 6] = v;
  __syncthreads();
  if (threadIdx.x == 0) {
    double t = 0.0;
    for (int i = 0; i < VB / 64; i++) t += s[i];
    part[blockIdx.x] = t;
  }
}
inline int nblk(int64_t n, int cap = 2048) {
  int64_t b = (n + VB - 1) / VB;
  if (b < 1) b = 1;
  return (int)(b > cap ? cap : b);
}

#pragma GCC visibility push(hidden)
int dz_spmv_blocks(dazim_ctx *ctx, int64_t nrows, int64_t nx = -1);
bool dz_use_scatter(dazim_ctx *ctx, const dazim_csr *A);
int dz_launch_spmvA(dazim_ctx *ctx, const dazim_csr *A, const float *x, float *out, const float *beta_p, float beta_sign,
                    double *sumsq, int *npart, const int *guard = nullptr);
int dz_launch_spmvT(dazim_ctx *ctx, const dazim_csr *A, const float *y, float ymax, float *out, const float *beta_p,
                    float beta_sign, double *sumsq, int *npart, const int *guard = nullptr);
int dz_build_transpose(dazim_ctx *ctx, dazim_csr *A);
int dz_invalidate_transpose(dazim_csr *A);
int dz_build_colblocks(dazim_ctx *ctx, dazim_csr *A, int64_t changed_from = 0);
int dz_scale_rows(dazim_ctx *ctx, dazim_csr *A, int64_t nrows, const float *w);
#pragma GCC visibility pop
```

Before: 54440.

## Defer CSR column-block prep, emit col16 and vmax in ray kernel, reduce statuses on device

Splits column-block construction into a lazy dz_csr_prepare that runs on first SpMV use, and tracks staleness and vmax knowledge. Appends can then update vmax from the new tail only, instead of rescanning all values. The ray emit kernel now writes 16-bit column indices and a wave-reduced absolute max directly, so separate narrowing and absmax passes are skipped. Ray status and boundary counts are reduced on the device into a pinned struct instead of copying full arrays to the host, which also removes several host syncs. The cost is more state to keep consistent: stale flags, vmax_known, and the col16 ownership passed into adopt.

Result: no change. 54670 (median of 6 runs) (+0.4%).

```diff
diff --git a/dazimsurftomo_amd/csrc/assemble.hip b/dazimsurftomo_amd/csrc/assemble.hip
--- a/dazimsurftomo_amd/csrc/assemble.hip
+++ b/dazimsurftomo_amd/csrc/assemble.hip
@@ -270,11 +270,12 @@
     DZ_HIP(hipGetLastError());
     A->m = m2;
     A->nnz = nz2;
-    if ((rc = dz_build_colblocks(ctx, A, nnz1 > 0 ? nnz1 : 0))) return rc;
+    if ((rc = dz_csr_cols_changed(ctx, A, nnz1 > 0 ? nnz1 : 0, nnz1))) return rc;
     if ((rc = dz_invalidate_transpose(A))) return rc;
     DZ_HIP(hipStreamSynchronize(ctx->stream));
     return 0;
   }
+  const int64_t nnz1 = A->nnz;
   int64_t *rowptr;
   int *col;
   float *val;
@@ -293,7 +294,7 @@
   A->rowptr = rowptr; A->col = col; A->val = val;
   A->m = m2; A->nnz = nz2;
   A->cap_m = A->cap_nnz = 0;
-  if ((rc = dz_build_colblocks(ctx, A))) return rc;
+  if ((rc = dz_csr_cols_changed(ctx, A, 0, nnz1))) return rc;
   if ((rc = dz_invalidate_transpose(A))) return rc;
   DZ_HIP(hipStreamSynchronize(ctx->stream));
   return 0;
diff --git a/dazimsurftomo_amd/csrc/dazim_internal.h b/dazimsurftomo_amd/csrc/dazim_internal.h
--- a/dazimsurftomo_amd/csrc/dazim_internal.h
+++ b/dazimsurftomo_amd/csrc/dazim_internal.h
@@ -137,7 +137,7 @@
 }
 
 extern "C" int dz_csr_adopt_cap(dazim_ctx *ctx, int64_t m, int64_t n, int64_t nnz, int64_t *rowptr, int *col, float *val,
-                                int64_t cap_m, int64_t cap_nnz, dazim_csr **out);
+                                int64_t cap_m, int64_t cap_nnz, dazim_csr **out, unsigned short *col16, const float *vmax);
 
 extern "C" int dz_csr_set_twin(dazim_ctx *ctx, dazim_csr *A, dazim_csr *B);
 
diff --git a/dazimsurftomo_amd/csrc/lsmr.hip b/dazimsurftomo_amd/csrc/lsmr.hip
--- a/dazimsurftomo_amd/csrc/lsmr.hip
+++ b/dazimsurftomo_amd/csrc/lsmr.hip
@@ -408,6 +408,7 @@
         (r = dz_scratch(ctx, "lsmr.state", 1, &S)))
       return r;
     if (trace && (r = dz_scratch(ctx, "lsmr.trace", (size_t)trace_cap, &d_trace))) return r;
+    if ((r = dz_csr_prepare(ctx, A))) return r;
     if (!dz_use_scatter(ctx, A) && !A->colptr && (r = dz_build_transpose(ctx, const_cast<dazim_csr *>(A)))) return r;
     const int64_t lv = localSize < 0 ? 0 : (localSize < n ? localSize : n);
     if (lv > 0 && (r = dz_scratch(ctx, "lsmr.localV", (size_t)n * lv, &localV))) return r;
diff --git a/dazimsurftomo_amd/csrc/rays.hip b/dazimsurftomo_amd/csrc/rays.hip
--- a/dazimsurftomo_amd/csrc/rays.hip
+++ b/dazimsurftomo_amd/csrc/rays.hip
@@ -63,6 +63,8 @@
   const long *rowptr;
   float *val;
   int *col;
+  unsigned short *col16;
+  unsigned *vmax_bits;
 };
 
 __device__ __forceinline__ float dz_sinf(float x) {
@@ -222,6 +224,7 @@
   unsigned *qcnt = A.qcount + (EMIT ? 8 : 0);
   int chunk = (int)(blockIdx.x % nxcd);
   int traced = 0;
+  float vmax = 0.0f;
   for (;;) {
     RAYS_ARGS_FRESH;
     long quad = -1;
@@ -655,6 +658,8 @@
               const long pos = rstart + cnt + __popc(m & ((1u << gl) - 1u));
               A.val[pos] = rowv;
               A.col[pos] = nk + cbase[i] - 1;
+              if (A.col16) A.col16[pos] = (unsigned short)(nk + cbase[i] - 1);
+              vmax = fmaxf(vmax, fabsf(rowv));
             }
             cnt += __popc(m);
           }
@@ -717,6 +722,8 @@
             const long pos = rstart + cnt + __popc(m & ((1u << gl) - 1u));
             A.val[pos] = rowv;
             A.col[pos] = nn - 1;
+            if (A.col16) A.col16[pos] = (unsigned short)(nn - 1);
+            vmax = fmaxf(vmax, fabsf(rowv));
           }
           cnt += __popc(m);
         }
@@ -728,9 +735,38 @@
       if (!status && nlist > A.LK) atomicAdd(&A.qcount[17], 1u);
     }
   }
+  if (EMIT) {
+    RAYS_ARGS_FRESH;
+#pragma unroll
+    for (int o = 32; o > 0; o >>= 1) vmax = fmaxf(vmax, __shfl_xor(vmax, o));
+    if (lane == 0 && A.vmax_bits && vmax > 0.0f) atomicMax(A.vmax_bits, __float_as_uint(vmax));
+  }
 }
 #undef A
 #undef RAYS_ARGS_FRESH
+
+__global__ void k_ray_status_reduce(long nray, const int *__restrict__ status, const int *__restrict__ rbflag, unsigned *out) {
+  int nb = 0;
+  unsigned long long key = 0;
+  for (long i = (long)blockIdx.x * blockDim.x + threadIdx.x; i < nray; i += (long)gridDim.x * blockDim.x) {
+    nb += rbflag[i];
+    if (status[i] && !key) key = (unsigned long long)(nray - i);
+  }
+#pragma unroll
+  for (int o = 32; o > 0; o >>= 1) {
+    nb += __shfl_xor(nb, o);
+    const unsigned long long k2 = __shfl_xor(key, o);
+    key = k2 > key ? k2 : key;
+  }
+  if ((threadIdx.x & 63) == 0) {
+    if (nb) atomicAdd(out, (unsigned)nb);
+    if (key) atomicMax(reinterpret_cast<unsigned long long *>(out) + 1, key);
+  }
+}
+__global__ void k_ray_status_pick(long nray, const int *__restrict__ status, unsigned *out) {
+  const unsigned long long key = reinterpret_cast<const unsigned long long *>(out)[1];
+  out[1] = key ? (unsigned)status[nray - (long)key] : 0u;
+}
 
 struct RayBuild {
   dazim_ctx *ctx;
@@ -763,7 +799,8 @@
   } d;
   struct Arrays {
     dazim_ctx *c; int64_t *rp = nullptr; float *v = nullptr; int *cl = nullptr; int64_t nnz = 0, cap_nnz = 0; bool keep = false;
-    ~Arrays() { if (!keep) { dz_big_put(c, rp); dz_big_put(c, v); dz_big_put(c, cl); } }
+    unsigned short *c16 = nullptr;
+    ~Arrays() { if (!keep) { dz_big_put(c, rp); dz_big_put(c, v); dz_big_put(c, cl); if (c16) dz_big_put(c, c16); } }
   } arrays, arrays_d;
   dazim_geom g;
   bool joint = false, tiled = false, overlap = false, twin = false;
@@ -771,6 +808,9 @@
   int64_t res_rows = 0, res_nnz = 0;
   long nwg = 0;
   double overlap_tail_s = 0.0;
+  int64_t ncols = 0;
+  bool have_vmax = false;
+  float vmax = 0.0f;
   RayArgs A;
   explicit RayBuild(dazim_ctx *c) : ctx(c), swap{c, c ? c->stream : nullptr}, arrays{c}, arrays_d{c} {}
   int check() {
@@ -1063,6 +1103,14 @@
     if ((rc = dz_big_get(ctx, cap, &M.v)) || (rc = dz_big_get(ctx, cap, &M.cl))) return rc;
     RayArgs R = A;
     R.rowptr = (const long *)M.rp; R.val = M.v; R.col = M.cl;
+    R.col16 = nullptr; R.vmax_bits = nullptr;
+    if (!dense_twin && nray > 0) {
+      if (ncols <= 65536 && M.nnz > 0 && dz_opt(ctx, "spmv.col16", 1) != 0 && dz_opt(ctx, "rays.emit_col16", 1) != 0) {
+        if ((rc = dz_big_get(ctx, (size_t)((M.cap_nnz + 3) & ~(int64_t)3), &M.c16))) return rc;
+        R.col16 = M.c16;
+      }
+      if (dz_opt(ctx, "rays.emit_vmax", 1) != 0) { R.vmax_bits = A.qcount + 24; have_vmax = true; }
+    }
     if (dense_twin) {
       R.dense = 1;
       DZ_HIP(hipMemsetAsync(A.qcount + 8, 0, 32, ctx->stream));
@@ -1071,37 +1119,56 @@
   }
   int statuses() {
     int rc;
-    std::vector<int> hs(nr1), hb(nr1);
-    unsigned hq[2] = {0, 0};
+    struct Host { unsigned sweeps, retraced, pending, pad, nb, status; unsigned long long key; unsigned vmax_bits; } *h;
+    { void *hp; if ((rc = dz_pinned(ctx, "rays.host_status", sizeof(Host), &hp))) return rc; h = (Host *)hp; }
+    memset(h, 0, sizeof(Host));
+    const bool reduce = dz_opt(ctx, "rays.status_reduce", 1) != 0;
+    std::vector<int> hs, hb;
     if (nray > 0) {
-      DZ_HIP(hipMemcpyAsync(hq, A.qcount + 16, 8, hipMemcpyDeviceToHost, ctx->stream));
-      DZ_HIP(hipMemcpyAsync(hs.data(), A.status, nray * 4, hipMemcpyDeviceToHost, ctx->stream));
-      DZ_HIP(hipMemcpyAsync(hb.data(), A.rbflag, nray * 4, hipMemcpyDeviceToHost, ctx->stream));
-      DZ_HIP(hipStreamSynchronize(ctx->stream));
-    }
+      if (reduce) {
+        unsigned nb_ = (unsigned)((nray + 255) / 256);
+        if (nb_ > (unsigned)ctx->num_cu * 4) nb_ = (unsigned)ctx->num_cu * 4;
+        hipLaunchKernelGGL(k_ray_status_reduce, dim3(nb_), dim3(256), 0, ctx->stream, (long)nray, A.status, A.rbflag, A.qcount + 20);
+        hipLaunchKernelGGL(k_ray_status_pick, dim3(1), dim3(1), 0, ctx->stream, (long)nray, A.status, A.qcount + 20);
+        DZ_HIP(hipGetLastError());
+      } else {
+        hs.resize(nr1); hb.resize(nr1);
+        DZ_HIP(hipMemcpyAsync(hs.data(), A.status, nray * 4, hipMemcpyDeviceToHost, ctx->stream));
+        DZ_HIP(hipMemcpyAsync(hb.data(), A.rbflag, nray * 4, hipMemcpyDeviceToHost, ctx->stream));
+      }
+      DZ_HIP(hipMemcpyAsync(h, A.qcount + 16, 36, hipMemcpyDeviceToHost, ctx->stream));
+    }
+    if ((rc = d.dsurf.finish())) return rc;
+    DZ_HIP(hipStreamSynchronize(ctx->stream));
     int nb = 0, err = 0;
-    for (int64_t i = 0; i < nray; i++) {
-      nb += hb[i];
-      if (hs[i] && !err) err = dz_fail(ctx, hs[i], "ray %ld: receiver lies outside model", (long)i);
-    }
+    if (reduce) {
+      nb = (int)h->nb;
+      if (h->key) err = dz_fail(ctx, (int)h->status, "ray %ld: receiver lies outside model", (long)(nray - (int64_t)h->key));
+    } else {
+      for (int64_t i = 0; i < nray; i++) {
+        nb += hb[i];
+        if (hs[i] && !err) err = dz_fail(ctx, hs[i], "ray %ld: receiver lies outside model", (long)i);
+      }
+    }
+    if (have_vmax) memcpy(&vmax, &h->vmax_bits, 4);
     if (n_boundary) *n_boundary = nb;
     if (nnz_out) *nnz_out = arrays.nnz;
-    ctx->ksec["rays.list_sweeps"] = hq[0];
-    ctx->ksec["rays.list_retraced"] = hq[1];
+    ctx->ksec["rays.list_sweeps"] = h->sweeps;
+    ctx->ksec["rays.list_retraced"] = h->retraced;
     ctx->ksec["rays.lcap"] = A.lcap;
-    if ((rc = d.dsurf.finish())) return rc;
-    DZ_HIP(hipStreamSynchronize(ctx->stream));
     return err;
   }
   int adopt() {
     int rc;
-    const int64_t n = (int64_t)g.nvx * g.nvz * (map ? kmax : nz - 1) * (joint ? 3 : 1);
+    const int64_t n = ncols;
     arrays.keep = true;
-    if ((rc = dz_csr_adopt_cap(ctx, nray, n, arrays.nnz, arrays.rp, arrays.cl, arrays.v, nray + res_rows, arrays.cap_nnz, G))) return rc;
+    if ((rc = dz_csr_adopt_cap(ctx, nray, n, arrays.nnz, arrays.rp, arrays.cl, arrays.v, nray + res_rows, arrays.cap_nnz, G, arrays.c16,
+                               have_vmax ? &vmax : nullptr)))
+      return rc;
     if (twin) {
       dazim_csr *Gd = nullptr;
       arrays_d.keep = true;
-      if ((rc = dz_csr_adopt_cap(ctx, nray, n, arrays_d.nnz, arrays_d.rp, arrays_d.cl, arrays_d.v, 0, 0, &Gd)) || (rc = dz_csr_set_twin(ctx, *G, Gd))) {
+      if ((rc = dz_csr_adopt_cap(ctx, nray, n, arrays_d.nnz, arrays_d.rp, arrays_d.cl, arrays_d.v, 0, 0, &Gd, nullptr, nullptr)) || (rc = dz_csr_set_twin(ctx, *G, Gd))) {
         dazim_csr_free(ctx, *G);
         *G = nullptr;
         return rc;
@@ -1115,6 +1182,7 @@
         (rc = launch_shape()) || (rc = sort_rays()))
       return rc;
     DzTimer t(ctx, "rays");
+    ncols = (int64_t)g.nvx * g.nvz * (map ? kmax : nz - 1) * (joint ? 3 : 1);
     DZ_HIP(hipMemsetAsync(A.count, 0, (size_t)(nray + 1) * 8, ctx->stream));
     if ((rc = overlap ? count_passes_beside_eikonal() : count_pass())) return rc;
     if ((rc = scan_and_emit(arrays, A.count, res_nnz, false))) return rc;
diff --git a/dazimsurftomo_amd/csrc/sparse.hip b/dazimsurftomo_amd/csrc/sparse.hip
--- a/dazimsurftomo_amd/csrc/sparse.hip
+++ b/dazimsurftomo_amd/csrc/sparse.hip
@@ -211,6 +211,9 @@
     best = b > best ? b : best;
   }
   if ((threadIdx.x & 63) == 0 && best) atomicMax(res, best);
+}
+__global__ void k_entries_before(int64_t nrows, const int64_t *__restrict__ ptr, unsigned long long *res) {
+  res[1] = res[0] <= (unsigned long long)nrows ? (unsigned long long)ptr[res[0]] : 0ull;
 }
 __global__ void k_narrow_cols(int64_t n, const int *__restrict__ col, unsigned short *__restrict__ col16, int mod) {
   for (int64_t i = ((int64_t)blockIdx.x * VB + threadIdx.x) * 4; i < n; i += (int64_t)gridDim.x * VB * 4) {
@@ -495,12 +498,12 @@
 
 bool use_blocked(dazim_ctx *ctx, const dazim_csr *A) {
   if (dz_opt(ctx, "spmv.blocked", 1) == 0) return false;
-  return A->cbptr && A->n > LDSX_MAX && A->nnz >= (1 << 22) && A->m >= (int64_t)ctx->num_cu * SCW;
+  return A->m > 0 && A->n > LDSX_MAX && A->nnz >= (1 << 22) && A->m >= (int64_t)ctx->num_cu * SCW;
 }
 int absmax_to_host(dazim_ctx *ctx, const float *x, int64_t n, float *res) {
   int rc;
   float *pm;
-  if ((rc = dz_scratch(ctx, "csr.absmax", (size_t)APART + 4, &pm))) return rc;
+  if ((rc = dz_scratch(ctx, "csr.absmax", (size_t)APART + 8, &pm))) return rc;
   const int nb = nblk((n + 3) / 4, APART);
   hipLaunchKernelGGL(k_absmax, dim3(nb), dim3(VB), 0, ctx->stream, n, x, pm);
   hipLaunchKernelGGL(k_absmax_finish, dim3(1), dim3(64), 0, ctx->stream, pm, nb, pm + APART);
@@ -579,11 +582,14 @@
   return 0;
 }
 
-int dz_build_colblocks(dazim_ctx *ctx, dazim_csr *A, int64_t changed_from) {
-  if (A->cbptr) { dz_big_put(ctx, A->cbptr); A->cbptr = nullptr; }
+static int col16_form(dazim_csr *A) {
   A->ncb = (int)((A->n + CBW_MAX - 1) / CBW_MAX);
   A->cbw = (int)(((A->n + A->ncb - 1) / A->ncb + 3) & ~3ll);
-  const int mod16 = A->n <= 65536 ? 0 : 2 * A->cbw;
+  return A->n <= 65536 ? 0 : 2 * A->cbw;
+}
+int dz_csr_cols_changed(dazim_ctx *ctx, dazim_csr *A, int64_t changed_from, int64_t tail_from) {
+  A->stale = true;
+  const int mod16 = col16_form(A);
   const bool want16 = mod16 <= 65536 && A->nnz > 0 && dz_opt(ctx, "spmv.col16", 1) != 0;
   if (A->col16 && (!want16 || A->col16_cap < A->nnz || changed_from == 0 || A->col16_mod != mod16)) {
     dz_big_put(ctx, A->col16);
@@ -604,6 +610,22 @@
       hipLaunchKernelGGL(k_narrow_cols, dim3(nblk((cnt + 3) / 4)), dim3(VB), 0, ctx->stream, cnt, A->col + from, A->col16 + from, mod16);
     DZ_HIP(hipGetLastError());
   }
+  if (A->vmax_known && tail_from >= 0 && tail_from < A->nnz) {
+    int rc;
+    void *hp;
+    if ((rc = dz_pinned(ctx, "csr.tail_vmax", 16, &hp)) || (rc = absmax_to_host(ctx, A->val + tail_from, A->nnz - tail_from, (float *)hp))) return rc;
+    DZ_HIP(hipStreamSynchronize(ctx->stream));
+    A->vmax = fmaxf(A->vmax, *(const float *)hp);
+  } else if (tail_from < 0 || !A->vmax_known) {
+    A->vmax_known = false;
+  }
+  return 0;
+}
+int dz_csr_prepare(dazim_ctx *ctx, const dazim_csr *A_) {
+  if (!A_->stale) return 0;
+  dazim_csr *A = const_cast<dazim_csr *>(A_);
+  (void)col16_form(A);
+  if (A->cbptr) { dz_big_put(ctx, A->cbptr); A->cbptr = nullptr; }
   const int64_t np = A->m * (A->ncb + 1);
   if (np > 0) {
     if (int rcp = dz_big_get(ctx, (size_t)np, &A->cbptr)) return rcp;
@@ -612,34 +634,42 @@
     DZ_HIP(hipGetLastError());
   }
   int rc;
-  A->vmax = 0.0f;
+  float *pm;
+  struct Host { unsigned long long last; int64_t at; float vmax; } *h;
+  { void *hp; if ((rc = dz_pinned(ctx, "csr.prepare", sizeof(Host), &hp))) return rc; h = (Host *)hp; }
+  h->last = 0; h->at = 0; h->vmax = 0.0f;
+  if (!A->vmax_known) A->vmax = 0.0f;
   A->split_row = A->m;
   A->long_avg = A->m > 0 ? (double)A->nnz / (double)A->m : 0.0;
-  if (A->m > 0 && A->nnz > 0) {
-    float *pm;
-    if ((rc = dz_scratch(ctx, "csr.absmax", (size_t)APART + 4, &pm))) return rc;
-    unsigned long long *d_last = reinterpret_cast<unsigned long long *>(pm + APART + 2), h_last = 0;
-    DZ_HIP(hipMemsetAsync(d_last, 0, 8, ctx->stream));
+  const bool rows = A->m > 0 && A->nnz > 0, vals = A->nnz > 0 && !A->vmax_known;
+  if (rows) {
+    if ((rc = dz_scratch(ctx, "csr.absmax", (size_t)APART + 8, &pm))) return rc;
+    unsigned long long *d_last = reinterpret_cast<unsigned long long *>(pm + APART + 2);
+    DZ_HIP(hipMemsetAsync(d_last, 0, 16, ctx->stream));
     hipLaunchKernelGGL(k_last_long_row, dim3(nblk(A->m)), dim3(VB), 0, ctx->stream, A->m, A->rowptr, SPLIT_SHORT, d_last);
-    DZ_HIP(hipMemcpyAsync(&h_last, d_last, 8, hipMemcpyDeviceToHost, ctx->stream));
-    DZ_HIP(hipStreamSynchronize(ctx->stream));
-    if ((int64_t)h_last < A->m && (int64_t)h_last > 0) {
-      int64_t at = 0;
-      DZ_HIP(hipMemcpy(&at, A->rowptr + h_last, 8, hipMemcpyDeviceToHost));
-      A->split_row = (int64_t)h_last;
-      A->long_avg = (double)at / (double)h_last;
-    }
-  }
-  if (A->nnz > 0 && (rc = absmax_to_host(ctx, A->val, A->nnz, &A->vmax))) return rc;
-  DZ_HIP(hipStreamSynchronize(ctx->stream));
+    hipLaunchKernelGGL(k_entries_before, dim3(1), dim3(1), 0, ctx->stream, A->m, A->rowptr, d_last);
+    DZ_HIP(hipMemcpyAsync(h, d_last, 16, hipMemcpyDeviceToHost, ctx->stream));
+  }
+  if (vals && (rc = absmax_to_host(ctx, A->val, A->nnz, &h->vmax))) return rc;
+  if (rows || vals) DZ_HIP(hipStreamSynchronize(ctx->stream));
+  if ((int64_t)h->last < A->m && (int64_t)h->last > 0) {
+    A->split_row = (int64_t)h->last;
+    A->long_avg = (double)h->at / (double)h->last;
+  }
+  if (vals) A->vmax = h->vmax;
+  A->vmax_known = true;
+  A->stale = false;
+  ctx->ksec["csr.prepares"] += 1.0;
+  ctx->ksec["csr.vmax"] = (double)A->vmax;
   return 0;
 }
 bool dz_use_scatter(dazim_ctx *ctx, const dazim_csr *A) {
   if (dz_opt(ctx, "spmv.scatter", 1) == 0) return false;
-  return A->cbptr && A->nnz >= (1 << 22) && A->m >= (int64_t)ctx->num_cu * SCW;
+  return A->m > 0 && A->nnz >= (1 << 22) && A->m >= (int64_t)ctx->num_cu * SCW;
 }
 int dz_launch_spmvT(dazim_ctx *ctx, const dazim_csr *A, const float *y, float ymax, float *out, const float *beta_p,
                     float beta_sign, double *sumsq, int *npart, const int *guard) {
+  if (const int rcp = dz_csr_prepare(ctx, A)) return rcp;
   const double pm = (double)A->vmax * (double)ymax;
   ctx->ksec["spmvt.kind"] = (dz_use_scatter(ctx, A) && std::isfinite(pm)) ? 1 : 0;
   ctx->ksec["spmvt.idx_bytes"] = (A->col16 && dz_use_scatter(ctx, A) && std::isfinite(pm)) ? 2 : 4;
@@ -681,6 +711,7 @@
 
 int dz_launch_spmvA(dazim_ctx *ctx, const dazim_csr *A, const float *x, float *out, const float *beta_p, float beta_sign,
                     double *sumsq, int *npart, const int *guard) {
+  if (const int rcp = dz_csr_prepare(ctx, A)) return rcp;
   ctx->ksec["spmv.kind"] = use_blocked(ctx, A) ? 2 : (use_ldsx(ctx, A->m, A->n) ? 1 : 0);
   ctx->ksec["spmv.idx_bytes"] = (A->col16 && (use_blocked(ctx, A) || (use_ldsx(ctx, A->m, A->n) && A->col16_mod == 0))) ? 2 : 4;
   if (!use_blocked(ctx, A)) {
@@ -719,7 +750,7 @@
   if (A->tperm) hipLaunchKernelGGL(k_gather_f, dim3(nblk(A->nnz)), dim3(VB), 0, ctx->stream, A->nnz, A->tperm, A->val, A->tval);
   DZ_HIP(hipGetLastError());
   DZ_HIP(hipStreamSynchronize(ctx->stream));
-  return dz_build_colblocks(ctx, A, -1);
+  return dz_csr_cols_changed(ctx, A, -1);
 }
 
 extern "C" {
@@ -815,7 +846,7 @@
   } else {
     DZ_HIP(hipMemsetAsync(A->rowptr, 0, (m + 1) * 8, ctx->stream));
   }
-  if ((rc = dz_build_colblocks(ctx, A))) return fail(rc);
+  if ((rc = dz_csr_cols_changed(ctx, A))) return fail(rc);
   if ((rc = dz_invalidate_transpose(A))) return fail(rc);
   DZ_HIP(hipStreamSynchronize(ctx->stream));
   *out = A;
@@ -824,23 +855,29 @@
 
 int dazim_csr_adopt(dazim_ctx *ctx, int64_t m, int64_t n, int64_t nnz, int64_t *rowptr, int *col, float *val,
                     dazim_csr **out) {
-  return dz_csr_adopt_cap(ctx, m, n, nnz, rowptr, col, val, 0, 0, out);
+  return dz_csr_adopt_cap(ctx, m, n, nnz, rowptr, col, val, 0, 0, out, nullptr, nullptr);
 }
 
 int dz_csr_adopt_cap(dazim_ctx *ctx, int64_t m, int64_t n, int64_t nnz, int64_t *rowptr, int *col, float *val,
-                     int64_t cap_m, int64_t cap_nnz, dazim_csr **out) {
+                     int64_t cap_m, int64_t cap_nnz, dazim_csr **out, unsigned short *col16, const float *vmax) {
   if (!ctx || !out || !rowptr) return DAZIM_E_BAD_ARG;
   dazim_csr *A = new dazim_csr;
   A->m = m; A->n = n; A->nnz = nnz;
   A->rowptr = rowptr; A->col = col; A->val = val;
   if (cap_m > m) A->cap_m = cap_m;
   if (cap_nnz > nnz) A->cap_nnz = cap_nnz;
-  int rc;
-  if ((rc = dz_build_colblocks(ctx, A)) || (rc = dz_invalidate_transpose(A))) {
+  if (col16) {
+    A->col16 = col16;
+    A->col16_cap = ((A->cap_nnz > nnz ? A->cap_nnz : nnz) + 3) & ~(int64_t)3;
+    A->col16_mod = 0;
+  }
+  int rc;
+  if ((rc = dz_csr_cols_changed(ctx, A, col16 ? -1 : 0)) || (rc = dz_invalidate_transpose(A))) {
     dazim_csr_free(ctx, A);
     return rc;
   }
-  DZ_HIP(hipStreamSynchronize(ctx->stream));
+  if (vmax) { A->vmax = *vmax; A->vmax_known = true; }
+  if (!col16) DZ_HIP(hipStreamSynchronize(ctx->stream));
   *out = A;
   return 0;
 }
@@ -877,7 +914,7 @@
                      (const long *)rowptr, col, val);
   DZ_HIP(hipGetLastError());
   arrays.keep = true;
-  return dz_csr_adopt_cap(ctx, m, A->n, nnz, rowptr, col, val, m + reserve_rows, cap, out);
+  return dz_csr_adopt_cap(ctx, m, A->n, nnz, rowptr, col, val, m + reserve_rows, cap, out, nullptr, nullptr);
 }
 
 int dazim_csr_append_coo(dazim_ctx *ctx, dazim_csr *A, int64_t extra_m, int64_t nnz2, const int *irow_u,
@@ -903,7 +940,7 @@
     dazim_csr_free(ctx, B);
     A->m = m2;
     A->nnz = nz2;
-    if ((rc = dz_build_colblocks(ctx, A, nnz1 > 0 ? nnz1 : 0))) return rc;
+    if ((rc = dz_csr_cols_changed(ctx, A, nnz1 > 0 ? nnz1 : 0, nnz1))) return rc;
     if ((rc = dz_invalidate_transpose(A))) return rc;
     DZ_HIP(hipStreamSynchronize(ctx->stream));
     return 0;
@@ -914,6 +951,7 @@
   if ((rc = dz_big_get(ctx, (size_t)(m2 + 1), &rowptr)) || (rc = dz_big_get(ctx, (size_t)(nz2 > 0 ? nz2 : 1), &col)) ||
       (rc = dz_big_get(ctx, (size_t)(nz2 > 0 ? nz2 : 1), &val)))
     return rc;
+  const int64_t nnz1 = A->nnz;
   DZ_HIP(hipMemcpyAsync(rowptr, A->rowptr, (A->m + 1) * 8, hipMemcpyDeviceToDevice, ctx->stream));
   if (extra_m > 0)
     hipLaunchKernelGGL(k_offset_ptr, dim3(nblk(extra_m + 1)), dim3(VB), 0, ctx->stream, extra_m + 1, B->rowptr, A->nnz, rowptr + A->m);
@@ -929,7 +967,7 @@
   A->rowptr = rowptr; A->col = col; A->val = val;
   A->m = m2; A->nnz = nz2;
   A->cap_m = A->cap_nnz = 0;
-  if ((rc = dz_build_colblocks(ctx, A))) return rc;
+  if ((rc = dz_csr_cols_changed(ctx, A, 0, nnz1))) return rc;
   if ((rc = dz_invalidate_transpose(A))) return rc;
   DZ_HIP(hipStreamSynchronize(ctx->stream));
   return 0;
@@ -974,6 +1012,7 @@
   unsigned long long *acc;
   if ((rc = dz_scratch(ctx, "csr.colacc", (size_t)A->n, &acc))) return rc;
   DZ_HIP(hipMemsetAsync(acc, 0, (size_t)A->n * 8, ctx->stream));
+  if ((rc = dz_csr_prepare(ctx, A))) return rc;
   const double scale = fixed_scale((double)A->vmax, A->m);
   if (A->nnz) hipLaunchKernelGGL(k_col_abs_sums, dim3(nblk(A->nnz)), dim3(VB), 0, ctx->stream, A->nnz, A->col, A->val, scale, acc);
   hipLaunchKernelGGL(k_fixed_to_float, dim3(nblk(A->n)), dim3(VB), 0, ctx->stream, A->n, acc, 1.0 / scale, out.dev);
@@ -990,6 +1029,7 @@
   int rc;
   if ((rc = x.init(ctx, x_u, A->n, true, mode == 2))) return rc;
   if ((rc = y.init(ctx, y_u, A->m, true, mode == 1))) return rc;
+  if ((rc = dz_csr_prepare(ctx, A))) return rc;
   if (mode == 1) {
     DzTimer t(ctx, "spmv");
     if ((rc = dz_launch_spmvA(ctx, A, x.dev, y.dev, nullptr, 1.0f, nullptr, nullptr))) return rc;
diff --git a/dazimsurftomo_amd/csrc/sparse_internal.h b/dazimsurftomo_amd/csrc/sparse_internal.h
--- a/dazimsurftomo_amd/csrc/sparse_internal.h
+++ b/dazimsurftomo_amd/csrc/sparse_internal.h
@@ -10,6 +10,7 @@
   int ncb = 0, cbw = 0;
   int64_t *cbptr = nullptr;
   float vmax = 0.0f;
+  bool stale = true, vmax_known = false;
   int64_t split_row = 0;
   double long_avg = 0.0;
   unsigned short *col16 = nullptr;
@@ -60,6 +61,7 @@
                     float beta_sign, double *sumsq, int *npart, const int *guard = nullptr);
 int dz_build_transpose(dazim_ctx *ctx, dazim_csr *A);
 int dz_invalidate_transpose(dazim_csr *A);
-int dz_build_colblocks(dazim_ctx *ctx, dazim_csr *A, int64_t changed_from = 0);
+int dz_csr_cols_changed(dazim_ctx *ctx, dazim_csr *A, int64_t changed_from = 0, int64_t tail_from = -1);
+int dz_csr_prepare(dazim_ctx *ctx, const dazim_csr *A);
 int dz_scale_rows(dazim_ctx *ctx, dazim_csr *A, int64_t nrows, const float *w);
 #pragma GCC visibility pop
```
